# drscotthawley/signaltrain

Measured on AMD Instinct MI355X. Metric: audio-frames/sec (train step) comp_4c 8192-sample windows @ 1/2/4/8 GPUs, higher is better.
Workload: dtype f32; 1 GPU; comp_4c synthetic, 8192-sample windows, batch 256/GPU, fp32 (BASELINE configs[1]); window=8192, frames_per_window=25, global_batch=256, parallelism=dp1

## Files before the change

### signaltrain_amd/csrc/st_ae.h

```cpp
#pragma once
#include "st_common.h"

namespace sta {

constexpr int NL = 9;
#ifndef ST_AE_ABLATE
#define ST_AE_ABLATE 0
#endif

struct AEOffsets { int w[NL]; int b[NL]; };

struct GroupWalk { int first, end, stride; };
__device__ __forceinline__ GroupWalk fwd_group_walk(const int ngroups, const int NW, const int wave)
{
    const int G = (int)gridDim.x, b = (int)blockIdx.x;
    if ((G & 7) == 0) {
        const int S = G >> 3, x = b & 7, slot = b >> 3;
        const int per = (ngroups + 7) >> 3;
        const int lo = x * per, hi = lo + per < ngroups ? lo + per : ngroups;
        return GroupWalk{lo + wave * S + slot, hi, S * NW};
    }
    return GroupWalk{wave * G + b, ngroups, G * NW};
}

struct CL {
    static constexpr int O0 = 64, O1 = 32, O2 = 16, O3 = 16, O4 = 16, O5 = 16, O6 = 32, O7 = 64, O8 = 16;
    static constexpr int I0 = 32, I1 = 64, I2 = 32, I3 = 16, I4 = 32, I5 = 16, I6 = 16, I7 = 32, I8 = 64;
    static constexpr int A0 = 0, A1 = A0 + O0 * I0, A2 = A1 + O1 * I1, A3 = A2 + O2 * I2, A4 = A3 + O3 * I3, A5 = A4 + O4 * I4,
                         A6 = A5 + O5 * I5, A7 = A6 + O6 * I6, A8 = A7 + O7 * I7, AEND = A8 + O8 * I8;
    static constexpr int B0 = AEND, B1 = B0 + O0, B2 = B1 + O1, B3 = B2 + O2, B4 = B3 + O3, B5 = B4 + O4, B6 = B5 + O5,
                         B7 = B6 + O6, B8 = B7 + O7, FWD_TOTAL = B8 + O8;
    static constexpr int G0 = FWD_TOTAL, G1 = G0 + O0 * I0, G2 = G1 + O1 * I1, G3 = G2 + O2 * I2, G4 = G3 + O3 * I3, G5 = G4 + O4 * I4,
                         G6 = G5 + O5 * I5, G7 = G6 + O6 * I6, G8 = G7 + O7 * I7, BWD_TOTAL = G8 + O8 * I8;
    static_assert(FWD_TOTAL % 4 == 0 && BWD_TOTAL % 4 == 0, "16-byte aligned regions");
};

constexpr int ae_max_elems(int l) { return l == 0 ? 64 * 32 : l == 1 ? 32 * 64 : l == 2 ? 16 * 32 : l == 3 ? 16 * 16 : l == 4 ? 16 * 32 :
                                           l == 5 ? 16 * 16 : l == 6 ? 32 * 16 : l == 7 ? 64 * 32 : 16 * 64; }
template <int NT>
struct AEParamRegs { float v[NL][(64 * 32 + NT - 1) / NT]; float bv[NL]; };

template <int NT>
__device__ __forceinline__ void ae_params_issue(AEParamRegs<NT>& r, const float* __restrict__ ae, const AEOffsets& go,
                                                const int T, const int OT, const int K, const int tid, const int l0, const int l1)
{
    const int out[NL] = {64, 32, 16, 16, 16, 16, 32, 64, OT};
    const int in[NL] = {T, 64, 32, 16, 16 + K, 16, 16, 32, 64};
#pragma unroll
    for (int l = 0; l < NL; ++l) {
        const bool on = l >= l0 && l < l1;
        const int n = on ? out[l] * in[l] : 0;
        const float* src = ae + go.w[l];
#pragma unroll
        for (int u = 0; u < (ae_max_elems(l) + NT - 1) / NT; ++u) { const int e = tid + u * NT; r.v[l][u] = src[e < n ? e : 0]; }
        r.bv[l] = ae[go.b[l] + (tid < out[l] ? tid : 0)];
    }
}
template <int BF> __device__ __forceinline__ unsigned short st_half_bits(const float v)
{
    if constexpr (BF == 2) { union { _Float16 h; unsigned short u; } p; p.h = (_Float16)v; return p.u; }
    else { union { __bf16 h; unsigned short u; } p; p.h = (__bf16)v; return p.u; }
}
template <int BF> __device__ __forceinline__ float st_half_to_float(const unsigned short b)
{
    if constexpr (BF == 2) { union { unsigned short u; _Float16 h; } p; p.u = b; return (float)p.h; }
    else return __uint_as_float((unsigned)b << 16);
}
template <int NT, int BF = 0>
__device__ __forceinline__ void ae_params_scatter(float* lds, const AEParamRegs<NT>& r, const int T, const int OT, const int K,
                                                  const int tid, const int l0, const int l1, const bool dgrad_images)
{
    const int out[NL] = {64, 32, 16, 16, 16, 16, 32, 64, OT};
    const int in[NL] = {T, 64, 32, 16, 16 + K, 16, 16, 32, 64};
    const int outp[NL] = {CL::O0, CL::O1, CL::O2, CL::O3, CL::O4, CL::O5, CL::O6, CL::O7, CL::O8};
    const int inp[NL] = {CL::I0, CL::I1, CL::I2, CL::I3, CL::I4, CL::I5, CL::I6, CL::I7, CL::I8};
    const int ao[NL] = {CL::A0, CL::A1, CL::A2, CL::A3, CL::A4, CL::A5, CL::A6, CL::A7, CL::A8};
    const int bo[NL] = {CL::B0, CL::B1, CL::B2, CL::B3, CL::B4, CL::B5, CL::B6, CL::B7, CL::B8};
    const int gi[NL] = {CL::G0, CL::G1, CL::G2, CL::G3, CL::G4, CL::G5, CL::G6, CL::G7, CL::G8};
#pragma unroll
    for (int l = 0; l < NL; ++l) {
        const bool on = l >= l0 && l < l1;
        const int IN = in[l], n = on ? out[l] * IN : 0, OP = outp[l], IP = inp[l];
#pragma unroll
        for (int u = 0; u < (ae_max_elems(l) + NT - 1) / NT; ++u) {
            const int e = tid + u * NT;
            if (e < n) {
                const int o = e / IN, i = e - o * IN;
                if constexpr (BF) {
                    const unsigned short hb = st_half_bits<BF>(r.v[l][u]);
                    reinterpret_cast<unsigned short*>(lds + ao[l])[(((i >> 2) * OP + o) << 2) + (i & 3)] = hb;
                    if (dgrad_images) reinterpret_cast<unsigned short*>(lds + gi[l])[(((o >> 2) * IP + i) << 2) + (o & 3)] = hb;
                } else {
                lds[ao[l] + (((i >> 2) * OP + o) << 2) + (i & 3)] = r.v[l][u];
                if (dgrad_images) lds[gi[l] + (((o >> 2) * IP + i) << 2) + (o & 3)] = r.v[l][u];
                }
            }
        }
        if (on && tid < out[l]) lds[bo[l] + tid] = r.bv[l];
    }
}
template <int NT, int BF = 0>
__device__ inline void ae_load_lds(float* lds, const float* __restrict__ ae, const AEOffsets& go, const int T, const int OT, const int K,
                                   const int tid, const int l0, const int l1, const bool dgrad_images)
{
    AEParamRegs<NT> r;
    ae_params_issue<NT>(r, ae, go, T, OT, K, tid, l0, l1);
    const int total = dgrad_images ? CL::BWD_TOTAL : CL::FWD_TOTAL;
    for (int e = tid; e < total; e += NT) lds[e] = 0.f;
    __syncthreads();
    ae_params_scatter<NT, BF>(lds, r, T, OT, K, tid, l0, l1, dgrad_images);
}
template <int NT, int BF = 0>
__device__ inline void ae_load_lds2(float* lds, const float* __restrict__ ae_m, const float* __restrict__ ae_p, const AEOffsets& go,
                                    const int T, const int OT, const int K, const int tid, const int l0, const int l1)
{
    AEParamRegs<NT> rm, rp;
    ae_params_issue<NT>(rm, ae_m, go, T, OT, K, tid, l0, l1);
    ae_params_issue<NT>(rp, ae_p, go, T, OT, K, tid, l0, l1);
    for (int e = tid; e < 2 * CL::FWD_TOTAL; e += NT) lds[e] = 0.f;
    __syncthreads();
    ae_params_scatter<NT, BF>(lds, rm, T, OT, K, tid, l0, l1, false);
    ae_params_scatter<NT, BF>(lds + CL::FWD_TOTAL, rp, T, OT, K, tid, l0, l1, false);
}

#define ST_MFMA16(a, b, c) __builtin_amdgcn_mfma_f32_16x16x4f32((a), (b), (c), 0, 0, 0)

__device__ __forceinline__ float ldg32(const float* __restrict__ base, const unsigned elem)
{
    return *reinterpret_cast<const float*>(reinterpret_cast<const char*>(base) + (size_t)(elem << 2));
}
__device__ __forceinline__ void stg32(float* __restrict__ base, const unsigned elem, const float v)
{
    *reinterpret_cast<float*>(reinterpret_cast<char*>(base) + (size_t)(elem << 2)) = v;
}
#define ST_MUL24(a, b) __umul24((unsigned)(a), (unsigned)(b))

typedef short s16x4 __attribute__((ext_vector_type(4)));
typedef __bf16 bf16x4_t __attribute__((ext_vector_type(4)));
typedef _Float16 f16x4_t __attribute__((ext_vector_type(4)));
template <int BF>
__device__ __forceinline__ f32x4 mfma16h(const s16x4 a, const s16x4 b, const f32x4 c)
{
    if constexpr (BF == 2) {
        union { s16x4 s; f16x4_t h; } pa, pb; pa.s = a; pb.s = b;
        return __builtin_amdgcn_mfma_f32_16x16x16f16(pa.h, pb.h, c, 0, 0, 0);
    } else return __builtin_amdgcn_mfma_f32_16x16x16bf16_1k(a, b, c, 0, 0, 0);
}
#define ST_MFMA16B(a, b, c) mfma16h<BF>((a), (b), (c))
template <int BF>
__device__ __forceinline__ s16x4 pack_h4(f32x4 v)
{
    if constexpr (BF == 2) {
        union { f16x4_t h; s16x4 s; } p; p.h = __builtin_convertvector(v, f16x4_t); return p.s;
    } else {
        typedef __bf16 bf16x2_t __attribute__((ext_vector_type(2)));
        typedef float f32x2_t __attribute__((ext_vector_type(2)));
        union { bf16x2_t h; unsigned u; } lo, hi;
        lo.h = __builtin_convertvector((f32x2_t){v[0], v[1]}, bf16x2_t);
        hi.h = __builtin_convertvector((f32x2_t){v[2], v[3]}, bf16x2_t);
        union { unsigned u[2]; s16x4 s; } r; r.u[0] = lo.u; r.u[1] = hi.u; return r.s;
    }
}
#define pack_bf16x4(v) pack_h4<BF>(v)
template <int BF>
__device__ __forceinline__ float round_h(const float v)
{
    if constexpr (BF == 2) return (float)(_Float16)v;
    else {
        union { __bf16 h; unsigned short u; } p; p.h = (__bf16)v;
        union { unsigned u; float f; } q; q.u = (unsigned)p.u << 16; return q.f;
    }
}
#define bf16_rne(v) round_h<BF>(v)

template <int BF>
__device__ __forceinline__ f32x4 frag_read(const float* img, const int idx)
{
    if constexpr (BF) {
        typedef float f32x2_t __attribute__((ext_vector_type(2)));
        const f32x2_t lo = *reinterpret_cast<const f32x2_t*>(reinterpret_cast<const unsigned short*>(img) + idx);
        return __builtin_shufflevector(lo, lo, 0, 1, -1, -1);
    } else return *reinterpret_cast<const f32x4*>(img + idx);
}
__device__ __forceinline__ s16x4 frag_bits(const f32x4 v)
{
    typedef float f32x2_t __attribute__((ext_vector_type(2)));
    union { f32x2_t f; s16x4 s; } p; p.f = __builtin_shufflevector(v, v, 0, 1); return p.s;
}
template <int OUTP, int BF = 0>
__device__ __forceinline__ f32x4 frag_fwd(const float* img, const int ot, const int it, const int g, const int c)
{
    return frag_read<BF>(img, ((4 * it + g) * OUTP + 16 * ot + c) << 2);
}
template <int INP, int BF = 0>
__device__ __forceinline__ f32x4 frag_dgrad(const float* img, const int ot, const int it, const int g, const int c)
{
    return frag_read<BF>(img, ((4 * ot + g) * INP + 16 * it + c) << 2);
}

template <int NC, int OTL, int ITL, int OUTP, int BF = 0>
__device__ __forceinline__ void layer_fwd(const float* const (&W)[NC], const float* const (&bias)[NC],
                                          const f32x4 (&hin)[NC][ITL], f32x4 (&hout)[NC][OTL], const int g, const int c)
{
    s16x4 ph[NC][ITL];
    if constexpr (BF) {
// ... 72 lines not shown
        for (int r = 0; r < 4; ++r) {
            const int t = 16 * it + 4 * g + r;
            const unsigned o = base + ST_MUL24(t < T ? t : 0, F);
            in.v[0][it][r] = ldg32(mag, o); in.v[1][it][r] = ldg32(phs, o);
        }
}
__device__ __forceinline__ void fwd_load_kn(FwdIn& in, const float* __restrict__ knobs, const int K, const int b, const int g)
{
#pragma unroll
    for (int q = 0; q < 4; ++q) { const int kn = 4 * q + g; in.kn[q] = ldg32(knobs, ST_MUL24(b, K) + (unsigned)(kn < K ? kn : 0)); }
}
__device__ __forceinline__ void fwd_load_tl(FwdIn& in, const float* __restrict__ mag, const float* __restrict__ phs,
                                            const int b, const int f, const bool fv, const int T, const int OT, const int F, const int g)
{
    const unsigned base = ST_MUL24(ST_MUL24(b, T), F) + (unsigned)(fv ? f : 0);
#pragma unroll
    for (int r = 0; r < 4; ++r) {
        const int to = 4 * g + r;
        const unsigned o = base + ST_MUL24(to < OT ? T - OT + to : 0, F);
        in.tl[0][r] = ldg32(mag, o); in.tl[1][r] = ldg32(phs, o);
    }
}
__device__ __forceinline__ void fwd_mask_v(f32x4 (&v)[2][2], const FwdIn& in, const bool fv, const int T, const int g)
{
#pragma unroll
    for (int it = 0; it < 2; ++it)
#pragma unroll
        for (int r = 0; r < 4; ++r) {
            const bool ok = fv && 16 * it + 4 * g + r < T;
            v[0][it][r] = ok ? in.v[0][it][r] : 0.f; v[1][it][r] = ok ? in.v[1][it][r] : 0.f;
        }
}
__device__ __forceinline__ void fwd_mask_kn(float (&kn)[4], const FwdIn& in, const int K, const int g)
{
#pragma unroll
    for (int q = 0; q < 4; ++q) kn[q] = (4 * q + g) < K ? in.kn[q] : 0.f;
}
__device__ __forceinline__ void fwd_mask_tl(float (&tl)[2][4], const FwdIn& in, const bool fv, const int OT, const int g)
{
#pragma unroll
    for (int r = 0; r < 4; ++r) { const bool ok = fv && 4 * g + r < OT; tl[0][r] = ok ? in.tl[0][r] : 0.f; tl[1][r] = ok ? in.tl[1][r] : 0.f; }
}

constexpr int AE_SV_TILES = 17;
#ifndef ST_SV_NT
#define ST_SV_NT 1
#endif
template <int NTL>
__device__ __forceinline__ void sv_store(float* __restrict__ p, const unsigned lane16, const int tile0, const f32x4 (&h)[NTL])
{
#pragma unroll
    for (int t = 0; t < NTL; ++t) {
        f32x4* q = reinterpret_cast<f32x4*>(reinterpret_cast<char*>(p + (tile0 + t) * 256) + (size_t)lane16);
#if ST_SV_NT & 1
        __builtin_nontemporal_store(h[t], q);
#else
        *q = h[t];
#endif
    }
}
template <int NTL>
__device__ __forceinline__ void sv_load(const float* __restrict__ p, const unsigned lane16, const int tile0, f32x4 (&h)[NTL])
{
#pragma unroll
    for (int t = 0; t < NTL; ++t) {
        const f32x4* q = reinterpret_cast<const f32x4*>(reinterpret_cast<const char*>(p + (tile0 + t) * 256) + (size_t)lane16);
#if ST_SV_NT & 2
        h[t] = __builtin_nontemporal_load(q);
#else
        h[t] = *q;
#endif
    }
}

template <int NW, int BF = 0, bool SV = false>
__global__ void __launch_bounds__(NW * 64)
ae_fwd_kernel(const float* __restrict__ mag, const float* __restrict__ phs, const float* __restrict__ knobs,
              const float* __restrict__ ae_m, const float* __restrict__ ae_p, const AEOffsets go,
              float* __restrict__ mag_hat, float* __restrict__ phs_hat, float* __restrict__ AA,
              float* __restrict__ reg_partial,
              const int B, const int T, const int OT, const int F, const int K, const int KP, const float expfac,
              float* __restrict__ h4x = nullptr,
              unsigned short* __restrict__ AA16 = nullptr, const int aa_ht = 0,
              float* __restrict__ sv = nullptr)
{
    extern __shared__ __attribute__((aligned(16))) float lds[];
    const int tid = threadIdx.x, lane = tid & 63, wave = tid >> 6;
    const int g = lane >> 4, c = lane & 15;
    const float* const lw[2] = {lds, lds + CL::FWD_TOTAL};
    ae_load_lds2<NW * 64, BF>(lds, ae_m, ae_p, go, T, OT, K, tid, 0, NL);
    __syncthreads();

    const int FP = KP / 2, gpw = FP / 16;
    const int ngroups = B * gpw;
    const int KQ = (K + 3) / 4;
    float reg = 0.f;
    float* const wtab = lds + 2 * CL::FWD_TOTAL;
    for (int i = tid; i < FP; i += NW * 64) wtab[i] = i < F ? expf(expfac * (float)i) : 0.f;
    unsigned toF[4], toK[4];
#pragma unroll
    for (int r = 0; r < 4; ++r) { toF[r] = ST_MUL24(4 * g + r, F); toK[r] = ST_MUL24(4 * g + r, KP); }
    __syncthreads();

    f32x4 vin[2][2];
    const GroupWalk gw = fwd_group_walk(ngroups, NW, wave);
    int grp = gw.first;
    if (grp < gw.end) {
        const int b = grp / gpw, f = (grp - b * gpw) * 16 + c;
        FwdIn first; fwd_load_v(first, mag, phs, b, f, f < F, T, F, g); fwd_mask_v(vin, first, f < F, T, g);
    }
    for (; grp < gw.end; grp += gw.stride) {
        asm volatile("" ::: "memory");
        const int b = grp / gpw, f = (grp - b * gpw) * 16 + c;
        const bool fv = f < F;
        const int gn = grp + gw.stride < gw.end ? grp + gw.stride : grp;
        const int bn = gn / gpw, fn = (gn - bn * gpw) * 16 + c;
        FwdIn cur;
        fwd_load_v(cur, mag, phs, bn, fn, fn < F, T, F, g); fwd_load_kn(cur, knobs, K, b, g); fwd_load_tl(cur, mag, phs, b, f, fv, T, OT, F, g);

        f32x4 h1[2][4], h2[2][2], h3[2][1], h4[2][1], h5[2][1], h6[2][1], h7[2][2], h8[2][4], e9[2][1];
        const int grp_u = SV ? __builtin_amdgcn_readfirstlane(grp) : 0;
#ifdef ST_SV_DIAG
        float* const sv0 = SV ? sv + (size_t)(grp_u & ST_SV_DIAG) * (AE_SV_TILES * 256) : nullptr;
#else
        float* const sv0 = SV ? sv + (size_t)grp_u * (AE_SV_TILES * 256) : nullptr;
#endif
        float* const sv1 = SV ? sv0 + (size_t)ngroups * (AE_SV_TILES * 256) : nullptr;
        const unsigned lane16 = (unsigned)lane << 4;
#define ST_SV(t0_, h_) do { if constexpr (SV) { sv_store(sv0, lane16, t0_, h_[0]); sv_store(sv1, lane16, t0_, h_[1]); } } while (0)
        { const float* const W[2] = ST_W2(CL::A0); const float* const bb[2] = ST_W2(CL::B0); layer_fwd<2, 4, 2, CL::O0, BF>(W, bb, vin, h1, g, c); } ST_SV(0, h1);
        { const float* const W[2] = ST_W2(CL::A1); const float* const bb[2] = ST_W2(CL::B1); layer_fwd<2, 2, 4, CL::O1, BF>(W, bb, h1, h2, g, c); } ST_SV(4, h2);
        { const float* const W[2] = ST_W2(CL::A2); const float* const bb[2] = ST_W2(CL::B2); layer_fwd<2, 1, 2, CL::O2, BF>(W, bb, h2, h3, g, c); } ST_SV(6, h3);
        { const float* const W[2] = ST_W2(CL::A3); const float* const bb[2] = ST_W2(CL::B3); layer_fwd<2, 1, 1, CL::O3, BF>(W, bb, h3, h4, g, c); } ST_SV(7, h4);
        if (h4x) {
            float4* hv = reinterpret_cast<float4*>(h4x);
            hv[(size_t)grp * 64 + lane] = make_float4(h4[0][0][0], h4[0][0][1], h4[0][0][2], h4[0][0][3]);
            hv[((size_t)ngroups + grp) * 64 + lane] = make_float4(h4[1][0][0], h4[1][0][1], h4[1][0][2], h4[1][0][3]);
        }
        if (mag_hat) {
        float knv[4]; fwd_mask_kn(knv, cur, K, g);
        layer5_fwd<2, BF>(lw, h4, knv, KQ, h5, g, c); ST_SV(8, h5);
        { const float* const W[2] = ST_W2(CL::A5); const float* const bb[2] = ST_W2(CL::B5); layer_fwd<2, 1, 1, CL::O5, BF>(W, bb, h5, h6, g, c); } ST_SV(9, h6);
        { const float* const W[2] = ST_W2(CL::A6); const float* const bb[2] = ST_W2(CL::B6); layer_fwd<2, 2, 1, CL::O6, BF>(W, bb, h6, h7, g, c); } ST_SV(10, h7);
        { const float* const W[2] = ST_W2(CL::A7); const float* const bb[2] = ST_W2(CL::B7); layer_fwd<2, 4, 2, CL::O7, BF>(W, bb, h7, h8, g, c); } ST_SV(12, h8);
        { const float* const W[2] = ST_W2(CL::A8); const float* const bb[2] = ST_W2(CL::B8); layer_fwd<2, 1, 4, CL::O8, BF>(W, bb, h8, e9, g, c); } ST_SV(16, e9);
#undef ST_SV
        const float wf = fv ? wtab[f] : 0.f;
        float tlv[2][4]; fwd_mask_tl(tlv, cur, fv, OT, g);
        const unsigned boF = ST_MUL24(ST_MUL24(b, OT), F) + (unsigned)f, boK = ST_MUL24(ST_MUL24(b, OT), KP) + (unsigned)f;
#pragma unroll
        for (int r = 0; r < 4; ++r) {
            const int to = 4 * g + r;
            if (to < OT) {
                float mh = 0.f, ph = 0.f, sn = 0.f, cs = 1.f;
                if (fv) {
                    mh = e9[0][0][r] * tlv[0][r];
                    ph = e9[1][0][r] + tlv[1][r];
                    st_sincos(ph, sn, cs);
                    stg32(mag_hat, boF + toF[r], mh);
                    stg32(phs_hat, boF + toF[r], ph);
                    reg += fabsf(mh * wf);
                }
                if (AA16) {
                    const int ht = BF ? BF : aa_ht;
                    AA16[boK + toK[r]] = st_to_h16(mh * cs, ht);
                    AA16[boK + toK[r] + (unsigned)FP] = st_to_h16(mh * sn, ht);
                } else {
                    stg32(AA, boK + toK[r], mh * cs);
                    stg32(AA, boK + toK[r] + (unsigned)FP, mh * sn);
                }
            }
        }
        }
        fwd_mask_v(vin, cur, fn < F, T, g);
    }
    if (reg_partial) {
        reg = wave_sum(reg);
        if (lane == 0) reg_partial[blockIdx.x * NW + wave] = reg;
    }
}

// ... 171 lines not shown
#pragma unroll
        for (int r = 0; r < 4; ++r) d[t][r] = __builtin_fmaf(d[t][r], __builtin_amdgcn_fmed3f(h[t][r], 0.f, -3.0e38f), d[t][r]);
}

template <int OTL, int ITL, int BF = 0>
__device__ __forceinline__ void wgrad_reg(f32x4 (&dW)[OTL][ITL], float (&db)[OTL], const f32x4 (&daT)[OTL], const f32x4 (&hT)[ITL])
{
    s16x4 pht[ITL];
    if constexpr (BF) {
#pragma unroll
        for (int it = 0; it < ITL; ++it) pht[it] = pack_bf16x4(hT[it]);
    }
#pragma unroll
    for (int ot = 0; ot < OTL; ++ot) {
        s16x4 pdt;
        if constexpr (BF) pdt = pack_bf16x4(daT[ot]);
#pragma unroll
        for (int it = 0; it < ITL; ++it) {
#if ST_AE_ABLATE & 4
            dW[ot][it][0] += daT[ot][0] * hT[it][0];
#else
            if constexpr (BF) dW[ot][it] = ST_MFMA16B(pdt, pht[it], dW[ot][it]);
            else {
#pragma unroll
                for (int r = 0; r < 4; ++r) dW[ot][it] = ST_MFMA16(daT[ot][r], hT[it][r], dW[ot][it]);
            }
#endif
        }
        db[ot] += (daT[ot][0] + daT[ot][1]) + (daT[ot][2] + daT[ot][3]);
    }
}
template <int OTL, int ITL, int BF>
__device__ __forceinline__ void wgrad_regh(f32x4 (&dW)[OTL][ITL], float (&db)[OTL], const f32x4 (&daT)[OTL], const typename TTy<BF>::type (&hT)[ITL])
{
    if constexpr (BF == 0) wgrad_reg<OTL, ITL, 0>(dW, db, daT, hT);
    else {
#pragma unroll
        for (int ot = 0; ot < OTL; ++ot) {
            const s16x4 pdt = pack_bf16x4(daT[ot]);
#pragma unroll
            for (int it = 0; it < ITL; ++it) dW[ot][it] = ST_MFMA16B(pdt, hT[it], dW[ot][it]);
            db[ot] += (daT[ot][0] + daT[ot][1]) + (daT[ot][2] + daT[ot][3]);
        }
    }
}
template <int OTL, int ITL, int INP, bool FIRST>
__device__ __forceinline__ void dw_flush(float* dW, const f32x4 (&acc)[OTL][ITL], const int g, const int c)
{
#pragma unroll
    for (int ot = 0; ot < OTL; ++ot)
#pragma unroll
        for (int it = 0; it < ITL; ++it)
#pragma unroll
            for (int r = 0; r < 4; ++r) {
                float* p = dW + (16 * ot + 4 * g + r) * INP + 16 * it + c;
                if constexpr (FIRST) *p = acc[ot][it][r]; else *p += acc[ot][it][r];
            }
}
template <int OTL, bool FIRST>
__device__ __forceinline__ void db_flush(float* dst, float (&db)[OTL], const int g, const int c)
{
#pragma unroll
    for (int ot = 0; ot < OTL; ++ot) {
        float v = db[ot];
        v += __shfl_xor(v, 16); v += __shfl_xor(v, 32);
        if (g == 0) { if constexpr (FIRST) dst[16 * ot + c] = v; else dst[16 * ot + c] += v; }
    }
}

__device__ __forceinline__ void group_colsum_store(float* __restrict__ dst, const f32x4& t, const int g, const int c)
{
    const float v = (t[0] + t[1]) + (t[2] + t[3]);
    const unsigned u = __builtin_bit_cast(unsigned, v);
    const auto p = __builtin_amdgcn_permlane16_swap(u, u, false, false);
    const float w = __builtin_bit_cast(float, (unsigned)p[0]) + __builtin_bit_cast(float, (unsigned)p[1]);
    const unsigned x = __builtin_bit_cast(unsigned, w);
    const auto q = __builtin_amdgcn_permlane32_swap(x, x, false, false);
    const float s = __builtin_bit_cast(float, (unsigned)q[0]) + __builtin_bit_cast(float, (unsigned)q[1]);
    if (g == 0) dst[c] = s;
}

constexpr int AE_BWD_SCR = (32 + 16 + 16) * SP + 2 * 4 * 320;
constexpr int ae_bwd_lds_floats(int nw) { return (CL::BWD_TOTAL + nw * AE_BWD_SCR) > nw * CL::FWD_TOTAL ? (CL::BWD_TOTAL + nw * AE_BWD_SCR) : nw * CL::FWD_TOTAL; }
template <int NW, bool INNER = false, int BF = 0, int VAR = 1, bool SAVED = false, bool KG = false>
__global__ void __launch_bounds__(NW * 64, 1)
ae_bwd_kernel(const float* __restrict__ mag, const float* __restrict__ phs, const float* __restrict__ knobs,
              const float* __restrict__ ae_m, const float* __restrict__ ae_p, const AEOffsets go, const int PG,
              const float* __restrict__ mag_hat, const float* __restrict__ phs_hat, const float* __restrict__ dAA,
              const float* __restrict__ g_mag_hat, const float reg_coef, const float expfac,
              float* __restrict__ dmag, float* __restrict__ dphs, float* __restrict__ ws,
              const int B, const int T, const int OT, const int F, const int K, const int KP,
              const int to_lo, const int to_hi,
              const int nslab, const size_t slab,
              const float* __restrict__ sv = nullptr,
              float* __restrict__ kg = nullptr)
{
    static_assert(!SAVED || (!INNER && BF == 0), "the kept-activation backward exists for the fused fp32 geometries");
    extern __shared__ __attribute__((aligned(16))) float lds[];
    const int ae = blockIdx.y;
    const int tid = threadIdx.x, lane = tid & 63, wave = tid >> 6;
    const int g = lane >> 4, c = lane & 15;
    float* lw = lds;
    float* Vs = lds + CL::BWD_TOTAL + wave * AE_BWD_SCR;
    float* Ys = Vs + 32 * SP;
    float* Ts = Ys + 16 * SP;
    float* XH = Ts + 16 * SP;
    float* XD = XH + 4 * 320;
    ae_load_lds<NW * 64, BF>(lw, ae ? ae_p : ae_m, go, INNER ? 16 : T, INNER ? 16 : OT, K, tid, INNER ? 1 : 0, INNER ? 8 : NL, true);
    __syncthreads();

    const float* vin = ae ? phs : mag;
    const float* dh8in = ae ? phs_hat : mag_hat;
    float* dvout = ae ? dphs : dmag;
    const int FP = KP / 2, gpw = FP / 16;
    const int ngroups = B * gpw;
    const int gstride = gridDim.x * NW;

    f32x4 rW1[4][2], rW2[2][4], rW3[1][2], rW4[1][1], rW5[1][2], rW6[1][1], rW7[2][1], rW8[4][2], rW9[1][4];
    float rb1[4], rb2[2], rb3[1], rb4[1], rb5[1], rb6[1], rb7[2], rb8[4], rb9[1];
#define ST_ZT(x, A, Bq) { _Pragma("unroll") for (int a_ = 0; a_ < A; ++a_) _Pragma("unroll") for (int b_ = 0; b_ < Bq; ++b_) x[a_][b_] = (f32x4){0.f, 0.f, 0.f, 0.f}; }
#define ST_ZB(x, A) { _Pragma("unroll") for (int a_ = 0; a_ < A; ++a_) x[a_] = 0.f; }
    ST_ZT(rW1, 4, 2) ST_ZT(rW2, 2, 4) ST_ZT(rW3, 1, 2) ST_ZT(rW4, 1, 1) ST_ZT(rW5, 1, 2) ST_ZT(rW6, 1, 1) ST_ZT(rW7, 2, 1) ST_ZT(rW8, 4, 2) ST_ZT(rW9, 1, 4)
    ST_ZB(rb1, 4) ST_ZB(rb2, 2) ST_ZB(rb3, 1) ST_ZB(rb4, 1) ST_ZB(rb5, 1) ST_ZB(rb6, 1) ST_ZB(rb7, 2) ST_ZB(rb8, 4) ST_ZB(rb9, 1)
#undef ST_ZT
#undef ST_ZB

    f32x4 vr[2];
    int grp = blockIdx.x * NW + wave;
    auto load_v = [&](int gq, f32x4 (&dst)[2]) {
        const int bq = gq / gpw, fq = (gq - bq * gpw) * 16 + c;
        const unsigned base = ST_MUL24(ST_MUL24(bq, T), F) + (unsigned)(fq < F ? fq : 0);
#pragma unroll
        for (int it = 0; it < 2; ++it)
#pragma unroll
            for (int r = 0; r < 4; ++r) {
                const int t = 16 * it + 4 * g + r;
                dst[it][r] = ldg32(vin, base + ST_MUL24(t < T ? t : 0, F));
            }
    };
    auto mask_v = [&](int gq, f32x4 (&dst)[2]) {
        const int bq = gq / gpw, fq = (gq - bq * gpw) * 16 + c;
        const bool ok0 = fq < F;
#pragma unroll
        for (int it = 0; it < 2; ++it)
#pragma unroll
            for (int r = 0; r < 4; ++r) dst[it][r] = (ok0 && 16 * it + 4 * g + r < T) ? dst[it][r] : 0.f;
    };
    if constexpr (!INNER) { if (grp < ngroups) { load_v(grp, vr); mask_v(grp, vr); } }
    f32x4 kn = (f32x4){0.f, 0.f, 0.f, 0.f}; float knT = 0.f;
    auto load_kn = [&](int gq, f32x4& d4, float& dT) {
        const unsigned kb = ST_MUL24(gq / gpw, K);
#pragma unroll
        for (int r = 0; r < 4; ++r) { const int kidx = 4 * g + r; d4[r] = ldg32(knobs, kb + (unsigned)(kidx < K ? kidx : 0)); }
        dT = ldg32(knobs, kb + (unsigned)(c < K ? c : 0));
    };
    auto mask_kn = [&](f32x4& d4, float& dT) {
#pragma unroll
        for (int r = 0; r < 4; ++r) d4[r] = (4 * g + r) < K ? d4[r] : 0.f;
        dT = c < K ? dT : 0.f;
    };
    if (grp < ngroups) { load_kn(grp, kn, knT); mask_kn(kn, knT); }
    const unsigned Rw = (unsigned)B * FP;

    constexpr bool GM = (VAR & 1) != 0, TAIL16 = (VAR & 2) != 0;
    float q_x[4][3], q_y[4][3], q_ph[4], q_mh[4], q_mt[4], q_gm[4];
    auto load_q = [&](const int gq) {
        const int bq = gq / gpw, fq0 = (gq - bq * gpw) * 16 + c;
        const bool fvq = fq0 < F;
        const int fq = fvq ? fq0 : 0;
        const size_t o1 = nslab > 1 ? slab : 0, o2 = nslab > 2 ? 2 * slab : 0;
        const float* const dA0 = dAA, * const dA1 = dAA + o1, * const dA2 = dAA + o2;
        const float* const dB0 = dA0 + FP, * const dB1 = dA1 + FP, * const dB2 = dA2 + FP;
        const unsigned bOT = ST_MUL24(bq, OT), btF = ST_MUL24(ST_MUL24(bq, T), F) + (unsigned)fq;
#pragma unroll
        for (int r = 0; r < 4; ++r) {
            const int to = 4 * g + r;
            const bool ok = fvq && to < OT;
            const bool lv = ok && to >= to_lo && to <= to_hi;
            const unsigned ro = bOT + (unsigned)(ok ? to : 0);
            const unsigned p0 = ST_MUL24(lv ? ro : 0u, KP) + (unsigned)fq;
            const unsigned pF = ST_MUL24(ro, F) + (unsigned)fq;
#if ST_AE_ABLATE & 1
            q_x[r][0] = q_x[r][1] = q_x[r][2] = q_y[r][0] = q_y[r][1] = q_y[r][2] = 1e-3f * (float)(p0 & 7); q_ph[r] = 0.3f; q_mh[r] = 0.2f + 1e-3f * (float)(pF & 3);
#else
            q_x[r][0] = ldg32(dA0, p0); q_x[r][1] = ldg32(dA1, p0); q_x[r][2] = ldg32(dA2, p0);
            q_y[r][0] = ldg32(dB0, p0); q_y[r][1] = ldg32(dB1, p0); q_y[r][2] = ldg32(dB2, p0);
            q_ph[r] = ldg32(phs_hat, pF); q_mh[r] = ldg32(mag_hat, pF);
#endif
            if constexpr (GM) q_gm[r] = ldg32(g_mag_hat, pF); else q_gm[r] = 0.f;
            if constexpr (!TAIL16) q_mt[r] = ldg32(vin, btF + ST_MUL24(ok ? T - OT + to : 0, F));
// ... 7 lines not shown
#else
    auto svp = [&](const int gq) { return svn + (size_t)__builtin_amdgcn_readfirstlane(gq) * (AE_SV_TILES * 256); };
#endif
    if constexpr (SAVED) {
        if (grp < ngroups) {
            load_q(grp);
            const float* const p = svp(grp);
            sv_load(p, lane16, 16, s_e9); sv_load(p, lane16, 12, s_h8); sv_load(p, lane16, 10, s_h7); sv_load(p, lane16, 9, s_h6); sv_load(p, lane16, 8, s_h5);
            sv_load(p, lane16, 7, s_h4); sv_load(p, lane16, 6, s_h3); sv_load(p, lane16, 4, s_h2); sv_load(p, lane16, 0, s_h1);
        }
    }

    for (; grp < ngroups; grp += gstride) {
        asm volatile("" ::: "memory");
        const int b = grp / gpw, f = (grp - b * gpw) * 16 + c;
        const bool fv = f < F;
        if constexpr (!INNER && !SAVED) load_q(grp);
        f32x4 h1in[4], dh8[4];
        if constexpr (INNER) {
            const unsigned col0 = (unsigned)b * FP + (unsigned)(grp - b * gpw) * 16;
#pragma unroll
            for (int ot = 0; ot < 4; ++ot) {
#pragma unroll
                for (int r = 0; r < 4; ++r) {
                    h1in[ot][r] = ldg32(vin, (unsigned)(16 * ot + 4 * g + r) * Rw + col0 + c);
                    dh8[ot][r] = ldg32(dh8in, (unsigned)(16 * ot + 4 * g + r) * Rw + col0 + c);
                }
            }
        }
        f32x4 vn[2], knn; float knTn;
        const int gnext = grp + gstride < ngroups ? grp + gstride : grp;
#if ST_AE_ABLATE & 64
        vn[0] = vr[0]; vn[1] = vr[1]; knn = kn; knTn = knT;
#else
        if constexpr (!INNER) load_v(gnext, vn);
        load_kn(gnext, knn, knTn);
#endif

        f32x4 h1[4], h2[2], h3[1], h4[1], h5[1], h6[1], h7[2], h8[4], e9[1];
        f32x4 fr9[1 * 4];
        if constexpr (SAVED) {
#pragma unroll
            for (int it = 0; it < 2; ++it)
#pragma unroll
                for (int r = 0; r < 4; ++r) Vs[(16 * it + 4 * g + r) * SP + c] = vr[it][r];
#pragma unroll
            for (int k = 0; k < 4; ++k) { h1[k] = s_h1[k]; h8[k] = s_h8[k]; }
#pragma unroll
            for (int k = 0; k < 2; ++k) { h2[k] = s_h2[k]; h7[k] = s_h7[k]; }
            h3[0] = s_h3[0]; h4[0] = s_h4[0]; h5[0] = s_h5[0]; h6[0] = s_h6[0]; e9[0] = s_e9[0];
        } else {
        f32x4 fr2[2 * 4];
        if constexpr (INNER) {
#pragma unroll
            for (int ot = 0; ot < 4; ++ot) h1[ot] = h1in[ot];
            frags_fwd<2, 4, CL::O1, BF>(fr2, lw + CL::A1, g, c);
        } else {
            f32x4 fr1[4 * 2]; frags_fwd<4, 2, CL::O0, BF>(fr1, lw + CL::A0, g, c);
            frags_fwd<2, 4, CL::O1, BF>(fr2, lw + CL::A1, g, c);
#pragma unroll
            for (int it = 0; it < 2; ++it)
#pragma unroll
                for (int r = 0; r < 4; ++r) Vs[(16 * it + 4 * g + r) * SP + c] = vr[it][r];
            ST_FENCE();
            fwdD_fr<4, 2, BF>(fr1, lw + CL::B0, vr, h1, g);
        }
        f32x4 fr3[1 * 2]; frags_fwd<1, 2, CL::O2, BF>(fr3, lw + CL::A2, g, c); ST_FENCE(); fwdD_fr<2, 4, BF>(fr2, lw + CL::B1, h1, h2, g);
        f32x4 fr4[1 * 1]; frags_fwd<1, 1, CL::O3, BF>(fr4, lw + CL::A3, g, c); ST_FENCE(); fwdD_fr<1, 2, BF>(fr3, lw + CL::B2, h2, h3, g);
        f32x4 fr5[1 * 2]; frags_fwd<1, 2, CL::O4, BF>(fr5, lw + CL::A4, g, c); ST_FENCE(); fwdD_fr<1, 1, BF>(fr4, lw + CL::B3, h3, h4, g);
        f32x4 fr6[1 * 1]; frags_fwd<1, 1, CL::O5, BF>(fr6, lw + CL::A5, g, c); ST_FENCE();
        {
            const f32x4 hk[2] = {h4[0], kn};
            fwdD_fr<1, 2, BF>(fr5, lw + CL::B4, hk, h5, g);
        }
        f32x4 fr7[2 * 1]; frags_fwd<2, 1, CL::O6, BF>(fr7, lw + CL::A6, g, c); ST_FENCE(); fwdD_fr<1, 1, BF>(fr6, lw + CL::B5, h5, h6, g);
        f32x4 fr8[4 * 2]; frags_fwd<4, 2, CL::O7, BF>(fr8, lw + CL::A7, g, c); ST_FENCE(); fwdD_fr<2, 1, BF>(fr7, lw + CL::B6, h6, h7, g);
        if constexpr (!INNER) frags_fwd<1, 4, CL::O8, BF>(fr9, lw + CL::A8, g, c);
        ST_FENCE(); fwdD_fr<4, 2, BF>(fr8, lw + CL::B7, h7, h8, g);
        }
        f32x4 da9[1];
        float dxA[4], mtA[4];
        if constexpr (!INNER) {
            ST_FENCE();
            const float wf = fv ? expf(expfac * (float)f) : 0.f;
#pragma unroll
            for (int r = 0; r < 4; ++r) {
                const int to = 4 * g + r;
                const bool ok = fv && to < OT;
                const bool lv = ok && to >= to_lo && to <= to_hi;
                const float gre = lv ? q_x[r][0] + (nslab > 1 ? q_x[r][1] : 0.f) + (nslab > 2 ? q_x[r][2] : 0.f) : 0.f;
                const float gim = lv ? q_y[r][0] + (nslab > 1 ? q_y[r][1] : 0.f) + (nslab > 2 ? q_y[r][2] : 0.f) : 0.f;
                const float ph = q_ph[r], mh = q_mh[r];
                if constexpr (!TAIL16) asm volatile("" :: "v"(q_mt[r]));
                float sn, cs; st_sincos(ph, sn, cs);
                const float sg = mh > 0.f ? 1.f : (mh < 0.f ? -1.f : 0.f);
                const float dmh = gre * cs + gim * sn + reg_coef * sg * wf + (GM ? q_gm[r] : 0.f);
                const float dph = mh * (gim * cs - gre * sn);
                dxA[r] = ok ? (ae == 0 ? dmh : dph) : 0.f;
                mtA[r] = ae == 0 ? (TAIL16 ? vr[1][r] : q_mt[r]) : 1.f;
            }
            if constexpr (!SAVED) fwdD_fr<1, 4, BF>(fr9, lw + CL::B8, h8, e9, g);
            if constexpr (BF == 0 && !SAVED) {
#pragma unroll
                for (int p_ = 0; p_ < 16; ++p_) { __builtin_amdgcn_sched_group_barrier(0x008, 1, 0); __builtin_amdgcn_sched_group_barrier(0x002, 7, 0); }
            }
            ST_FENCE();
        }
        if constexpr (!INNER) {
#pragma unroll
            for (int r = 0; r < 4; ++r) {
                const int to = 4 * g + r;
                const float eg = elu_grad_from_out(e9[0][r]);
                const float e1 = ae == 0 ? e9[0][r] : 1.f;
                const float d9 = dxA[r] * mtA[r] * eg;
                const float tail = dxA[r] * e1;
                da9[0][r] = d9;
                Ts[to * SP + c] = tail;
                Ys[to * SP + c] = d9;
            }
        }
#define ST_REFILL(...) do { if constexpr (SAVED) { ST_FENCE(); __VA_ARGS__; ST_FENCE(); } } while (0)
        const float* const svq = SAVED ? svp(gnext) : nullptr;
        ST_REFILL(load_q(gnext); sv_load(svq, lane16, 16, s_e9));
#define ST_PIPE(N_) do { \
        __builtin_amdgcn_sched_group_barrier(0x008, (N_) + 2, 0); \
        _Pragma("unroll") for (int p_ = 0; p_ < (N_) - 2; ++p_) { \
            __builtin_amdgcn_sched_group_barrier(0x002, 2, 0); __builtin_amdgcn_sched_group_barrier(0x300, 1, 0); \
            __builtin_amdgcn_sched_group_barrier(0x008, 1, 0); } \
        ST_FENCE(); } while (0)
#define ST_BWD_STAGE(O_, I_, FD_, DA_, DAT_, HP_, HTP_, DAP_, DATP_, RW_, RB_, NEXT_) \
        to_Th<I_, BF>(XH, HP_, HTP_, g, c); ST_FENCE(); \
        dgradD_fr<O_, I_, BF>(FD_, DA_, DAP_); mul_elu_grad<I_>(DAP_, HP_); \
        to_T<I_>(XD, DAP_, DATP_, g, c); NEXT_; \
        wgrad_regh<O_, I_, BF>(RW_, RB_, DAT_, HTP_); \
        ST_PIPE(BF ? O_ * I_ : O_ * I_ * 4);
        typedef typename TTy<BF>::type tt_t;
        tt_t hT8[4]; f32x4 da8[4], daT8[4], fd8[2 * 4];
        if constexpr (INNER) {
            frags_dgrad<4, 2, CL::I7, BF>(fd8, lw + CL::G7, g, c);
            to_Th<4, BF>(XH, h8, hT8, g, c);
#pragma unroll
            for (int ot = 0; ot < 4; ++ot) da8[ot] = dh8[ot];
            mul_elu_grad<4>(da8, h8); to_T<4>(XD, da8, daT8, g, c);
        } else {
            f32x4 daT9[1], fd9[4 * 1];
            frags_dgrad<1, 4, CL::I8, BF>(fd9, lw + CL::G8, g, c);
            daT9[0] = *reinterpret_cast<const f32x4*>(Ys + c * SP + 4 * g);
            ST_BWD_STAGE(1, 4, fd9, da9, daT9, h8, hT8, da8, daT8, rW9, rb9, (frags_dgrad<4, 2, CL::I7, BF>(fd8, lw + CL::G7, g, c)))
            ST_REFILL(sv_load(svq, lane16, 12, s_h8));
        }
        tt_t hT7[2]; f32x4 da7[2], daT7[2], fd7[1 * 2];
        ST_BWD_STAGE(4, 2, fd8, da8, daT8, h7, hT7, da7, daT7, rW8, rb8, (frags_dgrad<2, 1, CL::I6, BF>(fd7, lw + CL::G6, g, c)))
        ST_REFILL(sv_load(svq, lane16, 10, s_h7));
        tt_t hT6[1]; f32x4 da6[1], daT6[1], fd6[1];
        ST_BWD_STAGE(2, 1, fd7, da7, daT7, h6, hT6, da6, daT6, rW7, rb7, (frags_dgrad<1, 1, CL::I5, BF>(fd6, lw + CL::G5, g, c)))
        ST_REFILL(sv_load(svq, lane16, 9, s_h6));
        tt_t hT5[1]; f32x4 da5[1], daT5[1], fd5[1];
        ST_BWD_STAGE(1, 1, fd6, da6, daT6, h5, hT5, da5, daT5, rW6, rb6, (frags_dgrad<1, 1, CL::I4, BF>(fd5, lw + CL::G4, g, c)))
        ST_REFILL(sv_load(svq, lane16, 8, s_h5));
        tt_t hT4[1], hT4k[2]; f32x4 da4[1], daT4[1], fd4[1];
        {
            to_Th<1, BF>(XH, h4, hT4, g, c); ST_FENCE();
            dgradD_fr<1, 1, BF>(fd5, da5, da4); mul_elu_grad<1>(da4, h4);
            to_T<1>(XD, da4, daT4, g, c); frags_dgrad<1, 1, CL::I3, BF>(fd4, lw + CL::G3, g, c); ST_FENCE();
            hT4k[0] = hT4[0];
            hT4k[1] = tt_splat<BF>(knT);
            wgrad_regh<1, 2, BF>(rW5, rb5, daT5, hT4k);
            if constexpr (KG) group_colsum_store(kg + ((size_t)ae * ngroups + grp) * 16, daT5[0], g, c);
        }
        ST_REFILL(sv_load(svq, lane16, 7, s_h4));
        tt_t hT3[1]; f32x4 da3[1], daT3[1], fd3[2 * 1];
        ST_BWD_STAGE(1, 1, fd4, da4, daT4, h3, hT3, da3, daT3, rW4, rb4, (frags_dgrad<1, 2, CL::I2, BF>(fd3, lw + CL::G2, g, c)))
        ST_REFILL(sv_load(svq, lane16, 6, s_h3));
        tt_t hT2[2]; f32x4 da2[2], daT2[2], fd2[4 * 2];
        ST_BWD_STAGE(1, 2, fd3, da3, daT3, h2, hT2, da2, daT2, rW3, rb3, (frags_dgrad<2, 4, CL::I1, BF>(fd2, lw + CL::G1, g, c)))
        ST_REFILL(sv_load(svq, lane16, 4, s_h2));
        tt_t hT1[4]; f32x4 da1[4], daT1[4], fd1[2 * 4];
        if constexpr (INNER) {
            to_Th<4, BF>(XH, h1, hT1, g, c); ST_FENCE();
            dgradD_fr<2, 4, BF>(fd2, da2, da1); mul_elu_grad<4>(da1, h1);
            const unsigned col0 = (unsigned)b * FP + (unsigned)(grp - b * gpw) * 16;
#pragma unroll
            for (int ot = 0; ot < 4; ++ot)
#pragma unroll
                for (int r = 0; r < 4; ++r) stg32(dvout, (unsigned)(16 * ot + 4 * g + r) * Rw + col0 + c, da1[ot][r]);
            ST_FENCE();
            wgrad_regh<2, 4, BF>(rW2, rb2, daT2, hT1);
        } else {
            ST_BWD_STAGE(2, 4, fd2, da2, daT2, h1, hT1, da1, daT1, rW2, rb2, (frags_dgrad<4, 2, CL::I0, BF>(fd1, lw + CL::G0, g, c)))
            ST_REFILL(sv_load(svq, lane16, 0, s_h1));
        }
        f32x4 vT[2], dv[2];
        if constexpr (!INNER) {
#pragma unroll
            for (int it = 0; it < 2; ++it) vT[it] = *reinterpret_cast<const f32x4*>(Vs + (16 * it + c) * SP + 4 * g);
            ST_FENCE();
            dgradD_fr<4, 2, BF>(fd1, da1, dv);
            wgrad_reg<4, 2, BF>(rW1, rb1, daT1, vT);
        }
#undef ST_BWD_STAGE
#undef ST_PIPE
#undef ST_REFILL
        if constexpr (!INNER) {
            mask_v(gnext, vn);
            vr[0] = vn[0]; vr[1] = vn[1];
        }
        mask_kn(knn, knTn); kn = knn; knT = knTn;
        if constexpr (!INNER) {
        float dvs[2][4], tls[2][4];
#pragma unroll
        for (int it = 0; it < 2; ++it)
#pragma unroll
            for (int r = 0; r < 4; ++r) {
                dvs[it][r] = dv[it][r]; asm volatile("" : "+v"(dvs[it][r]));
                const int ti = 16 * it + 4 * g + r - (T - OT);
                tls[it][r] = Ts[(ti >= 0 && ti < OT ? ti : 0) * SP + c];
            }
        const unsigned dv0 = ST_MUL24(ST_MUL24(b, T), F) + (unsigned)f;
#pragma unroll
        for (int it = 0; it < 2; ++it)
#pragma unroll
            for (int r = 0; r < 4; ++r) {
                const int t = 16 * it + 4 * g + r;
                const float v = dvs[it][r] + (t >= T - OT ? tls[it][r] : 0.f);
#if ST_AE_ABLATE & 2
                asm volatile("" :: "v"(v));
#else
                if (fv && t < T) stg32(dvout, dv0 + ST_MUL24(t, F), v);
#endif
            }
        }
    }
    __syncthreads();
    static_assert(NW == 4, "the store pass sums exactly four per-wave images");
    float* dwl = lds + wave * CL::FWD_TOTAL;
    if constexpr (!INNER) { dw_flush<4, 2, CL::I0, true>(dwl + CL::A0, rW1, g, c); dw_flush<1, 4, CL::I8, true>(dwl + CL::A8, rW9, g, c);
                            db_flush<4, true>(dwl + CL::B0, rb1, g, c); db_flush<1, true>(dwl + CL::B8, rb9, g, c); }
    dw_flush<2, 4, CL::I1, true>(dwl + CL::A1, rW2, g, c); dw_flush<1, 2, CL::I2, true>(dwl + CL::A2, rW3, g, c);
    dw_flush<1, 1, CL::I3, true>(dwl + CL::A3, rW4, g, c); dw_flush<1, 2, CL::I4, true>(dwl + CL::A4, rW5, g, c);
    dw_flush<1, 1, CL::I5, true>(dwl + CL::A5, rW6, g, c); dw_flush<2, 1, CL::I6, true>(dwl + CL::A6, rW7, g, c);
    dw_flush<4, 2, CL::I7, true>(dwl + CL::A7, rW8, g, c);
    db_flush<2, true>(dwl + CL::B1, rb2, g, c); db_flush<1, true>(dwl + CL::B2, rb3, g, c); db_flush<1, true>(dwl + CL::B3, rb4, g, c);
    db_flush<1, true>(dwl + CL::B4, rb5, g, c); db_flush<1, true>(dwl + CL::B5, rb6, g, c); db_flush<2, true>(dwl + CL::B6, rb7, g, c);
    db_flush<4, true>(dwl + CL::B7, rb8, g, c);
    __syncthreads();
    auto sum4 = [&](int idx) { return (lds[idx] + lds[CL::FWD_TOTAL + idx]) + (lds[2 * CL::FWD_TOTAL + idx] + lds[3 * CL::FWD_TOTAL + idx]); };
    float* base = ws + ((size_t)blockIdx.x * 2 + ae) * PG;
    const int out[NL] = {64, 32, 16, 16, 16, 16, 32, 64, OT};
    const int in[NL] = {T, 64, 32, 16, 16 + K, 16, 16, 32, 64};
    const int inp[NL] = {CL::I0, CL::I1, CL::I2, CL::I3, CL::I4, CL::I5, CL::I6, CL::I7, CL::I8};
    const int ao[NL] = {CL::A0, CL::A1, CL::A2, CL::A3, CL::A4, CL::A5, CL::A6, CL::A7, CL::A8};
    const int bo[NL] = {CL::B0, CL::B1, CL::B2, CL::B3, CL::B4, CL::B5, CL::B6, CL::B7, CL::B8};
    constexpr int NT = NW * 64;
#pragma unroll
    for (int l = 0; l < NL; ++l) {
        const bool have = !INNER || (l >= 1 && l < 8);
        const int IN = in[l], n = out[l] * IN;
#pragma unroll
        for (int u = 0; u < (ae_max_elems(l) + NT - 1) / NT; ++u) {
            const int e = tid + u * NT;
            if (e < n) { const int o = e / IN, i = e - o * IN; base[go.w[l] + e] = have ? sum4(ao[l] + o * inp[l] + i) : 0.f; }
        }
        if (tid < out[l]) base[go.b[l] + tid] = have ? sum4(bo[l] + tid) : 0.f;
        { const int p0 = go.w[l] + n, np = go.b[l] - p0; if (tid < np) base[p0 + tid] = 0.f; }
        { const int p0 = go.b[l] + out[l], np = (l + 1 < NL ? go.w[l + 1] : PG) - p0; if (tid < np) base[p0 + tid] = 0.f; }
    }
}

}
```

### signaltrain_amd/csrc/st_api.hip

```cpp
#include <hip/hip_runtime.h>
#include <stdarg.h>
#include <stdio.h>
#include <string.h>
#include <math.h>
#include <mutex>
#include <set>
#include <utility>
#include "st_common.h"
#include "st_gemm.h"
#include "st_gemm_planes.h"
#include "st_gemm_tn.h"
#include "st_gemm16.h"
#include "st_misc.h"
#include "st_ae.h"
#include "st_ae_wide.h"
#include "st_ae_split.h"
#include "st_ae32.h"
#include "st_dp.h"
#include "st_feed.h"

static thread_local char g_err[512] = "";
int st_fail(int code, const char* fmt, ...)
{
    va_list ap; va_start(ap, fmt); vsnprintf(g_err, sizeof(g_err), fmt, ap); va_end(ap);
// ... 81 lines not shown
           d->T, d->L, d->N, d->H);
    ST_REQ(d->K <= 16, "at most 16 knobs");
    ST_REQ(d->prec >= ST_PREC_F32 && d->prec <= ST_PREC_F32X3, "st_dims.prec = %d is not an ST_PREC_* level", d->prec);
    ST_REQ(d->loss_scale >= 0.f && d->loss_scale <= 3.0e38f, "st_dims.loss_scale must be 0 (none) or a positive finite scale");
    ST_REQ((size_t)d->B * d->T < ((size_t)1 << 24) && (size_t)d->B * d->T * st_kp_of(d->F) < ((size_t)1 << 30) &&
           (size_t)d->B * ((size_t)d->L + 2 * (size_t)d->N) < ((size_t)1 << 30), "batch too large for 32-bit element offsets (B=%d)", d->B);
    ST_REQ(((unsigned long long)d->B * d->T - 1) * (unsigned long long)d->T < (1ull << 32), "row split inexact: (B*T - 1)*T must stay below 2^32 (B=%d T=%d)", d->B, d->T);
    return ST_OK;
}

static void ae_shapes(const st_dims* d, int* out, int* in)
{
    const int o[9] = {64, 32, 16, 16, 16, 16, 32, 64, d->OT};
    const int i[9] = {d->T, 64, 32, 16, 16 + d->K, 16, 16, 32, 64};
    memcpy(out, o, sizeof(o)); memcpy(in, i, sizeof(i));
}

extern "C" int64_t st_param_offsets(const st_dims* d, int64_t* offs)
{
    if (check_dims(d) != ST_OK) return -1;
    int64_t off = 0; int n = 0;
    auto put = [&](int64_t sz) { if (offs) offs[n] = off; ++n; off += (sz + 3) / 4 * 4; };
    for (int s = 0; s < 4; ++s) put((int64_t)d->N * d->N);
    int out[9], in[9]; ae_shapes(d, out, in);
    for (int a = 0; a < 2; ++a)
        for (int l = 0; l < 9; ++l) { put((int64_t)out[l] * in[l]); put(out[l]); }
    return off;
}

struct Layout {
    int64_t offs[40]; int64_t total; int64_t n_stft; int PG; sta::AEOffsets go; int KP;
};
static int make_layout(const st_dims* d, Layout* L)
{
    ST_TRY(check_dims(d));
    L->total = st_param_offsets(d, L->offs);
    L->n_stft = L->offs[4];
    L->PG = (int)(L->offs[22] - L->offs[4]);
    for (int l = 0; l < 9; ++l) {
        L->go.w[l] = (int)(L->offs[4 + 2 * l] - L->offs[4]);
        L->go.b[l] = (int)(L->offs[5 + 2 * l] - L->offs[4]);
    }
    L->KP = st_kp_of(d->F);
    return ST_OK;
}

static int num_cus()
{
    static int n = 0;
    if (!n) { int dev = 0; (void)hipGetDevice(&dev); hipDeviceProp_t p; if (hipGetDeviceProperties(&p, dev) == hipSuccess) n = p.multiProcessorCount; if (n <= 0) n = 256; }
    return n;
}
extern "C" int st_set_debug(int v) { return v == 0 ? ST_OK : st_fail(ST_ERR_ARG, "st_set_debug(%d): the product library has no run-time ablations (build with -DST_*_ABLATE=bits)", v); }
static int g_dp_inline = 1;
static int g_ae_save = 1;
static int g_ae_split = -1;
static int g_ae32 = 1;
static int g_pl_bf16 = 0;
static int g_wg_split = 0;
static int g_pl_dgrad = 0;
static int g_pl_shape = 3;
static int g_g16 = 1;
static int g_g16_dma = 0;
static int g_nt128 = 1;
static int g_tn128 = 1;
static int g_tn_fm = 3;
static int g_g16_crop = 15;
static int g_frs_nt = 1;
static int g_xt = 0;
static const int NORM_E_PARTIALS = 32;
static const int NORM_E_MAX = 4096;
static int g_wide_direct = 1;
static int g_an_bk = 32;
static int g_bk = 16;
static int g_wg_mode = 0;
#define ST_TUNING_LIST(X) X(g_ae_split, -1) X(g_ae_save, 1) X(g_dp_inline, 1) X(g_pl_bf16, 0) X(g_wg_split, 0) X(g_pl_dgrad, 0) X(g_pl_shape, 3) X(g_g16, 1) X(g_g16_dma, 0) \
    X(g_nt128, 1) X(g_tn128, 1) X(g_frs_nt, 1) X(g_xt, 0) X(g_an_bk, 32) X(g_bk, 16) X(g_wg_mode, 0) X(g_ae32, 1) X(g_wide_direct, 1) X(g_tn_fm, 3) X(g_g16_crop, 15)
static const struct { int first, count; int* var; int value; int* also; } k_tuning_codes[] = {
    {16, 1, &g_an_bk, 16, &g_bk}, {32, 1, &g_an_bk, 32, &g_bk},
    {100, 1, &g_wg_mode, 0, nullptr}, {102, 1, &g_wg_mode, 2, nullptr},
    {7000, 2, &g_xt, 0, nullptr},
    {8000, 2, &g_ae_split, 0, nullptr}, {8002, 1, &g_ae_split, -1, nullptr},
    {8100, 2, &g_ae32, 0, nullptr},
    {8200, 2, &g_ae_save, 0, nullptr},
    {8300, 2, &g_dp_inline, 0, nullptr},
    {9000, 2, &g_frs_nt, 0, nullptr},
    {9100, 1, &g_pl_shape, 0, nullptr}, {9103, 1, &g_pl_shape, 3, nullptr},
    {9200, 2, &g_pl_dgrad, 0, nullptr},
    {9300, 2, &g_wg_split, 0, nullptr},
    {9400, 2, &g_pl_bf16, 0, nullptr},
    {9500, 2, &g_tn128, 0, nullptr}, {9580, 1, &g_tn128, 2, nullptr}, {9581, 1, &g_tn128, 1, nullptr},
    {9540, 4, &g_tn_fm, 0, nullptr},
    {9560, 16, &g_g16_crop, 0, nullptr},
    {9600, 2, &g_g16, 0, nullptr},
    {9690, 4, &g_g16_dma, 0, nullptr},
    {9950, 2, &g_nt128, 0, nullptr},
    {9970, 2, &g_wide_direct, 0, nullptr},
};
extern "C" int st_set_tuning(int code)
{
    for (const auto& t : k_tuning_codes)
        if (code >= t.first && code < t.first + t.count) { *t.var = t.value + (code - t.first); if (t.also) *t.also = *t.var; return ST_OK; }
    return st_fail(ST_ERR_ARG, "st_set_tuning(%d): no such code", code);
}
extern "C" int st_get_tuning(int* out, int n)
{
    int i = 0;
#define X(v_, d_) if (out && i < n) out[i] = v_; ++i;
    ST_TUNING_LIST(X)
#undef X
    return i;
}
extern "C" int st_tuning_defaults(int* out, int n)
{
    int i = 0;
#define X(v_, d_) if (out && i < n) out[i] = d_; ++i;
    ST_TUNING_LIST(X)
#undef X
    return i;
}
extern "C" int st_reset_tuning(void)
{
#define X(v_, d_) v_ = d_;
    ST_TUNING_LIST(X)
#undef X
    return ST_OK;
}
static inline int gemm_ht(int prec) { return (prec == ST_PREC_BF16 || prec == ST_PREC_BF16_ALL) ? 1 : ((prec == ST_PREC_F16 || prec == ST_PREC_F16_ALL) ? 2 : (prec == ST_PREC_F32X3 ? 3 : 0)); }
static inline int ae_ht(int prec) { return prec == ST_PREC_BF16_ALL ? 1 : (prec == ST_PREC_F16_ALL ? 2 : 0); }
static inline float loss_scale_of(const st_dims* d) { return d->loss_scale > 0.f ? d->loss_scale : 1.0f; }
#define ST_GEMM_BK(BK_, W_, ...) do { const int ht_ = gemm_ht(d->prec); \
                              if (ht_ == 1) stg::launch_half<W_, 1>(__VA_ARGS__); else if (ht_ == 2) stg::launch_half<W_, 2>(__VA_ARGS__); \
                              else if (ht_ == 3) { ST_TRY((stg::launch_half<W_, 1, 3>(__VA_ARGS__))); } \
                              else if (g_xt) { if ((BK_) == 16) stg::launch<W_, 16, true>(__VA_ARGS__); else stg::launch<W_, 32, true>(__VA_ARGS__); } \
                              else if ((BK_) == 16) stg::launch<W_, 16>(__VA_ARGS__); else stg::launch<W_, 32>(__VA_ARGS__); } while (0)
#define ST_GEMM(W_, ...) ST_GEMM_BK(g_bk, W_, __VA_ARGS__)
#define ST_GEMM_AN(W_, ...) ST_GEMM_BK(g_an_bk, W_, __VA_ARGS__)
#define ST_GEMM_WG(...) do { if (g_wg_mode == 2 && gemm_ht(d->prec) == 0) stg::launch<3, 16, true>(__VA_ARGS__); \
                             else if (gemm_ht(d->prec) == 3 && !g_wg_split) stg::launch<3, 16>(__VA_ARGS__); else ST_GEMM(3, __VA_ARGS__); } while (0)
static int ensure_dyn_lds(const void* fn, const char* name)
{
    static std::mutex mu; static std::set<std::pair<int, const void*>> done;
    int dev = 0; (void)hipGetDevice(&dev);
    std::lock_guard<std::mutex> lk(mu);
    if (done.count({dev, fn})) return ST_OK;
    const hipError_t e = hipFuncSetAttribute(fn, hipFuncAttributeMaxDynamicSharedMemorySize, 160 * 1024);
    if (e != hipSuccess) return st_fail(ST_ERR_LAUNCH, "hipFuncSetAttribute(%s, 160 KB dynamic LDS): %s", name, hipGetErrorString(e));
    done.insert({dev, fn});
    return ST_OK;
}
#define ST_DYN_LDS(kernel_) ST_TRY(ensure_dyn_lds(reinterpret_cast<const void*>(&kernel_), #kernel_))
static const int AE_FWD_NW = 8, AE_BWD_NW = 4;
static int synth_live_rows(const st_dims* d);
static bool ae_is_wide(const st_dims* d);
static int ae_fwd_groups(const st_dims* d) { return d->B * (st_kp_of(d->F) / 32); }
static int ae_fwd_nw(const st_dims* d)
{
    if (ae_is_wide(d) || ae_ht(d->prec) != 0) return AE_FWD_NW;
    const int groups = ae_fwd_groups(d), c = num_cus();
    auto cost = [&](int nw) { int grid = (groups + nw - 1) / nw; if (grid > c) grid = c; const int rounds = (groups + grid * nw - 1) / (grid * nw); return rounds * nw; };
    return cost(11) < cost(AE_FWD_NW) ? 11 : AE_FWD_NW;
}
static int ae_inner_nw(const st_dims* d)
{
    const int groups = ae_fwd_groups(d), c = num_cus();
    int best = AE_FWD_NW, best_cost = 1 << 30;
    for (int nw : {8, 9, 12}) {
// ... 2 lines not shown
        if (cost < best_cost) { best_cost = cost; best = nw; }
    }
    return best;
}
static int ae_inner_grid(const st_dims* d) { const int nw = ae_inner_nw(d); int g = (ae_fwd_groups(d) + nw - 1) / nw; int c = num_cus(); return g < c ? g : c; }
static int ae_fwd_grid(const st_dims* d) { const int nw = ae_fwd_nw(d); int g = (ae_fwd_groups(d) + nw - 1) / nw; int c = num_cus(); return g < c ? g : c; }
static int ae_bwd_grid(const st_dims* d) { int groups = d->B * (st_kp_of(d->F) / 32); int g = (groups + AE_BWD_NW - 1) / AE_BWD_NW; int c = num_cus() / 2; if (c < 1) c = 1; return g < c ? g : c; }
static const int WSPLIT_ROWS = 200, WSPLIT_MAX = 16;
static int wgrad_split(int R) { int s = R / WSPLIT_ROWS; if (s < 1) s = 1; if (s > WSPLIT_MAX) s = WSPLIT_MAX; return s; }
static int wgrad_split_tiles(int R, int M, int Nc)
{
    int s = wgrad_split(R);
    const int tiles = ((M + 95) / 96) * ((Nc + 95) / 96), slots = 6 * num_cus();
    int fit = slots / (tiles > 0 ? tiles : 1); if (fit < 1) fit = 1;
    if (fit >= 2) fit &= ~1;
    return s < fit ? s : fit;
}
static int synth_split(int R) { return R >= 4096 ? 1 : 3; }

extern "C" int st_ae_fwd_partials(const st_dims* d) { return check_dims(d) != ST_OK ? 0 : ae_fwd_grid(d) * ae_fwd_nw(d); }
extern "C" int st_ola_loss_partials(const st_dims* d) { return check_dims(d) != ST_OK ? 0 : d->B * ((d->y + 255) / 256); }
extern "C" int st_norm_partials(const st_dims* d) { return check_dims(d) != ST_OK ? 0 : stm::norm_partial_count(d->F, d->N); }
static int tn_split(int R, int N)
{
    const int tiles = (N / 128) * (N / 128);
    int s = num_cus() / (tiles > 0 ? tiles : 1); if (s > 16) s = 16;
    const int cap = R / 64; if (s > cap) s = cap;
    return s < 1 ? 1 : s;
}
extern "C" size_t st_wgrad_ws_floats(const st_dims* d)
{
    if (check_dims(d) != ST_OK) return 0;
    int s = wgrad_split_tiles(d->B * d->T, st_kp_of(d->F), d->N);
    const int s2 = tn_split(d->B * d->T, d->N); if (s2 > s) s = s2;
    return (size_t)s * st_kp_of(d->F) * d->N + (size_t)64 * 2 * d->N;
}
static size_t synth_wgrad_ws_floats(const st_dims* d) { return st_wgrad_ws_floats(d); }
extern "C" int st_synth_slabs(const st_dims* d) { return check_dims(d) != ST_OK ? 0 : synth_split(synth_live_rows(d)); }
static int frames_split(int R) { return R >= 4096 ? 1 : 3; }
extern "C" int st_synth_frame_slabs(const st_dims* d) { return check_dims(d) != ST_OK ? 0 : frames_split(synth_live_rows(d)); }
static bool ae_is_wide(const st_dims* d) { return d->T > 32 || d->OT > 16; }
struct WideWS {
    float *W1p[2], *W5p[2], *V[2], *H[2][8], *E9[2];
    float *DA[2][9], *TL[2], *slabs, *inner_ws;
    size_t fwd_floats, floats; int Tp, nsplit; size_t R, SL; int so[10];
};
static void wide_carve(const st_dims* d, float* base, WideWS* w)
{
    const int FP = st_kp_of(d->F) / 2;
    const size_t R = (size_t)d->B * FP;
    const int hrows[8] = {64, 32, 16, 16 + d->K, 16, 16, 32, 64};
    const int drows[9] = {64, 32, 16, 16, 16, 16, 32, 64, d->OT};
    int out[9], in[9]; ae_shapes(d, out, in);
    w->R = R; w->Tp = st_round_up(d->T, 32);
    { long ns = (long)(R / 128); w->nsplit = (int)(ns < 1 ? 1 : (ns > 256 ? 256 : ns)); }
    w->so[0] = 0;
    for (int l = 0; l < 9; ++l) w->so[l + 1] = w->so[l] + st_round_up(out[l] * (in[l] + 1), 64);
    w->SL = (size_t)w->so[9];
    size_t off = 0;
    auto take = [&](size_t n) { float* p = base ? base + off : nullptr; off += (n + 63) / 64 * 64; return p; };
    for (int a = 0; a < 2; ++a) {
        w->W1p[a] = take((size_t)64 * w->Tp); w->W5p[a] = take(16 * 32);
        w->V[a] = take((size_t)(d->T + 1) * R);
        for (int j = 0; j < 8; ++j) w->H[a][j] = take((size_t)(hrows[j] + 1) * R);
        w->E9[a] = take((size_t)d->OT * R);
    }
    w->fwd_floats = off;
    for (int a = 0; a < 2; ++a) {
        for (int l = 0; l < 9; ++l) w->DA[a][l] = take((size_t)drows[l] * R);
        w->TL[a] = take((size_t)d->OT * R);
    }
    w->slabs = take((size_t)2 * w->nsplit * w->SL);
    { Layout L; if (make_layout(d, &L) == ST_OK) w->inner_ws = take((size_t)ae_bwd_grid(d) * 2 * L.PG); else w->inner_ws = nullptr; }
    w->floats = off;
}
static const int AE_SPLIT_NW = 8;
static size_t ae_h4_floats(const st_dims* d) { return (size_t)2 * ae_fwd_groups(d) * 256; }
static int ae_split_grid(const st_dims* d) { int g = (ae_fwd_groups(d) + AE_SPLIT_NW - 1) / AE_SPLIT_NW; int c = num_cus() / 2; if (c < 1) c = 1; return g < c ? g : c; }
static bool ae_use_split(const st_dims* d) { return (g_ae_split < 0 ? ae_ht(d->prec) != 0 : g_ae_split != 0) && !ae_is_wide(d); }
static size_t ae_sv_floats(const st_dims* d) { return (!ae_is_wide(d) && ae_ht(d->prec) == 0) ? (size_t)2 * ae_fwd_groups(d) * sta::AE_SV_TILES * 256 : 0; }
static int ae_parts_max(const st_dims* d) { return ae_split_grid(d) > ae_bwd_grid(d) ? ae_split_grid(d) : ae_bwd_grid(d); }
static bool ae_use_saved(const st_dims* d) { return g_ae_save && !ae_is_wide(d) && ae_ht(d->prec) == 0 && !ae_use_split(d); }
static float* ae_sv_ptr(const st_dims* d, const Layout& L, float* aews) { return aews + 2 * ae_h4_floats(d) + (size_t)ae_parts_max(d) * 2 * L.PG; }
static const char* ae_kg_why(const st_dims* d)
{
    if (ae_is_wide(d)) return nullptr;
    if (ae_use_split(d)) return ae_ht(d->prec) != 0 ? nullptr : "g_ae_split routes fp32 layers to the split kernels";
    if (ae_ht(d->prec) != 0) return "g_ae_split routes 16-bit layers to the single kernel";
    return ae_use_saved(d) ? nullptr : "g_ae_save is off: the recomputing fp32 kernel";
}
static bool ae_kg_route(const st_dims* d) { return ae_kg_why(d) == nullptr; }
extern "C" size_t st_ae_fwd_ws_floats(const st_dims* d)
{
    if (check_dims(d) != ST_OK) return 0;
    if (!ae_is_wide(d)) return ae_h4_floats(d);
    WideWS w; wide_carve(d, nullptr, &w); return w.fwd_floats;
}
extern "C" size_t st_ae_kept_activation_bytes(const st_dims* d)
{
    if (check_dims(d) != ST_OK || !ae_use_saved(d)) return 0;
    return ae_sv_floats(d) * sizeof(float);
}
extern "C" size_t st_ae_bwd_ws_floats(const st_dims* d)
{
    Layout L; if (make_layout(d, &L) != ST_OK) return 0;
    if (ae_is_wide(d)) { WideWS w; wide_carve(d, nullptr, &w); return w.floats; }
    return 2 * ae_h4_floats(d) + (size_t)ae_parts_max(d) * 2 * L.PG + ae_sv_floats(d);
}
static int ae_wide_fwd(const st_dims* d, const Layout& L, const float* mag, const float* phs, const float* knobs,
                       const float* ae_m, const float* ae_p, float* mag_hat, float* phs_hat, float* AA, float* reg_partial,
                       WideWS& w, void* stream, unsigned short* AA16 = nullptr, bool in_done = false);

struct PolarWide { float* Vm; float* Vp; int FP; unsigned RV; };
static inline void polar_wide_set(stg::PolarStore& ep, const PolarWide* pw) { if (pw && pw->Vm) { ep.Vm = pw->Vm; ep.Vp = pw->Vp; ep.FP = pw->FP; ep.RV = pw->RV; } }
static int analysis_fwd_impl(const st_dims* d, const float* sig, bool padded, const float* Wr, const float* Wi, float in_scale,
                             float* re, float* im, float* mag, float* phs, void* stream, bool dead_frames_done = false, const PolarWide* pw = nullptr)
{
    const stg::RowMap map = stg::live_frames(d->T, d->H, d->N, d->N, d->L);
    const int R = map.rows(d->B);
    stg::AnalysisW bl{Wr, Wi, d->F, d->N};
    stg::PolarStore ep{re, im, mag, phs, R, d->F, map};
    polar_wide_set(ep, pw);
    if (padded) {
        stg::FramedNT<true> al{sig, d->L, d->H, d->N, R, d->N, 1.0f, map};
        ST_GEMM_AN(4, al, bl, ep, R, 2 * d->F, d->N, 1, st_stream(stream));
    }
    else { stg::FramedNT<false> al{sig, d->L, d->H, d->N, R, d->N, in_scale, map}; ST_GEMM(4, al, bl, ep, R, 2 * d->F, d->N, 1, st_stream(stream)); }
    ST_LAUNCHED("analysis_fwd");
    if (map.Tv < d->T && !dead_frames_done) {
        hipLaunchKernelGGL(stm::zero_dead_frames_kernel, dim3(d->B * (d->T - map.Tv)), dim3(256), 0, st_stream(stream),
                           re, im, mag, phs, d->T, d->F, map.t_lo, map.Tv);
        ST_LAUNCHED("zero_dead_frames");
    }
    return ST_OK;
}
extern "C" int st_analysis_fwd(const st_dims* d, const float* x, const float* Wr, const float* Wi, float in_scale,
                               float* re, float* im, float* mag, float* phs, void* stream)
{
    ST_TRY(check_dims(d)); ST_REQ(x && Wr && Wi, "st_analysis_fwd: null input");
    return analysis_fwd_impl(d, x, false, Wr, Wi, in_scale, re, im, mag, phs, stream);
}
static int pad_scale(const float* in, float* out, int B, int Ls, int pad, float s, void* stream)
{
    hipLaunchKernelGGL(stm::pad_scale_kernel, dim3(((Ls + 2 * pad) / 4 + 255) / 256, B), dim3(256), 0, st_stream(stream), in, out, Ls, pad, s);
    ST_LAUNCHED("pad_scale");
    return ST_OK;
}

static int ae_fwd_impl(const st_dims* d, const float* mag, const float* phs, const float* knobs,
                       const float* ae_m, const float* ae_p, float* mag_hat, float* phs_hat, float* AA,
                       float* reg_partial, float* ws, void* stream, unsigned short* AA16 = nullptr, bool wide_in_done = false, float* sv = nullptr);
extern "C" int st_ae_fwd(const st_dims* d, const float* mag, const float* phs, const float* knobs,
                         const float* ae_m, const float* ae_p, float* mag_hat, float* phs_hat, float* AA,
                         float* reg_partial, float* ws, void* stream)
{
    return ae_fwd_impl(d, mag, phs, knobs, ae_m, ae_p, mag_hat, phs_hat, AA, reg_partial, ws, stream);
}
static int ae_fwd_impl(const st_dims* d, const float* mag, const float* phs, const float* knobs,
                       const float* ae_m, const float* ae_p, float* mag_hat, float* phs_hat, float* AA,
                       float* reg_partial, float* ws, void* stream, unsigned short* AA16, bool wide_in_done, float* sv)
{
    Layout L; ST_TRY(make_layout(d, &L));
    const int aa_ht = AA16 ? gemm_ht(d->prec) : 0;
    ST_REQ(mag && phs && (knobs || d->K == 0) && ae_m && ae_p && ((mag_hat && phs_hat && AA) || (!mag_hat && !phs_hat && !AA && ws)), "st_ae_fwd: null pointer");
    if (!knobs) knobs = ae_m;
    if (ae_is_wide(d)) {
        ST_REQ(mag_hat, "st_ae_fwd: the code-only pass exists for the fused geometries only");
        ST_REQ(ws, "st_ae_fwd: this geometry (T=%d, OT=%d) needs st_ae_fwd_ws_floats() floats of workspace", d->T, d->OT);
        WideWS w; wide_carve(d, ws, &w);
        return ae_wide_fwd(d, L, mag, phs, knobs, ae_m, ae_p, mag_hat, phs_hat, AA, reg_partial, w, stream, AA16, wide_in_done);
    }
    ST_REQ((size_t)d->B * d->T * d->F < ((size_t)1 << 30) && (size_t)d->B * d->OT * L.KP < ((size_t)1 << 30),
           "st_ae_fwd: batch too large for the kernel's 32-bit element offsets (B=%d)", d->B);
    const size_t lds = ((size_t)2 * sta::CL::FWD_TOTAL + (size_t)(L.KP / 2)) * sizeof(float);
    const float expfac = (float)(7.0 / d->F);
#define ST_AE_FWD_LAUNCH(HT_) do { ST_DYN_LDS((sta::ae_fwd_kernel<AE_FWD_NW, HT_>)); \
        hipLaunchKernelGGL((sta::ae_fwd_kernel<AE_FWD_NW, HT_>), dim3(ae_fwd_grid(d)), dim3(AE_FWD_NW * 64), lds, st_stream(stream), \
                           mag, phs, knobs, ae_m, ae_p, L.go, mag_hat, phs_hat, AA, reg_partial, \
                           d->B, d->T, d->OT, d->F, d->K, L.KP, expfac, ws, AA16, aa_ht); } while (0)
    const bool use32 = g_ae32 && ae_ht(d->prec) != 0 && L.KP / 2 <= 17 * 32 && AE_FWD_NW == 8;
#define ST_AE_FWD32_LAUNCH(HT_) do { ST_DYN_LDS((sta::ae_fwd32_kernel<AE_FWD_NW, HT_>)); \
        hipLaunchKernelGGL((sta::ae_fwd32_kernel<AE_FWD_NW, HT_>), dim3(ae_fwd_grid(d)), dim3(AE_FWD_NW * 64), (size_t)sta::ae32_lds_floats(L.KP / 2) * sizeof(float), st_stream(stream), \
                           mag, phs, knobs, ae_m, ae_p, L.go, mag_hat, phs_hat, AA, reg_partial, \
                           d->B, d->T, d->OT, d->F, d->K, L.KP, expfac, ws, AA16, aa_ht); } while (0)
    switch (ae_ht(d->prec)) {
    case 1: if (use32) ST_AE_FWD32_LAUNCH(1); else ST_AE_FWD_LAUNCH(1); break;
    case 2: if (use32) ST_AE_FWD32_LAUNCH(2); else ST_AE_FWD_LAUNCH(2); break;
    default:
        if (sv) {
            ST_REQ(mag_hat, "st_ae_fwd: internal: kept activations on a code-only pass");
#define ST_AE_FWD_SV(NW_) do { ST_DYN_LDS((sta::ae_fwd_kernel<NW_, 0, true>)); \
            hipLaunchKernelGGL((sta::ae_fwd_kernel<NW_, 0, true>), dim3(ae_fwd_grid(d)), dim3(NW_ * 64), lds, st_stream(stream), \
                               mag, phs, knobs, ae_m, ae_p, L.go, mag_hat, phs_hat, AA, reg_partial, d->B, d->T, d->OT, d->F, d->K, L.KP, expfac, ws, AA16, aa_ht, sv); } while (0)
            if (ae_fwd_nw(d) == 11) ST_AE_FWD_SV(11); else ST_AE_FWD_SV(AE_FWD_NW);
#undef ST_AE_FWD_SV
        } else if (ae_fwd_nw(d) == 11) {
            ST_DYN_LDS((sta::ae_fwd_kernel<11, 0>));
            hipLaunchKernelGGL((sta::ae_fwd_kernel<11, 0>), dim3(ae_fwd_grid(d)), dim3(11 * 64), lds, st_stream(stream),
                               mag, phs, knobs, ae_m, ae_p, L.go, mag_hat, phs_hat, AA, reg_partial, d->B, d->T, d->OT, d->F, d->K, L.KP, expfac, ws, AA16, aa_ht);
        } else ST_AE_FWD_LAUNCH(0);
    }
#undef ST_AE_FWD_LAUNCH
#undef ST_AE_FWD32_LAUNCH
    ST_LAUNCHED("ae_fwd"); return ST_OK;
}

extern "C" int st_synth_fold(const st_dims* d, const float* Sr, const float* Si, float* Sfold, void* stream)
{
    ST_TRY(check_dims(d)); ST_REQ(Sr && Si && Sfold, "st_synth_fold: null pointer");
    const int KP = st_kp_of(d->F);
    hipLaunchKernelGGL(stm::fold_kernel, dim3(KP), dim3(256), 0, st_stream(stream), Sr, Si, Sfold, d->N, d->F, KP);
    ST_LAUNCHED("synth_fold"); return ST_OK;
}

static stg::RowMap synth_live(const st_dims* d) { return stg::live_frames(d->OT, d->H, d->N, d->N, d->y); }
static int synth_live_rows(const st_dims* d) { return synth_live(d).rows(d->B); }

static int synthesis_frames_impl(const st_dims* d, const float* AA, const float* Sfold, const float* SfoldT, float* frs, void* stream);
extern "C" int st_synthesis_frames(const st_dims* d, const float* AA, const float* Sfold, float* frs, void* stream)
{
    ST_TRY(check_dims(d)); ST_REQ(AA && Sfold && frs, "st_synthesis_frames: null pointer");
    return synthesis_frames_impl(d, AA, Sfold, nullptr, frs, stream);
}
static double synth_crop_fraction(const st_dims* d)
{
    const stg::RowMap ms = synth_live(d);
    long live = 0;
    for (int t = ms.t_lo; t < ms.t_lo + ms.Tv; ++t) { int lo, hi; stg::ntw_live_taps(t, t, d->H, d->N, d->N, d->y, lo, hi); live += hi - lo; }
    return 1.0 - (double)live / ((double)ms.Tv * (double)d->N);
}
static inline bool fm_div_exact(int R, int B) { return R >= 0 && B >= 1 && (unsigned long long)(unsigned)R * (unsigned long long)(unsigned)B < (1ull << 32); }
extern "C" int st_fm_div_exact(int R, int B) { return fm_div_exact(R, B) ? 1 : 0; }
static bool use_nt128(const st_dims* d, int M, int Nc, int ncus = 0)
{
    if (!(g_nt128 && gemm_ht(d->prec) == 0 && d->N % 32 == 0 && (M + 127) / 128 <= 255 && fm_div_exact(M, d->B))) return false;
    if (ncus <= 0) ncus = num_cus();
    return ((M + 127) / 128) * ((Nc + 127) / 128) * 2 <= ncus || synth_crop_fraction(d) >= 0.10;
}
static int synthesis_frames_impl(const st_dims* d, const float* AA, const float* Sfold, const float* SfoldT, float* frs, void* stream)
{
    const int KP = st_kp_of(d->F);
    const stg::RowMap ms = synth_live(d);
    const int R = ms.rows(d->B);
    stg::PlainNT al{AA, R, KP, KP, ms};
    stg::PlainTN bl{Sfold, KP, d->N, d->N, stg::all_frames(1)};
    stg::StoreC ep{frs, R, d->N, d->N, (size_t)d->B * d->OT * d->N, ms};
    if (SfoldT && g_frs_nt) {
        stg::PlainNT bt{SfoldT, d->N, KP, KP, stg::all_frames(1)};
        stg::NTWork wk;
        if (use_nt128(d, R, d->N) && stg::ntw_frames(wk, ms, d->B, d->H, d->N, d->N, d->y, KP, frames_split(R), num_cus())) {
            const stg::NTRows ra = stg::ntrows_frame_major(AA, (unsigned)(d->OT * KP), (unsigned)KP, ms, d->B, R), rb{SfoldT, (unsigned)KP, 0u, 0u, 1, 0, d->N};
            const stg::StoreSlab es{frs, R, d->N, d->N, (size_t)d->B * d->OT * d->N, stg::frame_major(ms, d->B)};
            ST_TRY(stg::launch_nt128(ra, rb, es, wk, st_stream(stream)));
        }
        else if (R >= 4096) ST_GEMM(4, al, bt, ep, R, d->N, KP, 1, st_stream(stream));
        else ST_GEMM(2, al, bt, ep, R, d->N, KP, frames_split(R), st_stream(stream));
    }
    else if (R >= 4096) ST_GEMM(4, al, bl, ep, R, d->N, KP, 1, st_stream(stream));
    else ST_GEMM(2, al, bl, ep, R, d->N, KP, frames_split(R), st_stream(stream));
    ST_LAUNCHED("synthesis_frames"); return ST_OK;
}

extern "C" int st_nt128_worklist(const st_dims* d, int which, int ncus, unsigned* out, int cap, int* head6)
{
    if (check_dims(d) != ST_OK || !out || !head6 || cap < 0 || (which != 0 && which != 1)) return -1;
    const int KP = st_kp_of(d->F);
    const stg::RowMap ms = synth_live(d);
    const int R = ms.rows(d->B);
    if (ncus <= 0) ncus = num_cus();
    stg::NTWork wk; wk.n = 0;
    if (!use_nt128(d, R, which ? KP : d->N, ncus)) return 0;
    const bool ok = which ? stg::ntw_dgrad(wk, ms, d->B, d->H, d->N, d->N, d->y, d->F, KP, R >= 4096 ? 1 : synth_split(R), ncus)
                          : stg::ntw_frames(wk, ms, d->B, d->H, d->N, d->N, d->y, KP, frames_split(R), ncus);
    if (!ok) return 0;
    head6[0] = wk.nslabs; head6[1] = wk.col_h; head6[2] = wk.col_stride; head6[3] = d->B; head6[4] = wk.kunit; head6[5] = wk.kt_total;
    for (int i = 0; i < wk.n && i < cap; ++i) out[i] = wk.e[i];
    return wk.n;
}

static int ola_loss_impl(const st_dims* d, const float* frs, const float* x, const float* y_true,
                         float* y_hat, float* dsyn, int dsyn_pad, float* loss_partial, void* stream, unsigned short* dsyn16 = nullptr,
                         bool with_mae = false)
// ... 219 lines not shown
                       const float* g_mag_hat, float reg_coef, float* dmag, float* dphs, WideWS& w, float* g_m, float* g_p,
                       bool have_fwd, void* stream, const PolarSink* sink = nullptr,
                       const stw::SynReduce* syn = nullptr, float* norm_e = nullptr, int* n_norm_e = nullptr, float* kg = nullptr)
{
    hipStream_t s = st_stream(stream);
    const int FP = L.KP / 2, F = d->F, T = d->T, OT = d->OT, R = (int)w.R;
    const int wide_ht = ae_ht(d->prec);
    const stg::RowMap id = stg::all_frames(1);
    int out[9], in[9]; ae_shapes(d, out, in);
    if (!have_fwd) ST_TRY(ae_wide_fwd(d, L, mag, phs, knobs, ae_m, ae_p, nullptr, nullptr, nullptr, nullptr, w, stream));
    stw::OnesRows rows;
    for (int a = 0; a < 2; ++a) {
        rows.p[9 * a] = w.V[a] + (size_t)in[0] * R;
        for (int j = 0; j < 8; ++j) rows.p[9 * a + 1 + j] = w.H[a][j] + (size_t)in[j + 1] * R;
    }
    const float expfac = (float)(7.0 / d->F);
    const stg::RowMap ms = synth_live(d);
    {
        const size_t n = (size_t)d->B * OT * FP;
        ST_REQ(n < ((size_t)1 << 30), "wide autoencoder path: batch too large (B=%d)", d->B);
        int grid = (int)((n + 255) / 256); if (grid > 8192) grid = 8192;
        hipLaunchKernelGGL(stw::wide_dout_kernel, dim3(grid + 18 * d->B), dim3(256), 0, s, dAA, st_synth_slabs(d), (size_t)d->B * OT * L.KP,
                           mag_hat, phs_hat, w.E9[0], w.E9[1], w.V[0] + (size_t)(T - OT) * R, g_mag_hat, reg_coef, expfac,
                           w.DA[0][8], w.DA[1][8], w.TL[0], w.TL[1], d->B, OT, F, FP, L.KP, ms.t_lo, ms.t_lo + ms.Tv - 1, grid, rows);
        ST_LAUNCHED("ae_wide_dout");
    }
    stw::GradTab tab;
    for (int l = 0; l < 9; ++l) { tab.so[l] = w.so[l]; tab.out[l] = out[l]; tab.in[l] = in[l]; tab.gw[l] = L.go.w[l]; tab.gb[l] = L.go.b[l]; }
    tab.so[9] = w.so[9];
    int inner_parts = 0;
    wide_wgrad_pair(d, w, 8, out, in, s, wide_ht);
    {
        stg::PlainTN al0{ae_m + L.go.w[8], out[8], in[8], in[8], id}, al1{ae_p + L.go.w[8], out[8], in[8], in[8], id};
        stg::PlainTN bl0{w.DA[0][8], out[8], R, R, id}, bl1{w.DA[1][8], out[8], R, R, id};
        stg::StoreC ep0{w.DA[0][7], in[8], R, R, 0, id}, ep1{w.DA[1][7], in[8], R, R, 0, id};
        ST_WGEMM_PAIR(al0, bl0, ep0, al1, bl1, ep1, in[8], R, out[8], 1, s);
    }
    {
        const size_t lds = (size_t)sta::ae_bwd_lds_floats(AE_BWD_NW) * sizeof(float);
        const int grid = ae_bwd_grid(d);
#define ST_AE_INNER_BWD_K(HT_, KG_) do { ST_DYN_LDS((sta::ae_bwd_kernel<AE_BWD_NW, true, HT_, 0, false, KG_>)); \
            hipLaunchKernelGGL((sta::ae_bwd_kernel<AE_BWD_NW, true, HT_, 0, false, KG_>), dim3(grid, 2), dim3(AE_BWD_NW * 64), lds, s, \
                               (const float*)w.H[0][0], (const float*)w.H[1][0], knobs, ae_m, ae_p, L.go, L.PG, \
                               (const float*)w.DA[0][7], (const float*)w.DA[1][7], (const float*)nullptr, (const float*)nullptr, 0.f, 0.f, \
                               w.DA[0][0], w.DA[1][0], w.inner_ws, d->B, T, OT, F, d->K, L.KP, 0, 0, 1, (size_t)0, (const float*)nullptr, kg); } while (0)
#define ST_AE_INNER_BWD(HT_) do { if (kg) ST_AE_INNER_BWD_K(HT_, true); else ST_AE_INNER_BWD_K(HT_, false); } while (0)
        switch (wide_ht) { case 1: ST_AE_INNER_BWD(1); break; case 2: ST_AE_INNER_BWD(2); break; default: ST_AE_INNER_BWD(0); }
#undef ST_AE_INNER_BWD
#undef ST_AE_INNER_BWD_K
        inner_parts = grid;
    }
    for (int l = 1; l < 8; ++l) tab.out[l] = 0;
    wide_wgrad_pair(d, w, 0, out, in, s, wide_ht);
    if (norm_e && 2 * ((w.so[9] + 63) / 64 + (L.PG + 63) / 64) > NORM_E_MAX) norm_e = nullptr;
    hipLaunchKernelGGL(stw::wide_grad_finish_kernel, dim3((w.so[9] + 63) / 64 + (L.PG + 63) / 64 + (syn ? st_norm_partials(d) : 0), 2), dim3(256), 0, s, w.slabs, w.nsplit, w.SL, tab, g_m, g_p,
                       (w.so[9] + 63) / 64, (const float*)w.inner_ws, inner_parts, L.PG, syn ? *syn : stw::SynReduce{}, norm_e);
    if (norm_e && n_norm_e) *n_norm_e = 2 * ((w.so[9] + 63) / 64 + (L.PG + 63) / 64);
    {
        stw::DvPolarArgs q;
        q.DA1m = w.DA[0][0]; q.DA1p = w.DA[1][0]; q.TLm = w.TL[0]; q.TLp = w.TL[1]; q.W1m = ae_m + L.go.w[0]; q.W1p = ae_p + L.go.w[0];
        q.re = sink ? sink->re : nullptr; q.im = sink ? sink->im : nullptr; q.g_mag = sink ? sink->g_mag : nullptr;
        q.dG = sink ? sink->dG : nullptr; q.dG16 = sink ? sink->dG16 : nullptr;
        q.dmag = sink ? nullptr : dmag; q.dphs = sink ? nullptr : dphs;
        q.ht = gemm_ht(d->prec) <= 2 ? gemm_ht(d->prec) : 0; q.sat = gemm_ht(d->prec) == 2 ? 65504.0f : 0.0f;
        q.B = d->B; q.T = T; q.OT = OT; q.F = F; q.FP = FP; q.KP = L.KP;
        const int TP16 = (T + 15) / 16 * 16, groups = d->B * (FP / 16);
        ST_REQ(TP16 <= 192, "wide autoencoder path: T = %d frames exceeds the layer-1 data-gradient kernel's 192", T);
        const size_t lds = (size_t)2 * (wide_ht ? 32 : 64) * TP16 * sizeof(float);
        int grid = ((groups + 7) / 8) * (TP16 / 16); if (grid > num_cus()) grid = num_cus();
#define ST_DVP(HT_) do { ST_DYN_LDS((stw::wide_dv_polar_kernel<HT_>)); hipLaunchKernelGGL((stw::wide_dv_polar_kernel<HT_>), dim3(grid), dim3(512), lds, s, q); } while (0)
        switch (wide_ht) { case 1: ST_DVP(1); break; case 2: ST_DVP(2); break; default: ST_DVP(0); }
#undef ST_DVP
    }
    ST_LAUNCHED("ae_wide_bwd");
    return ST_OK;
}
#undef ST_WGEMM_PAIR

static int ae_bwd_impl(const st_dims* d, const float* mag, const float* phs, const float* knobs,
                       const float* ae_m, const float* ae_p, const float* mag_hat, const float* phs_hat,
                       const float* dAA, const float* g_mag_hat, float reg_coef, float* dmag, float* dphs, float* ws,
                       float* g_m, float* g_p, bool have_fwd, void* stream, bool* defer_reduce = nullptr,
                       const PolarSink* sink = nullptr, const stw::SynReduce* syn = nullptr, float* norm_e = nullptr, int* n_norm_e = nullptr,
                       float* kg = nullptr)
{
    Layout L; ST_TRY(make_layout(d, &L));
    ST_REQ(mag && phs && (knobs || d->K == 0) && ae_m && ae_p && mag_hat && phs_hat && dAA && dmag && dphs && ws && g_m && g_p, "st_ae_bwd: null pointer");
    if (!knobs) knobs = ae_m;
    if (ae_is_wide(d)) {
        if (defer_reduce) *defer_reduce = false;
        WideWS w; wide_carve(d, ws, &w);
        return ae_wide_bwd(d, L, mag, phs, knobs, ae_m, ae_p, mag_hat, phs_hat, dAA, g_mag_hat, reg_coef, dmag, dphs, w, g_m, g_p, have_fwd, stream, sink, syn, norm_e, n_norm_e, kg);
    }
    if (kg && !(ae_kg_route(d) && have_fwd)) return st_fail(ST_ERR_UNSUPPORTED, "st_ae_bwd: no per-group d a5 output on this autoencoder backward route (%s)", ae_kg_why(d));
    const size_t lds = (size_t)sta::ae_bwd_lds_floats(AE_BWD_NW) * sizeof(float);
    static_assert((size_t)sta::ae_bwd_lds_floats(AE_BWD_NW) * sizeof(float) <= 160 * 1024, "ae_bwd LDS budget");
    ST_REQ((size_t)st_synth_slabs(d) * d->B * d->OT * L.KP < ((size_t)1 << 30) && (size_t)d->B * d->T * L.KP < ((size_t)1 << 30),
           "st_ae_bwd: batch too large for the kernel's 32-bit element offsets (B=%d)", d->B);
    const float expfac = (float)(7.0 / d->F);
    const stg::RowMap live = synth_live(d);
    float* h4x = ws;
    float* da4x = ws + ae_h4_floats(d);
    float* parts = ws + 2 * ae_h4_floats(d);
    int grid = ae_bwd_grid(d);
    if (ae_use_split(d)) {
        if (!have_fwd) {
            st_dims dd = *d; dd.prec = d->prec;
            ST_TRY(st_ae_fwd(&dd, mag, phs, knobs, ae_m, ae_p, nullptr, nullptr, nullptr, nullptr, h4x, stream));
        }
        grid = ae_split_grid(d);
        static_assert((size_t)sta::ae_split_lds_floats<1>(AE_SPLIT_NW) * sizeof(float) <= 160 * 1024 && (size_t)sta::ae_split_lds_floats<2>(AE_SPLIT_NW) * sizeof(float) <= 160 * 1024, "split ae_bwd LDS budget");
#define ST_AE_PART_K(PART_, HT_, GM_, KG_) do { ST_DYN_LDS((sta::ae_bwd_part_kernel<AE_SPLIT_NW, PART_, HT_, GM_, KG_>)); \
        hipLaunchKernelGGL((sta::ae_bwd_part_kernel<AE_SPLIT_NW, PART_, HT_, GM_, KG_>), dim3(grid, 2), dim3(AE_SPLIT_NW * 64), \
                           (size_t)sta::ae_split_lds_floats<PART_>(AE_SPLIT_NW) * sizeof(float), st_stream(stream), \
                           mag, phs, knobs, ae_m, ae_p, L.go, L.PG, mag_hat, phs_hat, dAA, g_mag_hat, reg_coef, expfac, dmag, dphs, parts, \
                           (const float*)h4x, da4x, d->B, d->T, d->OT, d->F, d->K, L.KP, live.t_lo, live.t_lo + live.Tv - 1, st_synth_slabs(d), \
                           (size_t)d->B * d->OT * L.KP, kg); } while (0)
#define ST_AE_PART(PART_, HT_, GM_) ST_AE_PART_K(PART_, HT_, GM_, false)
#define ST_AE_PARTS(HT_) do { if (g_mag_hat) ST_AE_PART(1, HT_, true); else ST_AE_PART(1, HT_, false); ST_LAUNCHED("ae_bwd_dec"); ST_AE_PART(2, HT_, false); ST_LAUNCHED("ae_bwd_enc"); } while (0)
#define ST_AE_PARTS_KG(HT_) do { if (g_mag_hat) ST_AE_PART_K(1, HT_, true, true); else ST_AE_PART_K(1, HT_, false, true); ST_LAUNCHED("ae_bwd_dec"); ST_AE_PART(2, HT_, false); ST_LAUNCHED("ae_bwd_enc"); } while (0)
        if (kg) { if (ae_ht(d->prec) == 1) ST_AE_PARTS_KG(1); else ST_AE_PARTS_KG(2); }
        else
        switch (ae_ht(d->prec)) { case 1: ST_AE_PARTS(1); break; case 2: ST_AE_PARTS(2); break; default: ST_AE_PARTS(0); }
#undef ST_AE_PARTS_KG
#undef ST_AE_PARTS
#undef ST_AE_PART
#undef ST_AE_PART_K
        if (defer_reduce && *defer_reduce) return ST_OK;
        hipLaunchKernelGGL(stm::ae_grad_reduce_kernel, dim3((L.PG + 63) / 64, 2), dim3(256), 0, st_stream(stream), parts, grid, L.PG, g_m, g_p);
        ST_LAUNCHED("ae_grad_reduce"); return ST_OK;
    }
#define ST_AE_BWD_LAUNCH(HT_, VAR_) do { ST_DYN_LDS((sta::ae_bwd_kernel<AE_BWD_NW, false, HT_, VAR_>)); \
    hipLaunchKernelGGL((sta::ae_bwd_kernel<AE_BWD_NW, false, HT_, VAR_>), dim3(grid, 2), dim3(AE_BWD_NW * 64), lds, st_stream(stream), \
                       mag, phs, knobs, ae_m, ae_p, L.go, L.PG, mag_hat, phs_hat, dAA, g_mag_hat, reg_coef, expfac, \
                       dmag, dphs, parts, d->B, d->T, d->OT, d->F, d->K, L.KP, live.t_lo, live.t_lo + live.Tv - 1, st_synth_slabs(d), (size_t)d->B * d->OT * L.KP); } while (0)
    const int var = g_mag_hat ? 1 : (d->T - d->OT == 16 ? 2 : 0);
    if (have_fwd && ae_use_saved(d)) {
        const float* sv = ae_sv_ptr(d, L, ws);
#define ST_AE_BWD_SV_K(VAR_, KG_) do { ST_DYN_LDS((sta::ae_bwd_kernel<AE_BWD_NW, false, 0, VAR_, true, KG_>)); \
        hipLaunchKernelGGL((sta::ae_bwd_kernel<AE_BWD_NW, false, 0, VAR_, true, KG_>), dim3(grid, 2), dim3(AE_BWD_NW * 64), lds, st_stream(stream), \
                       mag, phs, knobs, ae_m, ae_p, L.go, L.PG, mag_hat, phs_hat, dAA, g_mag_hat, reg_coef, expfac, \
                       dmag, dphs, parts, d->B, d->T, d->OT, d->F, d->K, L.KP, live.t_lo, live.t_lo + live.Tv - 1, st_synth_slabs(d), (size_t)d->B * d->OT * L.KP, sv, kg); } while (0)
#define ST_AE_BWD_SV(VAR_) do { if (kg) ST_AE_BWD_SV_K(VAR_, true); else ST_AE_BWD_SV_K(VAR_, false); } while (0)
        if (var == 1) ST_AE_BWD_SV(1); else if (var == 2) ST_AE_BWD_SV(2); else ST_AE_BWD_SV(0);
#undef ST_AE_BWD_SV
#undef ST_AE_BWD_SV_K
        ST_LAUNCHED("ae_bwd");
        if (defer_reduce && *defer_reduce) return ST_OK;
        hipLaunchKernelGGL(stm::ae_grad_reduce_kernel, dim3((L.PG + 63) / 64, 2), dim3(256), 0, st_stream(stream), parts, grid, L.PG, g_m, g_p);
        ST_LAUNCHED("ae_grad_reduce"); return ST_OK;
    }
#define ST_AE_BWD_VARS(HT_) do { if (var == 1) ST_AE_BWD_LAUNCH(HT_, 1); else if (var == 2) ST_AE_BWD_LAUNCH(HT_, 2); else ST_AE_BWD_LAUNCH(HT_, 0); } while (0)
    switch (ae_ht(d->prec)) { case 1: ST_AE_BWD_VARS(1); break; case 2: ST_AE_BWD_VARS(2); break; default: ST_AE_BWD_VARS(0); }
#undef ST_AE_BWD_VARS
#undef ST_AE_BWD_LAUNCH
    ST_LAUNCHED("ae_bwd");
    if (defer_reduce && *defer_reduce) return ST_OK;
    hipLaunchKernelGGL(stm::ae_grad_reduce_kernel, dim3((L.PG + 63) / 64, 2), dim3(256), 0, st_stream(stream),
                       parts, grid, L.PG, g_m, g_p);
    ST_LAUNCHED("ae_grad_reduce"); return ST_OK;
}
extern "C" int st_ae_bwd(const st_dims* d, const float* mag, const float* phs, const float* knobs,
                         const float* ae_m, const float* ae_p, const float* mag_hat, const float* phs_hat,
                         const float* dAA, const float* g_mag_hat, float reg_coef, float* dmag, float* dphs, float* ws,
                         float* g_m, float* g_p, void* stream)
{
    return ae_bwd_impl(d, mag, phs, knobs, ae_m, ae_p, mag_hat, phs_hat, dAA, g_mag_hat, reg_coef, dmag, dphs, ws, g_m, g_p, false, stream);
}

extern "C" int st_polar_bwd(const st_dims* d, const float* re, const float* im, const float* dmag, const float* dphs,
                            const float* g_mag, float* dG, void* stream)
{
    ST_TRY(check_dims(d)); ST_REQ(re && im && dmag && dphs && dG, "st_polar_bwd: null pointer");
    const int R = d->B * d->T, KP = st_kp_of(d->F);
    hipLaunchKernelGGL(stm::polar_bwd_kernel, dim3((KP / 2 + 255) / 256, R), dim3(256), 0, st_stream(stream),
                       re, im, dmag, dphs, g_mag, dG, R, d->F, KP, gemm_ht(d->prec) == 2 ? 65504.0f : 0.0f);
    ST_LAUNCHED("polar_bwd"); return ST_OK;
}

static int analysis_wgrad_impl(const st_dims* d, const float* dG, const float* sig, bool padded, float in_scale, float* ws,
                               float* gWr, float* gWi, float* norm_partial, void* stream, int half = -1, float* stage = nullptr, int stage_bf16 = 0)
{
    const int KP = st_kp_of(d->F);
    const stg::RowMap ma = stg::live_frames(d->T, d->H, d->N, d->N, d->L);
    const int R = ma.rows(d->B);
    int ns = wgrad_split_tiles(R, KP, d->N);
    if (half >= 0) {
        const int tiles = ((KP / 2 + 95) / 96) * ((d->N + 95) / 96), cus = num_cus();
        int best = ns; double bf = -1.0;
        for (int c = ns; c >= (ns + 1) / 2 && c >= 1; --c) {
            const int w = tiles * c, rounds = (w + cus - 1) / cus;
            const double f = (double)w / ((double)rounds * cus);
            if (f > bf + 1e-9) { bf = f; best = c; }
        }
        ns = best;
    }
    const int M = half < 0 ? KP : KP / 2, m0 = half > 0 ? KP / 2 : 0;
    stm::NyqJob nyq{}; nyq.on = 0;
    const stg::TNOperand ta{dG, (unsigned)(d->T * KP), (unsigned)KP}, tb{sig, (unsigned)(d->L + 2 * d->N), (unsigned)d->H};
    if (half < 0 && use_tn128(d, padded) && stg::tn128_fits(ta, tb, sig, ma, d->N, d->N, (size_t)d->B * d->T * KP, (size_t)d->B * (d->L + 2 * d->N))) {
        ns = tn_split(R, d->N);
        const TNFrameMajor fm = tn_frame_major(ta, tb, ma, d->B, d->H, d->N, d->N, d->L, (g_tn_fm & 2) != 0);
        ST_TRY(wgrad_tn128(d, fm.a, fm.b, sig, fm.map, R, ws, ns, &nyq, stream, &fm.trim));
    } else {
        stg::PlainTN al{dG + m0, R, KP, M, ma};
        stg::StoreC ep{ws + (size_t)m0 * d->N, M, d->N, d->N, (size_t)KP * d->N, stg::all_frames(1)};
        if (padded) { stg::FramedTN<true> bl{sig, d->L, d->H, d->N, R, d->N, 1.0f, ma}; ST_GEMM_WG(al, bl, ep, M, d->N, R, ns, st_stream(stream)); }
        else { stg::FramedTN<false> bl{sig, d->L, d->H, d->N, R, d->N, in_scale, ma}; ST_GEMM_WG(al, bl, ep, M, d->N, R, ns, st_stream(stream)); }
    }
    ST_LAUNCHED("analysis_wgrad");
    const int nrows = half < 0 ? 2 * d->F : d->F, extra = half == 0 ? 0 : stm::nyq_blocks(d->N);
    hipLaunchKernelGGL(stm::wgrad_reduce_kernel, dim3(nrows + extra), dim3(256), 0, st_stream(stream),
                       ws, ns, gWr, gWi, norm_partial, d->N, d->F, KP, 0, half > 0 ? d->F : 0, nrows, stage, nyq, 0, stage_bf16);
    ST_LAUNCHED("analysis_wgrad_reduce");
    return ST_OK;
}
extern "C" int st_analysis_wgrad(const st_dims* d, const float* dG, const float* x, float in_scale, float* ws,
                                 float* gWr, float* gWi, float* norm_partial, void* stream)
{
    ST_TRY(check_dims(d)); ST_REQ(dG && x && ws && gWr && gWi && norm_partial, "st_analysis_wgrad: null pointer");
    return analysis_wgrad_impl(d, dG, x, false, in_scale, ws, gWr, gWi, norm_partial, stream);
}

extern "C" int st_finalize_scalars(const st_dims* d, const float* loss_partial, const float* reg_partial,
                                   const float* norm_a, const float* norm_s, float inv_world, float* scalars, void* stream)
{
// ... 241 lines not shown
    if ((g_g16_dma & 2) && d->N % 64 == 0 && d->N / 64 >= ns) {
        if (gemm_ht(d->prec) == 2) ST_TRY((stg::launch16_nt256<2>(ra, rb, ep, R, KP, d->N, ns, st_stream(stream))));
        else ST_TRY((stg::launch16_nt256<1>(ra, rb, ep, R, KP, d->N, ns, st_stream(stream))));
    }
    else if (gemm_ht(d->prec) == 2) ST_TRY((stg::launch16_nt<2>(ra, rb, ep, R, KP, d->N, ns, st_stream(stream), &cr)));
    else ST_TRY((stg::launch16_nt<1>(ra, rb, ep, R, KP, d->N, ns, st_stream(stream), &cr)));
    ST_LAUNCHED("synthesis_dgrad"); return ST_OK;
}
static int g16_wsplit(const st_dims* d, int R)
{
    const int KP = st_kp_of(d->F), tiles = ((KP + 127) / 128) * (d->N / 128);
    int s = (2 * num_cus()) / (tiles > 0 ? tiles : 1);
    const int cap = R / 128; if (s > cap) s = cap;
    const int room = (int)(st_wgrad_ws_floats(d) / ((size_t)KP * d->N)); if (s > room) s = room;
    return s < 1 ? 1 : s;
}
static int wgrad16(const st_dims* d, const unsigned short* A, unsigned SA1, const unsigned short* Bsig, unsigned SB1, const stg::RowMap& map, int R,
                   float* slabs, int ns, void* stream, int m0 = 0, int M = -1,
                   int trim_Ls = 0)
{
    const int KP = st_kp_of(d->F);
    if (M < 0) M = KP;
    const unsigned short* lo = A < Bsig ? A : Bsig;
    ST_REQ((size_t)(A - lo) + (size_t)R / map.Tv * SA1 + 256 < ((size_t)1 << 30) && (size_t)(Bsig - lo) + (size_t)R / map.Tv * SB1 + 256 < ((size_t)1 << 30) && map.Tv >= 2 &&
           SA1 < (1u << 23) && SB1 < (1u << 23), "16-bit weight-gradient GEMM: operands out of the 32-bit / 24-bit addressing range (B=%d)", d->B);
    stg::TN16Job j;
    j.base = lo; j.a0 = (unsigned)(A - lo) + (unsigned)m0; j.b0 = (unsigned)(Bsig - lo); j.zero = j.b0;
    j.SA1 = SA1; j.SA2 = (unsigned)KP; j.SB1 = SB1; j.SB2 = (unsigned)d->H;
    j.magic = map.magic; j.Tv = map.Tv; j.t_lo = map.t_lo; j.K = R;
    j.trim = 0; j.fB = 0; j.nsplit = 1;
    for (int i = 0; i < 64; ++i) { j.fa[i] = 0; j.fb[i] = 0; }
    if (trim_Ls > 0 && d->B >= 2 && fm_div_exact(R, d->B)) {
        const stg::FrameTrim ft = stg::frame_trim(map, d->B, d->H, d->N, d->N, trim_Ls);
        j.a0 += (unsigned)map.t_lo * (unsigned)KP; j.b0 += (unsigned)map.t_lo * (unsigned)d->H;
        j.SA1 = (unsigned)KP; j.SA2 = SA1; j.SB1 = (unsigned)d->H; j.SB2 = SB1;
        j.magic = stg::rowmap_magic(d->B); j.Tv = d->B; j.t_lo = 0;
        j.trim = ft.on; j.fB = d->B;
        for (int i = 0; i < 64; ++i) { j.fa[i] = ft.fa[i]; j.fb[i] = ft.fb[i]; }
    }
    stg::StoreC ep{slabs + (size_t)m0 * d->N, M, d->N, d->N, (size_t)KP * d->N, stg::all_frames(1)};
    const int ht = gemm_ht(d->prec);
    if (ht == 2) ST_TRY((stg::launch16_tn<2, 64>(j, ep, M, d->N, ns, st_stream(stream)))); else ST_TRY((stg::launch16_tn<1, 64>(j, ep, M, d->N, ns, st_stream(stream))));
    return ST_OK;
}

static int forward_impl(const st_dims* d, const Layout& L, const float* params, const float* x, const float* knobs,
                        const float* y_true, float* y_hat, float* mag, float* mag_hat, WS& w, bool save, void* stream, float* eval_p = nullptr)
{
    const float* Wr = params + L.offs[0]; const float* Wi = params + L.offs[1];
    const float* Sr = params + L.offs[2]; const float* Si = params + L.offs[3];
    const float* ae_m = params + L.offs[4]; const float* ae_p = params + L.offs[22];
    const bool wide_direct = ae_is_wide(d) && g_wide_direct && (size_t)d->B * (L.KP / 2) * (size_t)(d->T > 64 ? d->T : 64) < ((size_t)1 << 30);
    WideWS ww; if (wide_direct) wide_carve(d, w.aews, &ww);
    PolarWide pwide{nullptr, nullptr, 0, 0u};
    if (wide_direct) pwide = PolarWide{ww.V[0], ww.V[1], L.KP / 2, (unsigned)ww.R};
    {
        const stg::RowMap map = stg::live_frames(d->T, d->H, d->N, d->N, d->L);
        stm::PrepArgs a;
        a.x = x; a.xp = w.xp; a.Ls = d->L; a.pad = d->N; a.scale = 0.5f;
        a.nbx = ((d->L + 2 * d->N) / 4 + 255) / 256; a.n_pad = a.nbx * d->B;
        a.Sr = Sr; a.Si = Si; a.Sfold = w.Sfold; a.SfoldT = w.SfoldT; a.N = d->N; a.F = d->F; a.KP = L.KP; a.n_fold = (L.KP / 32) * (d->N / 32);
        a.re = save ? w.re : nullptr; a.im = save ? w.im : nullptr; a.mag = w.mag; a.phs = w.phs; a.T = d->T; a.t_lo = map.t_lo; a.Tv = map.Tv;
        const int n_dead = d->B * (d->T - map.Tv);
        a.n_dead = n_dead; a.ht = w.g16 ? gemm_ht(d->prec) : 0; a.n_w16 = 0;
        a.xp16 = w.xp16; a.Sfold16 = w.Sfold16; a.SfoldT16 = w.SfoldT16; a.W16 = w.W16; a.Wr = Wr; a.Wi = Wi;
        if (a.ht) a.n_w16 = (int)(((size_t)2 * d->F * (d->N / 4) + 255) / 256);
        a.wd = stm::PrepWide{}; a.wd.n_vpad = a.wd.n_kn = a.wd.n_pj = 0;
        if (wide_direct) {
            const int FP = L.KP / 2, Tp = ww.Tp;
            a.wd.Vm = ww.V[0]; a.wd.Vp = ww.V[1]; a.wd.FP = FP; a.wd.B = d->B; a.wd.R = (unsigned)ww.R;
            a.wd.H4Km = ww.H[0][3]; a.wd.H4Kp = ww.H[1][3]; a.wd.knobs = knobs; a.wd.K = d->K;
            int blk = 0;
            for (int n = 0; n < 2; ++n) {
                const float* ae = n ? ae_p : ae_m;
                a.wd.pj.src[2 * n] = ae + L.go.w[0]; a.wd.pj.dst[2 * n] = ww.W1p[n]; a.wd.pj.rows[2 * n] = 64; a.wd.pj.cols[2 * n] = d->T; a.wd.pj.pitch[2 * n] = Tp;
                a.wd.pj.blk0[2 * n] = blk; blk += (64 * Tp + 255) / 256;
                a.wd.pj.src[2 * n + 1] = ae + L.go.w[4]; a.wd.pj.dst[2 * n + 1] = ww.W5p[n]; a.wd.pj.rows[2 * n + 1] = 16; a.wd.pj.cols[2 * n + 1] = 16 + d->K; a.wd.pj.pitch[2 * n + 1] = 32;
                a.wd.pj.blk0[2 * n + 1] = blk; blk += 2;
            }
            a.wd.pj.blk0[4] = blk; a.wd.n_pj = blk;
            a.wd.n_vpad = (int)(((size_t)d->B * d->T * (FP - d->F) + 255) / 256); if (a.wd.n_vpad < 1) a.wd.n_vpad = 1;
            a.wd.n_kn = (int)(((size_t)d->K * d->B * (FP / 4) + 255) / 256);
        }
        hipLaunchKernelGGL(stm::prep_kernel, dim3(a.n_pad + a.n_fold + n_dead + a.wd.n_vpad + a.wd.n_kn + a.wd.n_pj + a.n_w16), dim3(256), 0, st_stream(stream), a);
        ST_LAUNCHED("prep");
    }
    const bool planes = use_planes(d) && !w.g16;
    const bool polar_rows = !(wide_direct && y_true && !mag);
    float* const pmag = polar_rows ? w.mag : nullptr; float* const pphs = polar_rows ? w.phs : nullptr;
    if (w.g16) ST_TRY(analysis_fwd16(d, w, save ? w.re : nullptr, save ? w.im : nullptr, pmag, pphs, stream, &pwide));
    else if (planes) {
        ST_TRY(planes_prepare(d, Wr, Wi, w, stream));
        ST_TRY(analysis_fwd_planes(d, w, save ? w.re : nullptr, save ? w.im : nullptr, pmag, pphs, stream, &pwide));
    } else
    ST_TRY(analysis_fwd_impl(d, w.xp, true, Wr, Wi, 1.0f, save ? w.re : nullptr, save ? w.im : nullptr, pmag, pphs, stream, true, &pwide));
    float* sv = nullptr;
    if (save && ae_use_saved(d)) { Layout Ls; ST_TRY(make_layout(d, &Ls)); sv = ae_sv_ptr(d, Ls, w.aews); }
    ST_TRY(ae_fwd_impl(d, w.mag, w.phs, knobs, ae_m, ae_p, w.mag_hat, w.phs_hat, w.AA, w.reg_p,
                       (ae_is_wide(d) || (save && ae_use_split(d))) ? w.aews : nullptr, stream, w.g16 ? w.AA16 : nullptr, wide_direct, sv));
    if (w.g16) ST_TRY(synthesis_frames16(d, w, stream)); else
    if (planes) ST_TRY(synthesis_frames_planes(d, w, stream)); else
    ST_TRY(synthesis_frames_impl(d, w.AA, w.Sfold, w.SfoldT, w.frs, stream));
    ST_TRY(ola_loss_impl(d, w.frs, x, y_true, y_hat ? y_hat : w.y_hat, (save && y_true) ? w.dsyn : nullptr, d->N,
                         eval_p ? eval_p : y_true ? w.loss_p : nullptr, stream, w.g16 ? w.dsyn16 : nullptr, eval_p != nullptr));
    const size_t nm = (size_t)d->B * d->T * d->F * sizeof(float), nh = (size_t)d->B * d->OT * d->F * sizeof(float);
    if (mag && hipMemcpyAsync(mag, w.mag, nm, hipMemcpyDeviceToDevice, st_stream(stream)) != hipSuccess) return st_fail(ST_ERR_LAUNCH, "copy mag");
    if (mag_hat && hipMemcpyAsync(mag_hat, w.mag_hat, nh, hipMemcpyDeviceToDevice, st_stream(stream)) != hipSuccess) return st_fail(ST_ERR_LAUNCH, "copy mag_hat");
    return ST_OK;
}

static int backward_syn(const st_dims* d, const Layout& L, float* grads, WS& w, void* stream, int* defer_slabs = nullptr, stm::NyqJob* defer_nyq = nullptr)
{
    if (w.g16) {
        ST_TRY(synthesis_dgrad16(d, w, stream));
        const stg::RowMap ms = synth_live(d);
        const int R = ms.rows(d->B), KP = st_kp_of(d->F), ns = g16_wsplit(d, R);
        ST_TRY(wgrad16(d, w.AA16, (unsigned)(d->OT * KP), w.dsyn16, (unsigned)(d->y + 2 * d->N), ms, R, w.wg, ns, stream, 0, -1, (g_g16_crop & 4) ? d->y : 0));
        ST_LAUNCHED("synthesis_wgrad");
        if (defer_slabs) { *defer_slabs = ns; if (defer_nyq) { *defer_nyq = stm::NyqJob{}; defer_nyq->on = 0; } return ST_OK; }
        stm::NyqJob nq{}; nq.on = 0;
        hipLaunchKernelGGL(stm::wgrad_reduce_kernel, dim3(st_norm_partials(d)), dim3(256), 0, st_stream(stream),
                           w.wg, ns, grads + L.offs[2], grads + L.offs[3], w.norm_s, d->N, d->F, KP, 1, 0, 2 * d->F, (float*)nullptr, nq);
        ST_LAUNCHED("synthesis_wgrad_reduce");
        return ST_OK;
    }
    if (use_planes(d) && g_pl_dgrad) ST_TRY(synthesis_dgrad_planes(d, w, stream)); else
    ST_TRY(synthesis_dgrad_impl(d, w.dsyn, true, w.Sfold, w.dAA, stream));
    return synthesis_wgrad_impl(d, w.AA, w.dsyn, true, w.wg, grads + L.offs[2], grads + L.offs[3], w.norm_s, stream, defer_slabs, defer_nyq);
}
static int backward_ae(const st_dims* d, const Layout& L, const float* params, float* grads,
                       const float* knobs, const float* g_mag_hat, const float* g_mag, float reg_coef, WS& w, void* stream, int syn_slabs = 0,
                       const stm::NyqJob* syn_nyq = nullptr, float* kg = nullptr)
{
    const float* ae_m = params + L.offs[4]; const float* ae_p = params + L.offs[22];
    bool deferred = true;
    const PolarSink sink{w.re, w.im, g_mag, w.g16 ? nullptr : w.dG, w.g16 ? w.dG16 : nullptr};
    stw::SynReduce syn{};
    if (syn_slabs > 0 && ae_is_wide(d)) {
        syn.wg = w.wg; syn.nz = syn_slabs; syn.gSr = grads + L.offs[2]; syn.gSi = grads + L.offs[3]; syn.norm_s = w.norm_s; syn.N = d->N; syn.F = d->F; syn.KP = L.KP;
        syn.nyq = stm::NyqJob{}; syn.nyq.on = 0; if (syn_nyq) syn.nyq = *syn_nyq;
    }
    ST_TRY(ae_bwd_impl(d, w.mag, w.phs, knobs, ae_m, ae_p, w.mag_hat, w.phs_hat, w.dAA, g_mag_hat, reg_coef, w.dmag, w.dphs,
                       w.aews, grads + L.offs[4], grads + L.offs[22], true, stream, &deferred, &sink, syn.wg ? &syn : nullptr,
                       (d->clip_all && ae_is_wide(d)) ? w.norm_e : nullptr, &w.n_norm_e, kg));
    if (!deferred) return ST_OK;
    stm::PostAeArgs a;
    a.ws = w.aews + 2 * ae_h4_floats(d); a.nparts = ae_use_split(d) ? ae_split_grid(d) : ae_bwd_grid(d); a.PG = L.PG; a.g_m = grads + L.offs[4]; a.g_p = grads + L.offs[22];
    a.n_red_x = (L.PG + 63) / 64; a.n_red = 2 * a.n_red_x;
    a.re = w.re; a.im = w.im; a.dmag = w.dmag; a.dphs = w.dphs; a.g_mag = g_mag; a.dG = w.dG; a.F = d->F; a.KP = L.KP;
    a.gx = (L.KP / 2 + 255) / 256; a.sat = gemm_ht(d->prec) == 2 ? 65504.0f : 0.0f;
    a.n_polar = a.gx * d->B * d->T;
    a.polar_total = 0; a.polar_magic = 0;
    if (stm::polar_flat_ok((long long)d->B * d->T, L.KP / 2)) {
        a.polar_total = (unsigned)((long long)d->B * d->T * (L.KP / 2)); a.polar_magic = stm::polar_magic(L.KP / 2);
        a.n_polar = (int)((a.polar_total + 256 * stm::POLAR_EPT - 1) / (256 * stm::POLAR_EPT));
    }
    a.wg = w.wg; a.wg_nz = syn_slabs; a.gSr = grads + L.offs[2]; a.gSi = grads + L.offs[3]; a.norm_s = w.norm_s; a.N = d->N;
    a.nyq = stm::NyqJob{}; a.nyq.on = 0; if (syn_nyq) a.nyq = *syn_nyq;
    a.dG16 = nullptr; a.ht = 0;
    if (w.g16) { a.dG16 = w.dG16; a.ht = gemm_ht(d->prec); a.dG = nullptr; }
    a.norm_e = nullptr;
    if (d->clip_all && a.n_red <= NORM_E_MAX) { a.norm_e = w.norm_e; w.n_norm_e = a.n_red; }
    hipLaunchKernelGGL(stm::post_ae_kernel, dim3(a.n_red + a.n_polar + (syn_slabs > 0 ? st_norm_partials(d) : 0)), dim3(256), 0, st_stream(stream), a);
    ST_LAUNCHED("post_ae");
    return ST_OK;
}
static int backward_p1(const st_dims* d, const Layout& L, const float* params, float* grads,
                       const float* knobs, const float* g_mag_hat, const float* g_mag, float reg_coef, WS& w, void* stream, float* kg = nullptr)
{
    int syn_slabs = 0; stm::NyqJob syn_nyq{}; syn_nyq.on = 0;
    ST_TRY(backward_syn(d, L, grads, w, stream, &syn_slabs, &syn_nyq));
    return backward_ae(d, L, params, grads, knobs, g_mag_hat, g_mag, reg_coef, w, stream, syn_slabs, &syn_nyq, kg);
}
static int backward_p2(const st_dims* d, const Layout& L, float* grads, const float* x, WS& w, void* stream, float* stage = nullptr, int stage_bf16 = 0)
{
    (void)x;
    if (w.g16) {
        const stg::RowMap ma = stg::live_frames(d->T, d->H, d->N, d->N, d->L);
        const int R = ma.rows(d->B), KP = st_kp_of(d->F), ns = g16_wsplit(d, R);
        ST_TRY(wgrad16(d, w.dG16, (unsigned)(d->T * KP), w.xp16, (unsigned)(d->L + 2 * d->N), ma, R, w.wg, ns, stream, 0, -1, (g_g16_crop & 8) ? d->L : 0));
        ST_LAUNCHED("analysis_wgrad");
        stm::NyqJob nq{}; nq.on = 0;
        hipLaunchKernelGGL(stm::wgrad_reduce_kernel, dim3(st_norm_partials(d)), dim3(256), 0, st_stream(stream),
                           w.wg, ns, grads + L.offs[0], grads + L.offs[1], w.norm_a, d->N, d->F, KP, 0, 0, 2 * d->F, stage, nq, 0, stage_bf16);
        ST_LAUNCHED("analysis_wgrad_reduce");
        return ST_OK;
    }
    return analysis_wgrad_impl(d, w.dG, w.xp, true, 1.0f, w.wg, grads + L.offs[0], grads + L.offs[1], w.norm_a, stream, -1, stage, stage_bf16);
}
static int analysis_wgrad_half(const st_dims* d, const Layout& L, float* grads, WS& w, int half, float* stage, int stage_bf16, stm::NyqJob* nyq_io, void* stream)
{
    const int KP = st_kp_of(d->F), F = d->F, N = d->N, m0 = half ? KP / 2 : 0;
    const stg::RowMap ma = stg::live_frames(d->T, d->H, d->N, d->N, d->L);
    const int R = ma.rows(d->B);
    const int room = (int)((st_wgrad_ws_floats(d) - (size_t)64 * 2 * N) / ((size_t)KP * N));
    const int per = stm::nyq_blocks(N) / 2;
    int ns;
    const stg::TNOperand ta{w.dG + m0, (unsigned)(d->T * KP), (unsigned)KP}, tb{w.xp, (unsigned)(d->L + 2 * d->N), (unsigned)d->H};
    if (w.g16) {
        const int tiles = ((KP / 2 + 127) / 128) * (N / 128);
        ns = (2 * num_cus()) / (tiles > 0 ? tiles : 1);
        if (ns > R / 128) ns = R / 128; if (ns > room) ns = room; if (ns < 1) ns = 1;
        ST_TRY(wgrad16(d, w.dG16, (unsigned)(d->T * KP), w.xp16, (unsigned)(d->L + 2 * d->N), ma, R, w.wg, ns, stream, m0, KP / 2, (g_g16_crop & 8) ? d->L : 0));
        if (!half) { *nyq_io = stm::NyqJob{}; nyq_io->on = 0; }
    } else if (use_tn128(d, true) && stg::tn128_fits(ta, tb, w.xp, ma, N / 2, N, (size_t)d->B * d->T * KP, (size_t)d->B * (d->L + 2 * d->N))) {
        const int mh = (N / 2) / 128, tiles = mh * (N / 128);
        ns = num_cus() / (tiles > 0 ? tiles : 1); if (ns > 16) ns = 16; if (ns > R / 64) ns = R / 64; if (ns > room) ns = room; if (ns < 1) ns = 1;
        float* part = w.wg + (size_t)room * KP * N;
        int P = 0;
        const TNFrameMajor fm = tn_frame_major(ta, tb, ma, d->B, d->H, N, N, d->L, (g_tn_fm & 2) != 0);
        ST_TN128(fm.a, fm.b, w.xp, fm.map, R, N / 2, mh, (unsigned)(KP / 2), N, w.wg + (size_t)m0 * N, N, (size_t)KP * N, ns, st_stream(stream),
                 half ? nullptr : part, (unsigned)(F - 1), (unsigned)(KP / 2 + F - 1), &P, &fm.trim);
        if (!half) { nyq_io->part = part; nyq_io->P = P; nyq_io->on = 1; }
    } else {
        ST_LAUNCHED("analysis_wgrad");
        if (!half) { *nyq_io = stm::NyqJob{}; nyq_io->on = 0; }
        return analysis_wgrad_impl(d, w.dG, w.xp, true, 1.0f, w.wg, grads + L.offs[0], grads + L.offs[1], w.norm_a, stream, half, stage, stage_bf16);
    }
    ST_LAUNCHED("analysis_wgrad");
    hipLaunchKernelGGL(stm::wgrad_reduce_kernel, dim3(F + per), dim3(256), 0, st_stream(stream),
                       w.wg, ns, grads + L.offs[0], grads + L.offs[1], w.norm_a, N, F, KP, 0, half * F, F, stage, *nyq_io, half * per, stage_bf16);
    ST_LAUNCHED("analysis_wgrad_reduce");
    return ST_OK;
}
static int backward_impl(const st_dims* d, const Layout& L, const float* params, float* grads, const float* x,
                         const float* knobs, const float* g_mag_hat, const float* g_mag, float reg_coef, WS& w, void* stream, float* kg = nullptr)
{
// ... 592 lines not shown
    ST_REQ(params && grads && x && (knobs || d->K == 0) && y_true && ws, "st_dp_train_step: null pointer");
    if (!knobs) knobs = params;
    const float gs = (1.0f / (float)p->world) / loss_scale_of(d);
    const bool split_last = (force_exchange & 2) != 0;
    const int pack16 = ((force_exchange & 4) != 0 && ae_ht(d->prec) != 0) ? 1 : 0;
    WS w; carve(d, ws, &w);
    w.g16 = use_g16(d);
    {
        prof_mark("begin", stream);
        ST_TRY(forward_impl(d, L, params, x, knobs, y_true, nullptr, nullptr, nullptr, w, true, stream));
        const float reg_coef = loss_scale_of(d) * (float)(2e-5 / 10.0) / ((float)d->B * (float)d->OT * (float)d->F);
        int syn_slabs = 0; stm::NyqJob syn_nyq{}; syn_nyq.on = 0;
        float* const wg_main = w.wg;
        if (g_dp_inline) w.wg = w.wg2;
        ST_TRY(backward_syn(d, L, grads, w, stream, &syn_slabs, &syn_nyq));
        ST_TRY(dp_fork(p, stream));
        hipLaunchKernelGGL(stm::wgrad_reduce_kernel, dim3(st_norm_partials(d)), dim3(256), 0, p->cs,
                           w.wg, syn_slabs, grads + L.offs[2], grads + L.offs[3], w.norm_s, d->N, d->F, L.KP, 1, 0, 2 * d->F, (float*)nullptr, syn_nyq);
        w.wg = wg_main;
        if (!g_dp_inline) ST_HIP(hipEventRecord(p->wgfree, p->cs), "event record");
        ST_TRY(dp_allreduce_on_cs(p, grads + L.offs[2], L.offs[4] - L.offs[2], ncclFloat32));
        hipLaunchKernelGGL(stm::l1_partial_kernel, dim3(st_norm_partials(d)), dim3(256), 0, p->cs, grads + L.offs[2], L.offs[4] - L.offs[2], gs, w.norm_s);
        ST_TRY(backward_ae(d, L, params, grads, knobs, nullptr, nullptr, reg_coef, w, stream, 0, nullptr));
        ST_TRY(st_dp_allreduce(p, grads + L.offs[4], L.total - L.offs[4], stream));
        if (d->clip_all) hipLaunchKernelGGL(stm::l1_partial_kernel, dim3(NORM_E_PARTIALS), dim3(256), 0, p->cs, grads + L.n_stft, L.total - L.n_stft, gs, w.norm_e);
        if (!g_dp_inline) ST_HIP(hipStreamWaitEvent(st_stream(stream), p->wgfree, 0), "stream wait");
    }
    const int64_t half_n = (int64_t)d->F * d->N;
    bool last_in_line = false;
    if (!split_last && g_dp_inline) {
        ST_HIP(hipEventRecord(p->done, p->cs), "event record");
        ST_TRY(backward_p2(d, L, grads, x, w, stream, stage, pack16));
        ST_HIP(hipStreamWaitEvent(st_stream(stream), p->done, 0), "stream wait");
        ST_NCCL(p, p->AllReduce(stage, stage, (size_t)(2 * half_n), pack16 ? ncclBfloat16 : ncclFloat32, ncclSum, p->comm, st_stream(stream)), "ncclAllReduce");
        last_in_line = true;
    } else if (!split_last) {
        ST_TRY(backward_p2(d, L, grads, x, w, stream, stage, pack16));
        ST_TRY(dp_fork(p, stream));
        ST_TRY(dp_allreduce_on_cs(p, stage, 2 * half_n, pack16 ? ncclBfloat16 : ncclFloat32));
    } else {
        stm::NyqJob nyq{}; nyq.on = 0;
        for (int h = 0; h < 2; ++h) {
            ST_TRY(analysis_wgrad_half(d, L, grads, w, h, stage, pack16, &nyq, stream));
            void* part = pack16 ? (void*)(reinterpret_cast<unsigned short*>(stage) + (size_t)h * half_n) : (void*)(stage + (size_t)h * half_n);
            if (h == 1 && g_dp_inline) {
                ST_HIP(hipStreamWaitEvent(st_stream(stream), p->done, 0), "stream wait");
                ST_NCCL(p, p->AllReduce(part, part, (size_t)half_n, pack16 ? ncclBfloat16 : ncclFloat32, ncclSum, p->comm, st_stream(stream)), "ncclAllReduce");
                last_in_line = true;
                break;
            }
            ST_TRY(dp_fork(p, stream));
            ST_TRY(dp_allreduce_on_cs(p, part, half_n, pack16 ? ncclBfloat16 : ncclFloat32));
            if (g_dp_inline) ST_HIP(hipEventRecord(p->done, p->cs), "event record");
        }
    }
    if (!last_in_line) ST_TRY(st_dp_sync(p, stream));
    {
        const int np = st_norm_partials(d);
        hipLaunchKernelGGL(stm::unstage_l1_kernel, dim3(2 * d->F), dim3(256), 0, st_stream(stream), stage, grads + L.offs[0], grads + L.offs[1], d->F, d->N, gs, w.norm_a, np, pack16);
        ST_LAUNCHED("unstage_l1");
        stm::FinArgs f = fin_args(d, w.loss_p, w.reg_p, w.norm_a, w.norm_s, 1.0f);
        if (d->clip_all) { f.norm_e = w.norm_e; f.n_ne = NORM_E_PARTIALS; }
        return clip_adam_impl(params, grads, m, v, L.total, d->clip_all ? L.total : L.n_stft, scalars, gs, lr, beta1, beta2, eps, step, &f, stream);
    }
}


struct st_graph { hipGraph_t graph; hipGraphExec_t exec; };

static int attr_prepare(const st_dims* d)
{
    const int ht = ae_ht(d->prec);
#define ST_PREP3(K0_, K1_, K2_) do { if (ht == 1) ST_DYN_LDS(K1_); else if (ht == 2) ST_DYN_LDS(K2_); else ST_DYN_LDS(K0_); } while (0)
    if (ae_is_wide(d)) {
        ST_PREP3((sta::ae_inner_fwd_kernel<AE_FWD_NW, 0>), (sta::ae_inner_fwd_kernel<AE_FWD_NW, 1>), (sta::ae_inner_fwd_kernel<AE_FWD_NW, 2>));
        ST_PREP3((sta::ae_inner_fwd_kernel<9, 0>), (sta::ae_inner_fwd_kernel<9, 1>), (sta::ae_inner_fwd_kernel<9, 2>));
        ST_PREP3((sta::ae_inner_fwd_kernel<12, 0>), (sta::ae_inner_fwd_kernel<12, 1>), (sta::ae_inner_fwd_kernel<12, 2>));
        ST_PREP3((sta::ae_bwd_kernel<AE_BWD_NW, true, 0, 0>), (sta::ae_bwd_kernel<AE_BWD_NW, true, 1, 0>), (sta::ae_bwd_kernel<AE_BWD_NW, true, 2, 0>));
        ST_PREP3((stw::wide_dv_polar_kernel<0>), (stw::wide_dv_polar_kernel<1>), (stw::wide_dv_polar_kernel<2>));
    } else {
        ST_PREP3((sta::ae_fwd_kernel<AE_FWD_NW, 0>), (sta::ae_fwd_kernel<AE_FWD_NW, 1>), (sta::ae_fwd_kernel<AE_FWD_NW, 2>));
        if (ht == 1) ST_DYN_LDS((sta::ae_fwd32_kernel<AE_FWD_NW, 1>)); else if (ht == 2) ST_DYN_LDS((sta::ae_fwd32_kernel<AE_FWD_NW, 2>));
        if (ht == 0) { ST_DYN_LDS((sta::ae_fwd_kernel<11, 0>)); ST_DYN_LDS((sta::ae_fwd_kernel<11, 0, true>)); ST_DYN_LDS((sta::ae_fwd_kernel<AE_FWD_NW, 0, true>));
                       ST_DYN_LDS((sta::ae_bwd_kernel<AE_BWD_NW, false, 0, 0, true>)); ST_DYN_LDS((sta::ae_bwd_kernel<AE_BWD_NW, false, 0, 1, true>)); ST_DYN_LDS((sta::ae_bwd_kernel<AE_BWD_NW, false, 0, 2, true>)); }
        ST_PREP3((sta::ae_bwd_part_kernel<AE_SPLIT_NW, 1, 0, false>), (sta::ae_bwd_part_kernel<AE_SPLIT_NW, 1, 1, false>), (sta::ae_bwd_part_kernel<AE_SPLIT_NW, 1, 2, false>));
        ST_PREP3((sta::ae_bwd_part_kernel<AE_SPLIT_NW, 2, 0, false>), (sta::ae_bwd_part_kernel<AE_SPLIT_NW, 2, 1, false>), (sta::ae_bwd_part_kernel<AE_SPLIT_NW, 2, 2, false>));
        if (d->T - d->OT == 16) ST_PREP3((sta::ae_bwd_kernel<AE_BWD_NW, false, 0, 2>), (sta::ae_bwd_kernel<AE_BWD_NW, false, 1, 2>), (sta::ae_bwd_kernel<AE_BWD_NW, false, 2, 2>));
        else ST_PREP3((sta::ae_bwd_kernel<AE_BWD_NW, false, 0, 0>), (sta::ae_bwd_kernel<AE_BWD_NW, false, 1, 0>), (sta::ae_bwd_kernel<AE_BWD_NW, false, 2, 0>));
    }
#undef ST_PREP3
    if (g_nt128 && gemm_ht(d->prec) == 0) ST_DYN_LDS((stg::gemm_nt128_kernel));
    if (use_g16(d)) {
        if (gemm_ht(d->prec) == 2) {
            ST_DYN_LDS((stg::gemm16_nt256_kernel<2, stg::PolarStore>)); ST_DYN_LDS((stg::gemm16_nt256_kernel<2, stg::StoreC>));
            ST_DYN_LDS((stg::gemm16_nt_kernel<2, 64, stg::PolarStore>)); ST_DYN_LDS((stg::gemm16_nt_kernel<2, 64, stg::StoreC>)); ST_DYN_LDS((stg::gemm16_tn_kernel<2, 64>));
        } else {
            ST_DYN_LDS((stg::gemm16_nt256_kernel<1, stg::PolarStore>)); ST_DYN_LDS((stg::gemm16_nt256_kernel<1, stg::StoreC>));
            ST_DYN_LDS((stg::gemm16_nt_kernel<1, 64, stg::PolarStore>)); ST_DYN_LDS((stg::gemm16_nt_kernel<1, 64, stg::StoreC>)); ST_DYN_LDS((stg::gemm16_tn_kernel<1, 64>));
        }
    }
    if (use_planes(d)) {
        ST_DYN_LDS((stg::gemm_planes_kernel<4, 3, stg::FramedNT<true>, stg::ChunkP, stg::PolarStore>));
        ST_DYN_LDS((stg::gemm_planes_kernel<8, 3, stg::FramedNT<true>, stg::ChunkP, stg::PolarStore>));
        ST_DYN_LDS((stg::gemm_planes_kernel<4, 3, stg::PlainNT, stg::ChunkP, stg::StoreC>));
        ST_DYN_LDS((stg::gemm_planes_kernel<4, 3, stg::FramedNT<true>, stg::ChunkP, stg::StoreC>));
    }
    (void)num_cus();
    return ST_OK;
}

extern "C" int st_graph_create(const st_dims* d, float* params, float* grads, float* m, float* v, const float* x,
                               const float* knobs, const float* y_true, void* ws, float* scalars,
                               const float* lr_table, int n_lr, float beta1, float beta2, float eps, void* stream, st_graph** out)
{
    Layout L; ST_TRY(make_layout(d, &L));
    ST_REQ(params && grads && m && v && x && (knobs || d->K == 0) && y_true && ws && scalars && lr_table && n_lr > 0 && out, "st_graph_create: bad arguments");
    if (!knobs) knobs = params;
    ST_REQ(!g_prof, "st_graph_create: switch the event profiling off first (event records would be captured)");
    ST_TRY(attr_prepare(d));
    hipStream_t s = st_stream(stream);
    if (hipStreamBeginCapture(s, hipStreamCaptureModeThreadLocal) != hipSuccess) return st_fail(ST_ERR_LAUNCH, "st_graph_create: hipStreamBeginCapture failed (is `stream` the legacy default stream?)");
    hipLaunchKernelGGL(stm::step_tick_kernel, dim3(1), dim3(64), 0, s, scalars, lr_table, n_lr);
    int rc = train_step_impl(d, params, grads, m, v, x, knobs, y_true, ws, scalars, 0.f, beta1, beta2, eps, 1, stream, true);
    hipGraph_t g = nullptr;
    const hipError_t e = hipStreamEndCapture(s, &g);
    if (rc != ST_OK) { if (g) (void)hipGraphDestroy(g); return rc; }
    if (e != hipSuccess || !g) return st_fail(ST_ERR_LAUNCH, "st_graph_create: capture failed: %s", hipGetErrorString(e));
    hipGraphExec_t ex = nullptr;
    if (hipGraphInstantiate(&ex, g, nullptr, nullptr, 0) != hipSuccess) { (void)hipGraphDestroy(g); return st_fail(ST_ERR_LAUNCH, "st_graph_create: hipGraphInstantiate failed"); }
    st_graph* p = new st_graph{g, ex};
    *out = p;
    return ST_OK;
}
extern "C" int st_graph_launch(st_graph* g, void* stream)
{
    ST_REQ(g && g->exec, "st_graph_launch: null graph");
    const hipError_t e = hipGraphLaunch(g->exec, st_stream(stream));
    if (e != hipSuccess) return st_fail(ST_ERR_LAUNCH, "hipGraphLaunch: %s", hipGetErrorString(e));
    return ST_OK;
}
extern "C" int st_graph_destroy(st_graph* g)
{
    if (!g) return ST_OK;
    if (g->exec) (void)hipGraphExecDestroy(g->exec);
    if (g->graph) (void)hipGraphDestroy(g->graph);
    delete g;
    return ST_OK;
}
```

### signaltrain_amd/csrc/st_misc.h

```cpp
#pragma once
#include "st_common.h"

namespace stm {

__device__ __forceinline__ void fold_row(const float* __restrict__ Sr, const float* __restrict__ Si, float* __restrict__ Sfold,
                                         const int N, const int F, const int KP, const int row)
{
    const int half = KP / 2;
    const bool is_im = row >= half;
    const int k = is_im ? row - half : row;
    const float* S = is_im ? Si : Sr;
    const bool valid = k < F;
    const bool paired = valid && k >= 1 && k <= F - 2;
    const float sgn = is_im ? -1.f : 1.f;
    for (int n4 = threadIdx.x; n4 < N / 4; n4 += blockDim.x) {
        float4 v = make_float4(0.f, 0.f, 0.f, 0.f);
        if (valid) {
            v = reinterpret_cast<const float4*>(S + (size_t)k * N)[n4];
            if (paired) {
                const float4 u = reinterpret_cast<const float4*>(S + (size_t)(N - k) * N)[n4];
                v.x += sgn * u.x; v.y += sgn * u.y; v.z += sgn * u.z; v.w += sgn * u.w;
            }
        }
        reinterpret_cast<float4*>(Sfold + (size_t)row * N)[n4] = v;
    }
}
__global__ void __launch_bounds__(256)
fold_kernel(const float* __restrict__ Sr, const float* __restrict__ Si, float* __restrict__ Sfold, int N, int F, int KP)
{
    fold_row(Sr, Si, Sfold, N, F, KP, blockIdx.x);
}

__device__ __forceinline__ void zero_dead_frame(float* __restrict__ a0, float* __restrict__ a1, float* __restrict__ a2, float* __restrict__ a3,
                                                const int T, const int F, const int t_lo, const int Tv, const int blk)
{
    const int nd = T - Tv;
    const int b = blk / nd, j = blk - b * nd;
    const int t = j < t_lo ? j : j + Tv;
    const size_t base = ((size_t)b * T + t) * F;
    for (int f = threadIdx.x; f < F; f += 256) {
        if (a0) a0[base + f] = 0.f;
        if (a1) a1[base + f] = 0.f;
        if (a2) a2[base + f] = 0.f;
        if (a3) a3[base + f] = 0.f;
    }
}
__global__ void __launch_bounds__(256)
zero_dead_frames_kernel(float* __restrict__ a0, float* __restrict__ a1, float* __restrict__ a2, float* __restrict__ a3,
                        int T, int F, int t_lo, int Tv)
{
    zero_dead_frame(a0, a1, a2, a3, T, F, t_lo, Tv, blockIdx.x);
}

__host__ __device__ __forceinline__ int mae_partial_offset(const int n_loss) { return (n_loss + 3) & ~3; }
template <bool MAE = false>
__global__ void __launch_bounds__(256)
ola_loss_kernel(const float* __restrict__ frs, const float* __restrict__ x, const float* __restrict__ y_true,
                float* __restrict__ y_hat, float* __restrict__ dsyn, float* __restrict__ loss_partial,
                int L, int N, int H, int OT, int ysz, float inv_count, int nslab, size_t slab, int dsyn_pad,
                unsigned short* __restrict__ dsyn16 = nullptr, int ht = 0)
{
    __shared__ float red[4];
    const int b = blockIdx.y;
    const int j = blockIdx.x * 256 + threadIdx.x;
    float lc = 0.f;
    [[maybe_unused]] float ma = 0.f;
    if (j < ysz) {
        int t0 = j / H + 1;
        int t1 = (N + j) / H;
        if (t1 > OT - 1) t1 = OT - 1;
        const float* fb = frs + (size_t)b * OT * N;
        float s = 0.f;
        for (int t = t0; t <= t1; ++t) {
            const size_t o = (size_t)t * N + (N + j - H * t);
            float v[6];
#pragma unroll
            for (int z = 0; z < 6; ++z) v[z] = fb[(z < nslab ? z * slab : 0) + o];
#pragma unroll
            for (int z = 0; z < 6; ++z) s += z < nslab ? v[z] : 0.f;
        }
        const float out = x ? 2.0f * (s + 0.5f * x[(size_t)b * L + (L - ysz) + j]) : s;
        if (y_hat) y_hat[(size_t)b * ysz + j] = out;
        if (y_true) {
            const float dlt = y_true[(size_t)b * ysz + j] - out;
// ... 82 lines not shown
            const float dlt = ys[q] - out[q];
            const float a = fabsf(dlt);
            float l1;
            if (a < 8.0f) { const float u = expm1f(0.5f * a); const float sh = 0.5f * (u + u / (u + 1.0f)); l1 = log1pf(2.0f * sh * sh); }
            else l1 = a + log1pf(__expf(-2.0f * a)) - 0.69314718056f;
            lc += y_true ? l1 : 0.f;
            if (MAE) ma += y_true ? a : 0.f;
            if (!MAE) ds[q] = -2.0f * tanhf(dlt) * inv_count;
        }
        if (y_hat) *reinterpret_cast<float4*>(y_hat + (size_t)b * ysz + j) = make_float4(out[0], out[1], out[2], out[3]);
        if (!MAE && y_true) {
            const size_t o = (size_t)b * (ysz + 2 * dsyn_pad) + dsyn_pad + j;
            if (dsyn16) *reinterpret_cast<uint2*>(dsyn16 + o) = st_to_h16x4(make_float4(ds[0], ds[1], ds[2], ds[3]), ht);
            else if (dsyn) *reinterpret_cast<float4*>(dsyn + o) = make_float4(ds[0], ds[1], ds[2], ds[3]);
        }
    }
    if (!MAE && (dsyn || dsyn16) && dsyn_pad > 0) {
        const size_t ro = (size_t)b * (ysz + 2 * dsyn_pad);
        for (int m = blockIdx.x * 256 + threadIdx.x; m < 2 * dsyn_pad; m += gridDim.x * 256) {
            if (dsyn16) dsyn16[ro + (m < dsyn_pad ? m : ysz + m)] = 0;
            else dsyn[ro + (m < dsyn_pad ? m : ysz + m)] = 0.f;
        }
    }
    if (loss_partial) {
        float q = lc;
#pragma unroll
        for (int o = 1; o < 64; o <<= 1) q += __shfl_xor(q, o);
        const int slot = 4 * blockIdx.x + (threadIdx.x >> 6);
        if ((threadIdx.x & 63) == 0 && slot < nslot) loss_partial[blockIdx.y * nslot + slot] = q;
    }
    if (MAE) {
        float q = ma;
#pragma unroll
        for (int o = 1; o < 64; o <<= 1) q += __shfl_xor(q, o);
        const int slot = 4 * blockIdx.x + (threadIdx.x >> 6);
        if ((threadIdx.x & 63) == 0 && slot < nslot) loss_partial[mae_partial_offset(gridDim.y * nslot) + blockIdx.y * nslot + slot] = q;
    }
}

__device__ __forceinline__ void pad_scale_block(const float* __restrict__ in, float* __restrict__ out, const int Ls, const int pad, const float s,
                                                const int bx, const int nbx, const int b, unsigned short* __restrict__ out16 = nullptr, const int ht = 0)
{
    const int Lp4 = (Ls + 2 * pad) / 4;
    const float4* src = reinterpret_cast<const float4*>(in + (size_t)b * Ls);
    float4* dst = reinterpret_cast<float4*>(out + (size_t)b * (Ls + 2 * pad));
    uint2* dst16 = reinterpret_cast<uint2*>(out16 + (size_t)b * (Ls + 2 * pad));
    for (int i = bx * 256 + threadIdx.x; i < Lp4; i += nbx * 256) {
        const int j = i - pad / 4;
        float4 v = make_float4(0.f, 0.f, 0.f, 0.f);
        if (j >= 0 && j < Ls / 4) { v = src[j]; v.x *= s; v.y *= s; v.z *= s; v.w *= s; }
        if (out16) dst16[i] = st_to_h16x4(v, ht);
        else dst[i] = v;
    }
}
__global__ void __launch_bounds__(256)
pad_scale_kernel(const float* __restrict__ in, float* __restrict__ out, int Ls, int pad, float s)
{
    pad_scale_block(in, out, Ls, pad, s, blockIdx.x, gridDim.x, blockIdx.y);
}

struct PadJobs { const float* src[4]; float* dst[4]; int rows[4], cols[4], pitch[4], blk0[5]; };
__device__ __forceinline__ void pad_rows4_block(const PadJobs& j, const int blk)
{
    int q = 0;
#pragma unroll
    for (int k = 1; k < 4; ++k) q += blk >= j.blk0[k];
    const int i = (blk - j.blk0[q]) * 256 + threadIdx.x;
    if (i >= j.rows[q] * j.pitch[q]) return;
    const int r = i / j.pitch[q], c = i - r * j.pitch[q];
    j.dst[q][i] = c < j.cols[q] ? j.src[q][r * j.cols[q] + c] : 0.f;
}
struct PrepWide {
    float *Vm, *Vp; int FP, B; unsigned R;
    float *H4Km, *H4Kp; const float* knobs; int K;
    PadJobs pj;
    int n_vpad, n_kn, n_pj;
};
struct PrepArgs {
    const float* x; float* xp; int Ls, pad; float scale; int nbx, n_pad;
    const float* Sr; const float* Si; float* Sfold; float* SfoldT; int N, F, KP, n_fold;
    float *re, *im, *mag, *phs; int T, t_lo, Tv;
    int ht; unsigned short *xp16, *Sfold16, *SfoldT16, *W16; const float* Wr; const float* Wi; int n_w16, n_dead;
    PrepWide wd;
};
__device__ __forceinline__ void fold_tile(const float* __restrict__ Sr, const float* __restrict__ Si, float* __restrict__ Sfold,
                                          float* __restrict__ SfoldT, const int N, const int F, const int KP, const int tile,
                                          unsigned short* __restrict__ Sfold16 = nullptr, unsigned short* __restrict__ SfoldT16 = nullptr, const int ht = 0)
{
    __shared__ float tl[32][33];
    const int ntn = N / 32, tk = tile / ntn, tn = tile - tk * ntn;
    const int half = KP / 2;
    const int cx = threadIdx.x & 31, ry = threadIdx.x >> 5;
    float a0[4], a1[4];
#pragma unroll
    for (int j = 0; j < 4; ++j) {
        const int row = tk * 32 + ry + 8 * j, n = tn * 32 + cx;
        const bool is_im = row >= half;
        const int k = is_im ? row - half : row;
        const float* S = is_im ? Si : Sr;
        const int kc = k < F ? k : F - 1, km = (k >= 1 && k <= F - 2) ? N - k : N - 1;
        a0[j] = S[(size_t)kc * N + n]; a1[j] = S[(size_t)km * N + n];
    }
#pragma unroll
    for (int j = 0; j < 4; ++j) {
        const int row = tk * 32 + ry + 8 * j, n = tn * 32 + cx;
        const bool is_im = row >= half;
        const int k = is_im ? row - half : row;
        float v = 0.f;
        if (k < F) {
            v = a0[j];
            if (k >= 1 && k <= F - 2) v += is_im ? -a1[j] : a1[j];
        }
        if (Sfold16) Sfold16[(size_t)row * N + n] = st_to_h16(v, ht); else Sfold[(size_t)row * N + n] = v;
        tl[ry + 8 * j][cx] = v;
    }
    __syncthreads();
#pragma unroll
    for (int j = 0; j < 4; ++j) {
        const int n = tn * 32 + ry + 8 * j, row = tk * 32 + cx;
        if (SfoldT16) SfoldT16[(size_t)n * KP + row] = st_to_h16(tl[cx][ry + 8 * j], ht); else SfoldT[(size_t)n * KP + row] = tl[cx][ry + 8 * j];
    }
}
__global__ void __launch_bounds__(256)
prep_kernel(const PrepArgs a)
{
    const int blk = blockIdx.x;
    if (blk < a.n_pad) { const int b = blk / a.nbx; pad_scale_block(a.x, a.xp, a.Ls, a.pad, a.scale, blk - b * a.nbx, a.nbx, b, a.ht ? a.xp16 : nullptr, a.ht); }
    else if (blk < a.n_pad + a.n_fold) fold_tile(a.Sr, a.Si, a.Sfold, a.SfoldT, a.N, a.F, a.KP, blk - a.n_pad, a.ht ? a.Sfold16 : nullptr, a.ht ? a.SfoldT16 : nullptr, a.ht);
    else if (blk < a.n_pad + a.n_fold + a.n_dead) {
        zero_dead_frame(a.re, a.im, a.mag, a.phs, a.T, a.F, a.t_lo, a.Tv, blk - a.n_pad - a.n_fold);
        if (a.wd.n_vpad) {
            const int nd = a.T - a.Tv, j0 = blk - a.n_pad - a.n_fold, b = j0 / nd, j = j0 - b * nd, t = j < a.t_lo ? j : j + a.Tv;
            const size_t o = (size_t)t * a.wd.R + (size_t)b * a.wd.FP;
            for (int f = threadIdx.x; f < a.wd.FP; f += 256) { a.wd.Vm[o + f] = 0.f; a.wd.Vp[o + f] = 0.f; }
        }
    }
    else if (blk < a.n_pad + a.n_fold + a.n_dead + a.wd.n_vpad) {
        const int np = a.wd.FP - a.F;
        const unsigned idx = (unsigned)(blk - a.n_pad - a.n_fold - a.n_dead) * 256u + threadIdx.x;
        if (np > 0 && idx < (unsigned)a.wd.B * (unsigned)a.T * (unsigned)np) {
            const unsigned bt = idx / (unsigned)np, pcol = idx - bt * (unsigned)np, b = bt / (unsigned)a.T, t = bt - b * (unsigned)a.T;
            const size_t o = (size_t)t * a.wd.R + (size_t)b * a.wd.FP + a.F + pcol;
            a.wd.Vm[o] = 0.f; a.wd.Vp[o] = 0.f;
        }
    }
    else if (blk < a.n_pad + a.n_fold + a.n_dead + a.wd.n_vpad + a.wd.n_kn) {
        const unsigned Q = (unsigned)a.wd.FP / 4, idx = (unsigned)(blk - a.n_pad - a.n_fold - a.n_dead - a.wd.n_vpad) * 256u + threadIdx.x;
        if (idx < (unsigned)a.wd.K * (unsigned)a.wd.B * Q) {
            const unsigned kb = idx / Q, j = idx - kb * Q, k = kb / (unsigned)a.wd.B, b = kb - k * (unsigned)a.wd.B;
            const int f0 = 4 * (int)j;
            const float v = a.wd.knobs[b * a.wd.K + k];
            const float4 q = make_float4(f0 < a.F ? v : 0.f, f0 + 1 < a.F ? v : 0.f, f0 + 2 < a.F ? v : 0.f, f0 + 3 < a.F ? v : 0.f);
            const size_t o = (size_t)(16 + k) * a.wd.R + (size_t)b * a.wd.FP;
            reinterpret_cast<float4*>(a.wd.H4Km + o)[j] = q; reinterpret_cast<float4*>(a.wd.H4Kp + o)[j] = q;
        }
    }
    else if (blk < a.n_pad + a.n_fold + a.n_dead + a.wd.n_vpad + a.wd.n_kn + a.wd.n_pj)
        pad_rows4_block(a.wd.pj, blk - a.n_pad - a.n_fold - a.n_dead - a.wd.n_vpad - a.wd.n_kn);
    else {
        const size_t i4 = (size_t)(blk - a.n_pad - a.n_fold - a.n_dead - a.wd.n_vpad - a.wd.n_kn - a.wd.n_pj) * 256 + threadIdx.x, n4 = a.N / 4;
        if (i4 < (size_t)2 * a.F * n4) {
            const int jrow = (int)(i4 / n4), c = (int)(i4 - (size_t)jrow * n4);
            const float4 v = reinterpret_cast<const float4*>(((jrow & 1) ? a.Wi : a.Wr) + (size_t)(jrow >> 1) * a.N)[c];
            reinterpret_cast<uint2*>(a.W16 + (size_t)jrow * a.N)[c] = st_to_h16x4(v, a.ht);
        }
    }
}

__global__ void __launch_bounds__(256)
scale_kernel(const float* __restrict__ in, float* __restrict__ out, int64_t n, float s)
{
    for (int64_t i = (int64_t)blockIdx.x * 256 + threadIdx.x; i < n; i += (int64_t)gridDim.x * 256) out[i] = s * in[i];
}

__device__ __forceinline__ void polar_bwd_block(const float* __restrict__ re, const float* __restrict__ im, const float* __restrict__ dmag,
                 const float* __restrict__ dphs, const float* __restrict__ g_mag, float* __restrict__ dG, const int F, const int KP,
                 const float sat,
                 const int bx, const int r, unsigned short* __restrict__ dG16 = nullptr, const int ht = 0)
{
    const int half = KP / 2;
    const int c = bx * 256 + threadIdx.x;
    if (c >= half) return;
    float gre = 0.f, gim = 0.f;
    if (c < F) {
        const size_t i = (size_t)r * F + c;
        const float a = re[i], bb = im[i], dm = dmag[i] + (g_mag ? g_mag[i] : 0.f), dp = dphs[i];
        const float mg = sqrtf(a * a + bb * bb);
        const float inv = mg > 0.f ? 1.0f / mg : 0.f;
        const float rp = a + 1e-7f;
        const float den = rp * rp + bb * bb;
        gre = dm * a * inv - dp * bb / den;
        gim = dm * bb * inv + dp * rp / den;
        if (sat > 0.f) { gre = __builtin_amdgcn_fmed3f(gre, -sat, sat); gim = __builtin_amdgcn_fmed3f(gim, -sat, sat); }
    }
    if (dG16) { dG16[(size_t)r * KP + c] = st_to_h16(gre, ht); dG16[(size_t)r * KP + half + c] = st_to_h16(gim, ht); }
    if (dG) { dG[(size_t)r * KP + c] = gre; dG[(size_t)r * KP + half + c] = gim; }
}
constexpr int POLAR_EPT = 4;
__host__ __device__ static inline unsigned polar_magic(int half) { return (unsigned)((0x100000000ull + (unsigned)half - 1) / (unsigned)half); }
__host__ static inline bool polar_flat_ok(long long R, int half)
{
    const unsigned long long M = polar_magic(half), slack = M * (unsigned)half - 0x100000000ull;
    const unsigned long long total = (unsigned long long)R * (unsigned)half;
    return total < 0x7fffffffull && (slack == 0 || total < 0x100000000ull / slack);
}
__device__ __forceinline__ void polar_bwd_flat(const float* __restrict__ re, const float* __restrict__ im, const float* __restrict__ dmag,
                 const float* __restrict__ dphs, const float* __restrict__ g_mag, float* __restrict__ dG, const int F, const int KP, const float sat,
                 const unsigned bx, const unsigned total, const unsigned magic, unsigned short* __restrict__ dG16, const int ht)
{
    const unsigned half = (unsigned)KP / 2;
    unsigned r[POLAR_EPT], c[POLAR_EPT]; bool on[POLAR_EPT], live[POLAR_EPT];
    float a[POLAR_EPT], bb[POLAR_EPT], dm[POLAR_EPT], dp[POLAR_EPT];
#pragma unroll
    for (int u = 0; u < POLAR_EPT; ++u) {
        const unsigned e = (bx * POLAR_EPT + u) * 256 + threadIdx.x;
        on[u] = e < total;
        r[u] = __umulhi(on[u] ? e : 0u, magic); c[u] = (on[u] ? e : 0u) - r[u] * half;
        live[u] = on[u] && c[u] < (unsigned)F;
        const size_t i = live[u] ? (size_t)r[u] * F + c[u] : 0;
        a[u] = re[i]; bb[u] = im[i]; dm[u] = dmag[i] + (g_mag ? g_mag[i] : 0.f); dp[u] = dphs[i];
    }
#pragma unroll
    for (int u = 0; u < POLAR_EPT; ++u) {
        float gre = 0.f, gim = 0.f;
        if (live[u]) {
            const float mg = sqrtf(a[u] * a[u] + bb[u] * bb[u]);
            const float inv = mg > 0.f ? 1.0f / mg : 0.f;
            const float rp = a[u] + 1e-7f;
            const float den = rp * rp + bb[u] * bb[u];
            gre = dm[u] * a[u] * inv - dp[u] * bb[u] / den;
            gim = dm[u] * bb[u] * inv + dp[u] * rp / den;
            if (sat > 0.f) { gre = __builtin_amdgcn_fmed3f(gre, -sat, sat); gim = __builtin_amdgcn_fmed3f(gim, -sat, sat); }
        }
        if (on[u]) {
            const size_t o = (size_t)r[u] * KP + c[u];
            if (dG16) { dG16[o] = st_to_h16(gre, ht); dG16[o + half] = st_to_h16(gim, ht); }
            if (dG) { dG[o] = gre; dG[o + half] = gim; }
        }
    }
}
__global__ void __launch_bounds__(256)
polar_bwd_kernel(const float* __restrict__ re, const float* __restrict__ im, const float* __restrict__ dmag,
                 const float* __restrict__ dphs, const float* __restrict__ g_mag, float* __restrict__ dG, int R, int F, int KP, const float sat,
// ... 589 lines not shown
```

Before: 10.92 million frames/s.

## Prebuild autoencoder LDS weight images once in prep kernel for fwd/bwd

Adds a prep-kernel pass that builds the swizzled, zero-padded LDS images of both autoencoder weight sets, the frequency weight table, and the transposed dgrad images in workspace memory. The fused forward kernel and the kept-activation backward kernel then copy these images straight into LDS with vector loads, instead of each block doing scattered gathers, zero-fill, a barrier and an expf table. This removes per-block setup cost in exchange for an extra workspace write/read and more prep blocks. The g_ae_save knob range grows so the old path can still be selected, and ablation flags are added.

```diff
diff --git a/signaltrain_amd/csrc/st_ae.h b/signaltrain_amd/csrc/st_ae.h
--- a/signaltrain_amd/csrc/st_ae.h
+++ b/signaltrain_amd/csrc/st_ae.h
@@ -41,7 +41,7 @@
 struct AEParamRegs { float v[NL][(64 * 32 + NT - 1) / NT]; float bv[NL]; };
 
 template <int NT>
-__device__ __forceinline__ void ae_params_issue(AEParamRegs<NT>& r, const float* __restrict__ ae, const AEOffsets& go,
+__host__ __device__ __forceinline__ void ae_params_issue(AEParamRegs<NT>& r, const float* __restrict__ ae, const AEOffsets& go,
                                                 const int T, const int OT, const int K, const int tid, const int l0, const int l1)
 {
     const int out[NL] = {64, 32, 16, 16, 16, 16, 32, 64, OT};
@@ -67,7 +67,7 @@
     else return __uint_as_float((unsigned)b << 16);
 }
 template <int NT, int BF = 0>
-__device__ __forceinline__ void ae_params_scatter(float* lds, const AEParamRegs<NT>& r, const int T, const int OT, const int K,
+__host__ __device__ __forceinline__ void ae_params_scatter(float* lds, const AEParamRegs<NT>& r, const int T, const int OT, const int K,
                                                   const int tid, const int l0, const int l1, const bool dgrad_images)
 {
     const int out[NL] = {64, 32, 16, 16, 16, 16, 32, 64, OT};
@@ -103,17 +103,24 @@
 __device__ inline void ae_load_lds(float* lds, const float* __restrict__ ae, const AEOffsets& go, const int T, const int OT, const int K,
                                    const int tid, const int l0, const int l1, const bool dgrad_images)
 {
+    const int total = dgrad_images ? CL::BWD_TOTAL : CL::FWD_TOTAL;
+#if ST_AE_ABLATE & 128
+    for (int e = tid; e < total; e += NT) lds[e] = 0.f;
+#else
     AEParamRegs<NT> r;
     ae_params_issue<NT>(r, ae, go, T, OT, K, tid, l0, l1);
-    const int total = dgrad_images ? CL::BWD_TOTAL : CL::FWD_TOTAL;
     for (int e = tid; e < total; e += NT) lds[e] = 0.f;
     __syncthreads();
     ae_params_scatter<NT, BF>(lds, r, T, OT, K, tid, l0, l1, dgrad_images);
+#endif
 }
 template <int NT, int BF = 0>
 __device__ inline void ae_load_lds2(float* lds, const float* __restrict__ ae_m, const float* __restrict__ ae_p, const AEOffsets& go,
                                     const int T, const int OT, const int K, const int tid, const int l0, const int l1)
 {
+#if ST_AE_ABLATE & 128
+    for (int e = tid; e < 2 * CL::FWD_TOTAL; e += NT) lds[e] = 0.f;
+#else
     AEParamRegs<NT> rm, rp;
     ae_params_issue<NT>(rm, ae_m, go, T, OT, K, tid, l0, l1);
     ae_params_issue<NT>(rp, ae_p, go, T, OT, K, tid, l0, l1);
@@ -121,6 +128,47 @@
     __syncthreads();
     ae_params_scatter<NT, BF>(lds, rm, T, OT, K, tid, l0, l1, false);
     ae_params_scatter<NT, BF>(lds + CL::FWD_TOTAL, rp, T, OT, K, tid, l0, l1, false);
+#endif
+}
+
+constexpr int AE_IMG_DG = CL::BWD_TOTAL - CL::FWD_TOTAL;
+__host__ __device__ constexpr int ae_img_fwd_floats(const int FP) { return 2 * CL::FWD_TOTAL + FP; }
+__host__ __device__ constexpr int ae_img_floats(const int FP) { return ae_img_fwd_floats(FP) + 2 * AE_IMG_DG; }
+struct AEImgJob { const float* ae[2]; float* img; AEOffsets go; int T, OT, K, F, FP; float expfac; int n, n_blk; };
+__host__ __device__ __forceinline__ float ae_freq_weight(const float expfac, const int f) { return expf(expfac * (float)f); }
+__host__ __device__ __forceinline__ void ae_img_build(const AEImgJob& j, const int p)
+{
+    if (p >= j.n) return;
+    const int out[NL] = {64, 32, 16, 16, 16, 16, 32, 64, j.OT};
+    const int in[NL] = {j.T, 64, 32, 16, 16 + j.K, 16, 16, 32, 64};
+    const int outp[NL] = {CL::O0, CL::O1, CL::O2, CL::O3, CL::O4, CL::O5, CL::O6, CL::O7, CL::O8};
+    const int inp[NL] = {CL::I0, CL::I1, CL::I2, CL::I3, CL::I4, CL::I5, CL::I6, CL::I7, CL::I8};
+    const int ao[NL + 1] = {CL::A0, CL::A1, CL::A2, CL::A3, CL::A4, CL::A5, CL::A6, CL::A7, CL::A8, CL::AEND};
+    const int bo[NL + 1] = {CL::B0, CL::B1, CL::B2, CL::B3, CL::B4, CL::B5, CL::B6, CL::B7, CL::B8, CL::FWD_TOTAL};
+    float v = 0.f;
+    const int q0 = p - 2 * CL::FWD_TOTAL;
+    if (q0 >= 0 && q0 < j.FP) v = q0 < j.F ? ae_freq_weight(j.expfac, q0) : 0.f;
+    else {
+        const bool dg = q0 >= 0;
+        const int net = dg ? (q0 - j.FP >= AE_IMG_DG) : (p >= CL::FWD_TOTAL);
+        const int q = dg ? q0 - j.FP - net * AE_IMG_DG : p - net * CL::FWD_TOTAL;
+        const float* __restrict__ ae = j.ae[net];
+        if (!dg && q >= CL::AEND) {
+#pragma unroll
+            for (int l = 0; l < NL; ++l)
+                if (q >= bo[l] && q < bo[l + 1]) { const int o = q - bo[l]; if (o < out[l]) v = ae[j.go.b[l] + o]; }
+        } else {
+#pragma unroll
+            for (int l = 0; l < NL; ++l)
+                if (q >= ao[l] && q < ao[l + 1]) {
+                    const int s = (q - ao[l]) >> 2, lo = (q - ao[l]) & 3;
+                    const int o = dg ? ((s / inp[l]) << 2) + lo : s % outp[l];
+                    const int i = dg ? s % inp[l] : ((s / outp[l]) << 2) + lo;
+                    if (o < out[l] && i < in[l]) v = ae[j.go.w[l] + o * in[l] + i];
+                }
+        }
+    }
+    j.img[p] = v;
 }
 
 #define ST_MFMA16(a, b, c) __builtin_amdgcn_mfma_f32_16x16x4f32((a), (b), (c), 0, 0, 0)
@@ -359,21 +407,37 @@
               const int B, const int T, const int OT, const int F, const int K, const int KP, const float expfac,
               float* __restrict__ h4x = nullptr,
               unsigned short* __restrict__ AA16 = nullptr, const int aa_ht = 0,
-              float* __restrict__ sv = nullptr)
+              float* __restrict__ sv = nullptr,
+              const float* __restrict__ img = nullptr)
 {
     extern __shared__ __attribute__((aligned(16))) float lds[];
     const int tid = threadIdx.x, lane = tid & 63, wave = tid >> 6;
     const int g = lane >> 4, c = lane & 15;
     const float* const lw[2] = {lds, lds + CL::FWD_TOTAL};
-    ae_load_lds2<NW * 64, BF>(lds, ae_m, ae_p, go, T, OT, K, tid, 0, NL);
-    __syncthreads();
-
     const int FP = KP / 2, gpw = FP / 16;
+    float* const wtab = lds + 2 * CL::FWD_TOTAL;
+    const bool ready = BF == 0 && !(ST_AE_ABLATE & 128) && img != nullptr;
+    if (ready) {
+        constexpr int N4 = 2 * CL::FWD_TOTAL / 4, U = (N4 + NW * 64 - 1) / (NW * 64);
+        f32x4 v[U];
+#pragma unroll
+        for (int u = 0; u < U; ++u) { const int e = tid + u * NW * 64; v[u] = reinterpret_cast<const f32x4*>(img)[e < N4 ? e : 0]; }
+        for (int i = tid; i < FP / 4; i += NW * 64) reinterpret_cast<f32x4*>(wtab)[i] = reinterpret_cast<const f32x4*>(img + 2 * CL::FWD_TOTAL)[i];
+#pragma unroll
+        for (int u = 0; u < U; ++u) { const int e = tid + u * NW * 64; if (e < N4) reinterpret_cast<f32x4*>(lds)[e] = v[u]; }
+    } else {
+        ae_load_lds2<NW * 64, BF>(lds, ae_m, ae_p, go, T, OT, K, tid, 0, NL);
+        __syncthreads();
+#if ST_AE_ABLATE & 128
+        for (int i = tid; i < FP; i += NW * 64) wtab[i] = 0.f;
+#else
+        for (int i = tid; i < FP; i += NW * 64) wtab[i] = i < F ? ae_freq_weight(expfac, i) : 0.f;
+#endif
+    }
+
     const int ngroups = B * gpw;
     const int KQ = (K + 3) / 4;
     float reg = 0.f;
-    float* const wtab = lds + 2 * CL::FWD_TOTAL;
-    for (int i = tid; i < FP; i += NW * 64) wtab[i] = i < F ? expf(expfac * (float)i) : 0.f;
     unsigned toF[4], toK[4];
 #pragma unroll
     for (int r = 0; r < 4; ++r) { toF[r] = ST_MUL24(4 * g + r, F); toK[r] = ST_MUL24(4 * g + r, KP); }
@@ -711,7 +775,7 @@
 
 constexpr int AE_BWD_SCR = (32 + 16 + 16) * SP + 2 * 4 * 320;
 constexpr int ae_bwd_lds_floats(int nw) { return (CL::BWD_TOTAL + nw * AE_BWD_SCR) > nw * CL::FWD_TOTAL ? (CL::BWD_TOTAL + nw * AE_BWD_SCR) : nw * CL::FWD_TOTAL; }
-template <int NW, bool INNER = false, int BF = 0, int VAR = 1, bool SAVED = false, bool KG = false>
+template <int NW, bool INNER = false, int BF = 0, int VAR = 1, bool SAVED = false, bool KG = false, bool IMG = false>
 __global__ void __launch_bounds__(NW * 64, 1)
 ae_bwd_kernel(const float* __restrict__ mag, const float* __restrict__ phs, const float* __restrict__ knobs,
               const float* __restrict__ ae_m, const float* __restrict__ ae_p, const AEOffsets go, const int PG,
@@ -722,9 +786,11 @@
               const int to_lo, const int to_hi,
               const int nslab, const size_t slab,
               const float* __restrict__ sv = nullptr,
-              float* __restrict__ kg = nullptr)
+              float* __restrict__ kg = nullptr,
+              const float* __restrict__ img = nullptr)
 {
     static_assert(!SAVED || (!INNER && BF == 0), "the kept-activation backward exists for the fused fp32 geometries");
+    static_assert(!IMG || SAVED, "ready-made images: the kept-activation backward only");
     extern __shared__ __attribute__((aligned(16))) float lds[];
     const int ae = blockIdx.y;
     const int tid = threadIdx.x, lane = tid & 63, wave = tid >> 6;
@@ -735,6 +801,17 @@
     float* Ts = Ys + 16 * SP;
     float* XH = Ts + 16 * SP;
     float* XD = XH + 4 * 320;
+    if constexpr (IMG && !(ST_AE_ABLATE & 128)) {
+        const int FPi = KP / 2;
+        const float* const dg = img + 2 * CL::FWD_TOTAL + FPi + ae * AE_IMG_DG;
+        constexpr int N4 = AE_IMG_DG / 4, U = (N4 + NW * 64 - 1) / (NW * 64);
+        f32x4 v[U];
+#pragma unroll
+        for (int u = 0; u < U; ++u) { const int e = tid + u * NW * 64; v[u] = reinterpret_cast<const f32x4*>(dg)[e < N4 ? e : 0]; }
+        for (int i = tid; i < FPi / 4; i += NW * 64) reinterpret_cast<f32x4*>(lds)[i] = reinterpret_cast<const f32x4*>(img + 2 * CL::FWD_TOTAL)[i];
+#pragma unroll
+        for (int u = 0; u < U; ++u) { const int e = tid + u * NW * 64; if (e < N4) reinterpret_cast<f32x4*>(lds + CL::G0)[e] = v[u]; }
+    } else
     ae_load_lds<NW * 64, BF>(lw, ae ? ae_p : ae_m, go, INNER ? 16 : T, INNER ? 16 : OT, K, tid, INNER ? 1 : 0, INNER ? 8 : NL, true);
     __syncthreads();
 
@@ -908,7 +985,9 @@
         float dxA[4], mtA[4];
         if constexpr (!INNER) {
             ST_FENCE();
-            const float wf = fv ? expf(expfac * (float)f) : 0.f;
+            float wf;
+            if constexpr (IMG && !(ST_AE_ABLATE & 128)) wf = fv ? lds[f] : 0.f;
+            else wf = fv ? ae_freq_weight(expfac, f) : 0.f;
 #pragma unroll
             for (int r = 0; r < 4; ++r) {
                 const int to = 4 * g + r;
@@ -1057,6 +1136,17 @@
             }
         }
     }
+#if ST_AE_ABLATE & 256
+    {
+#define ST_KT(x, A, Bq) { _Pragma("unroll") for (int a_ = 0; a_ < A; ++a_) _Pragma("unroll") for (int b_ = 0; b_ < Bq; ++b_) _Pragma("unroll") for (int r_ = 0; r_ < 4; ++r_) asm volatile("" :: "v"(x[a_][b_][r_])); }
+#define ST_KB(x, A) { _Pragma("unroll") for (int a_ = 0; a_ < A; ++a_) asm volatile("" :: "v"(x[a_])); }
+        ST_KT(rW1, 4, 2) ST_KT(rW2, 2, 4) ST_KT(rW3, 1, 2) ST_KT(rW4, 1, 1) ST_KT(rW5, 1, 2) ST_KT(rW6, 1, 1) ST_KT(rW7, 2, 1) ST_KT(rW8, 4, 2) ST_KT(rW9, 1, 4)
+        ST_KB(rb1, 4) ST_KB(rb2, 2) ST_KB(rb3, 1) ST_KB(rb4, 1) ST_KB(rb5, 1) ST_KB(rb6, 1) ST_KB(rb7, 2) ST_KB(rb8, 4) ST_KB(rb9, 1)
+#undef ST_KT
+#undef ST_KB
+        return;
+    }
+#endif
     __syncthreads();
     static_assert(NW == 4, "the store pass sums exactly four per-wave images");
     float* dwl = lds + wave * CL::FWD_TOTAL;
diff --git a/signaltrain_amd/csrc/st_api.hip b/signaltrain_amd/csrc/st_api.hip
--- a/signaltrain_amd/csrc/st_api.hip
+++ b/signaltrain_amd/csrc/st_api.hip
@@ -187,7 +187,7 @@
     {7000, 2, &g_xt, 0, nullptr},
     {8000, 2, &g_ae_split, 0, nullptr}, {8002, 1, &g_ae_split, -1, nullptr},
     {8100, 2, &g_ae32, 0, nullptr},
-    {8200, 2, &g_ae_save, 0, nullptr},
+    {8200, 3, &g_ae_save, 0, nullptr},
     {8300, 2, &g_dp_inline, 0, nullptr},
     {9000, 2, &g_frs_nt, 0, nullptr},
     {9100, 1, &g_pl_shape, 0, nullptr}, {9103, 1, &g_pl_shape, 3, nullptr},
@@ -356,6 +356,15 @@
 static int ae_parts_max(const st_dims* d) { return ae_split_grid(d) > ae_bwd_grid(d) ? ae_split_grid(d) : ae_bwd_grid(d); }
 static bool ae_use_saved(const st_dims* d) { return g_ae_save && !ae_is_wide(d) && ae_ht(d->prec) == 0 && !ae_use_split(d); }
 static float* ae_sv_ptr(const st_dims* d, const Layout& L, float* aews) { return aews + 2 * ae_h4_floats(d) + (size_t)ae_parts_max(d) * 2 * L.PG; }
+static int ae_img_level(const st_dims* d)
+{
+    if (g_ae_save == 2 || ae_is_wide(d) || ae_ht(d->prec) != 0 || ae_use_split(d)) return 0;
+    const int FP = st_kp_of(d->F) / 2;
+    const size_t room = 2 * ae_h4_floats(d);
+    if (FP > sta::CL::FWD_TOTAL || room < (size_t)sta::ae_img_fwd_floats(FP)) return 0;
+    return room >= (size_t)sta::ae_img_floats(FP) ? 2 : 1;
+}
+static float* ae_img_ptr(float* aews) { return aews; }
 static const char* ae_kg_why(const st_dims* d)
 {
     if (ae_is_wide(d)) return nullptr;
@@ -423,7 +432,7 @@
 
 static int ae_fwd_impl(const st_dims* d, const float* mag, const float* phs, const float* knobs,
                        const float* ae_m, const float* ae_p, float* mag_hat, float* phs_hat, float* AA,
-                       float* reg_partial, float* ws, void* stream, unsigned short* AA16 = nullptr, bool wide_in_done = false, float* sv = nullptr);
+                       float* reg_partial, float* ws, void* stream, unsigned short* AA16 = nullptr, bool wide_in_done = false, float* sv = nullptr, const float* img = nullptr);
 extern "C" int st_ae_fwd(const st_dims* d, const float* mag, const float* phs, const float* knobs,
                          const float* ae_m, const float* ae_p, float* mag_hat, float* phs_hat, float* AA,
                          float* reg_partial, float* ws, void* stream)
@@ -432,7 +441,7 @@
 }
 static int ae_fwd_impl(const st_dims* d, const float* mag, const float* phs, const float* knobs,
                        const float* ae_m, const float* ae_p, float* mag_hat, float* phs_hat, float* AA,
-                       float* reg_partial, float* ws, void* stream, unsigned short* AA16, bool wide_in_done, float* sv)
+                       float* reg_partial, float* ws, void* stream, unsigned short* AA16, bool wide_in_done, float* sv, const float* img)
 {
     Layout L; ST_TRY(make_layout(d, &L));
     const int aa_ht = AA16 ? gemm_ht(d->prec) : 0;
@@ -451,7 +460,7 @@
 #define ST_AE_FWD_LAUNCH(HT_) do { ST_DYN_LDS((sta::ae_fwd_kernel<AE_FWD_NW, HT_>)); \
         hipLaunchKernelGGL((sta::ae_fwd_kernel<AE_FWD_NW, HT_>), dim3(ae_fwd_grid(d)), dim3(AE_FWD_NW * 64), lds, st_stream(stream), \
                            mag, phs, knobs, ae_m, ae_p, L.go, mag_hat, phs_hat, AA, reg_partial, \
-                           d->B, d->T, d->OT, d->F, d->K, L.KP, expfac, ws, AA16, aa_ht); } while (0)
+                           d->B, d->T, d->OT, d->F, d->K, L.KP, expfac, ws, AA16, aa_ht, (float*)nullptr, HT_ == 0 ? img : nullptr); } while (0)
     const bool use32 = g_ae32 && ae_ht(d->prec) != 0 && L.KP / 2 <= 17 * 32 && AE_FWD_NW == 8;
 #define ST_AE_FWD32_LAUNCH(HT_) do { ST_DYN_LDS((sta::ae_fwd32_kernel<AE_FWD_NW, HT_>)); \
         hipLaunchKernelGGL((sta::ae_fwd32_kernel<AE_FWD_NW, HT_>), dim3(ae_fwd_grid(d)), dim3(AE_FWD_NW * 64), (size_t)sta::ae32_lds_floats(L.KP / 2) * sizeof(float), st_stream(stream), \
@@ -465,13 +474,13 @@
             ST_REQ(mag_hat, "st_ae_fwd: internal: kept activations on a code-only pass");
 #define ST_AE_FWD_SV(NW_) do { ST_DYN_LDS((sta::ae_fwd_kernel<NW_, 0, true>)); \
             hipLaunchKernelGGL((sta::ae_fwd_kernel<NW_, 0, true>), dim3(ae_fwd_grid(d)), dim3(NW_ * 64), lds, st_stream(stream), \
-                               mag, phs, knobs, ae_m, ae_p, L.go, mag_hat, phs_hat, AA, reg_partial, d->B, d->T, d->OT, d->F, d->K, L.KP, expfac, ws, AA16, aa_ht, sv); } while (0)
+                               mag, phs, knobs, ae_m, ae_p, L.go, mag_hat, phs_hat, AA, reg_partial, d->B, d->T, d->OT, d->F, d->K, L.KP, expfac, ws, AA16, aa_ht, sv, img); } while (0)
             if (ae_fwd_nw(d) == 11) ST_AE_FWD_SV(11); else ST_AE_FWD_SV(AE_FWD_NW);
 #undef ST_AE_FWD_SV
         } else if (ae_fwd_nw(d) == 11) {
             ST_DYN_LDS((sta::ae_fwd_kernel<11, 0>));
             hipLaunchKernelGGL((sta::ae_fwd_kernel<11, 0>), dim3(ae_fwd_grid(d)), dim3(11 * 64), lds, st_stream(stream),
-                               mag, phs, knobs, ae_m, ae_p, L.go, mag_hat, phs_hat, AA, reg_partial, d->B, d->T, d->OT, d->F, d->K, L.KP, expfac, ws, AA16, aa_ht);
+                               mag, phs, knobs, ae_m, ae_p, L.go, mag_hat, phs_hat, AA, reg_partial, d->B, d->T, d->OT, d->F, d->K, L.KP, expfac, ws, AA16, aa_ht, (float*)nullptr, img);
         } else ST_AE_FWD_LAUNCH(0);
     }
 #undef ST_AE_FWD_LAUNCH
@@ -857,7 +866,7 @@
                        const float* dAA, const float* g_mag_hat, float reg_coef, float* dmag, float* dphs, float* ws,
                        float* g_m, float* g_p, bool have_fwd, void* stream, bool* defer_reduce = nullptr,
                        const PolarSink* sink = nullptr, const stw::SynReduce* syn = nullptr, float* norm_e = nullptr, int* n_norm_e = nullptr,
-                       float* kg = nullptr)
+                       float* kg = nullptr, bool have_img = false)
 {
     Layout L; ST_TRY(make_layout(d, &L));
     ST_REQ(mag && phs && (knobs || d->K == 0) && ae_m && ae_p && mag_hat && phs_hat && dAA && dmag && dphs && ws && g_m && g_p, "st_ae_bwd: null pointer");
@@ -912,11 +921,13 @@
     const int var = g_mag_hat ? 1 : (d->T - d->OT == 16 ? 2 : 0);
     if (have_fwd && ae_use_saved(d)) {
         const float* sv = ae_sv_ptr(d, L, ws);
-#define ST_AE_BWD_SV_K(VAR_, KG_) do { ST_DYN_LDS((sta::ae_bwd_kernel<AE_BWD_NW, false, 0, VAR_, true, KG_>)); \
-        hipLaunchKernelGGL((sta::ae_bwd_kernel<AE_BWD_NW, false, 0, VAR_, true, KG_>), dim3(grid, 2), dim3(AE_BWD_NW * 64), lds, st_stream(stream), \
+        const float* img = (have_img && ae_img_level(d) == 2) ? ae_img_ptr(ws) : nullptr;
+#define ST_AE_BWD_SV_K(VAR_, KG_, IMG_) do { ST_DYN_LDS((sta::ae_bwd_kernel<AE_BWD_NW, false, 0, VAR_, true, KG_, IMG_>)); \
+        hipLaunchKernelGGL((sta::ae_bwd_kernel<AE_BWD_NW, false, 0, VAR_, true, KG_, IMG_>), dim3(grid, 2), dim3(AE_BWD_NW * 64), lds, st_stream(stream), \
                        mag, phs, knobs, ae_m, ae_p, L.go, L.PG, mag_hat, phs_hat, dAA, g_mag_hat, reg_coef, expfac, \
-                       dmag, dphs, parts, d->B, d->T, d->OT, d->F, d->K, L.KP, live.t_lo, live.t_lo + live.Tv - 1, st_synth_slabs(d), (size_t)d->B * d->OT * L.KP, sv, kg); } while (0)
-#define ST_AE_BWD_SV(VAR_) do { if (kg) ST_AE_BWD_SV_K(VAR_, true); else ST_AE_BWD_SV_K(VAR_, false); } while (0)
+                       dmag, dphs, parts, d->B, d->T, d->OT, d->F, d->K, L.KP, live.t_lo, live.t_lo + live.Tv - 1, st_synth_slabs(d), (size_t)d->B * d->OT * L.KP, sv, kg, img); } while (0)
+#define ST_AE_BWD_SV(VAR_) do { if (img) { if (kg) ST_AE_BWD_SV_K(VAR_, true, true); else ST_AE_BWD_SV_K(VAR_, false, true); } \
+                                else { if (kg) ST_AE_BWD_SV_K(VAR_, true, false); else ST_AE_BWD_SV_K(VAR_, false, false); } } while (0)
         if (var == 1) ST_AE_BWD_SV(1); else if (var == 2) ST_AE_BWD_SV(2); else ST_AE_BWD_SV(0);
 #undef ST_AE_BWD_SV
 #undef ST_AE_BWD_SV_K
@@ -1324,7 +1335,13 @@
             a.wd.n_vpad = (int)(((size_t)d->B * d->T * (FP - d->F) + 255) / 256); if (a.wd.n_vpad < 1) a.wd.n_vpad = 1;
             a.wd.n_kn = (int)(((size_t)d->K * d->B * (FP / 4) + 255) / 256);
         }
-        hipLaunchKernelGGL(stm::prep_kernel, dim3(a.n_pad + a.n_fold + n_dead + a.wd.n_vpad + a.wd.n_kn + a.wd.n_pj + a.n_w16), dim3(256), 0, st_stream(stream), a);
+        a.ai = sta::AEImgJob{}; a.ai.n_blk = 0;
+        if (ae_img_level(d)) {
+            a.ai.ae[0] = ae_m; a.ai.ae[1] = ae_p; a.ai.img = ae_img_ptr(w.aews); a.ai.go = L.go;
+            a.ai.T = d->T; a.ai.OT = d->OT; a.ai.K = d->K; a.ai.F = d->F; a.ai.FP = L.KP / 2; a.ai.expfac = (float)(7.0 / d->F);
+            a.ai.n = ae_img_level(d) == 2 ? sta::ae_img_floats(L.KP / 2) : sta::ae_img_fwd_floats(L.KP / 2); a.ai.n_blk = (a.ai.n + 255) / 256;
+        }
+        hipLaunchKernelGGL(stm::prep_kernel, dim3(a.n_pad + a.n_fold + n_dead + a.wd.n_vpad + a.wd.n_kn + a.wd.n_pj + a.ai.n_blk + a.n_w16), dim3(256), 0, st_stream(stream), a);
         ST_LAUNCHED("prep");
     }
     const bool planes = use_planes(d) && !w.g16;
@@ -1339,7 +1356,8 @@
     float* sv = nullptr;
     if (save && ae_use_saved(d)) { Layout Ls; ST_TRY(make_layout(d, &Ls)); sv = ae_sv_ptr(d, Ls, w.aews); }
     ST_TRY(ae_fwd_impl(d, w.mag, w.phs, knobs, ae_m, ae_p, w.mag_hat, w.phs_hat, w.AA, w.reg_p,
-                       (ae_is_wide(d) || (save && ae_use_split(d))) ? w.aews : nullptr, stream, w.g16 ? w.AA16 : nullptr, wide_direct, sv));
+                       (ae_is_wide(d) || (save && ae_use_split(d))) ? w.aews : nullptr, stream, w.g16 ? w.AA16 : nullptr, wide_direct, sv,
+                       ae_img_level(d) ? ae_img_ptr(w.aews) : nullptr));
     if (w.g16) ST_TRY(synthesis_frames16(d, w, stream)); else
     if (planes) ST_TRY(synthesis_frames_planes(d, w, stream)); else
     ST_TRY(synthesis_frames_impl(d, w.AA, w.Sfold, w.SfoldT, w.frs, stream));
@@ -1384,7 +1402,7 @@
     }
     ST_TRY(ae_bwd_impl(d, w.mag, w.phs, knobs, ae_m, ae_p, w.mag_hat, w.phs_hat, w.dAA, g_mag_hat, reg_coef, w.dmag, w.dphs,
                        w.aews, grads + L.offs[4], grads + L.offs[22], true, stream, &deferred, &sink, syn.wg ? &syn : nullptr,
-                       (d->clip_all && ae_is_wide(d)) ? w.norm_e : nullptr, &w.n_norm_e, kg));
+                       (d->clip_all && ae_is_wide(d)) ? w.norm_e : nullptr, &w.n_norm_e, kg, true));
     if (!deferred) return ST_OK;
     stm::PostAeArgs a;
     a.ws = w.aews + 2 * ae_h4_floats(d); a.nparts = ae_use_split(d) ? ae_split_grid(d) : ae_bwd_grid(d); a.PG = L.PG; a.g_m = grads + L.offs[4]; a.g_p = grads + L.offs[22];
@@ -2143,7 +2161,9 @@
         ST_PREP3((sta::ae_fwd_kernel<AE_FWD_NW, 0>), (sta::ae_fwd_kernel<AE_FWD_NW, 1>), (sta::ae_fwd_kernel<AE_FWD_NW, 2>));
         if (ht == 1) ST_DYN_LDS((sta::ae_fwd32_kernel<AE_FWD_NW, 1>)); else if (ht == 2) ST_DYN_LDS((sta::ae_fwd32_kernel<AE_FWD_NW, 2>));
         if (ht == 0) { ST_DYN_LDS((sta::ae_fwd_kernel<11, 0>)); ST_DYN_LDS((sta::ae_fwd_kernel<11, 0, true>)); ST_DYN_LDS((sta::ae_fwd_kernel<AE_FWD_NW, 0, true>));
-                       ST_DYN_LDS((sta::ae_bwd_kernel<AE_BWD_NW, false, 0, 0, true>)); ST_DYN_LDS((sta::ae_bwd_kernel<AE_BWD_NW, false, 0, 1, true>)); ST_DYN_LDS((sta::ae_bwd_kernel<AE_BWD_NW, false, 0, 2, true>)); }
+                       ST_DYN_LDS((sta::ae_bwd_kernel<AE_BWD_NW, false, 0, 0, true>)); ST_DYN_LDS((sta::ae_bwd_kernel<AE_BWD_NW, false, 0, 1, true>)); ST_DYN_LDS((sta::ae_bwd_kernel<AE_BWD_NW, false, 0, 2, true>));
+                       ST_DYN_LDS((sta::ae_bwd_kernel<AE_BWD_NW, false, 0, 0, true, false, true>)); ST_DYN_LDS((sta::ae_bwd_kernel<AE_BWD_NW, false, 0, 1, true, false, true>));
+                       ST_DYN_LDS((sta::ae_bwd_kernel<AE_BWD_NW, false, 0, 2, true, false, true>)); }
         ST_PREP3((sta::ae_bwd_part_kernel<AE_SPLIT_NW, 1, 0, false>), (sta::ae_bwd_part_kernel<AE_SPLIT_NW, 1, 1, false>), (sta::ae_bwd_part_kernel<AE_SPLIT_NW, 1, 2, false>));
         ST_PREP3((sta::ae_bwd_part_kernel<AE_SPLIT_NW, 2, 0, false>), (sta::ae_bwd_part_kernel<AE_SPLIT_NW, 2, 1, false>), (sta::ae_bwd_part_kernel<AE_SPLIT_NW, 2, 2, false>));
         if (d->T - d->OT == 16) ST_PREP3((sta::ae_bwd_kernel<AE_BWD_NW, false, 0, 2>), (sta::ae_bwd_kernel<AE_BWD_NW, false, 1, 2>), (sta::ae_bwd_kernel<AE_BWD_NW, false, 2, 2>));
diff --git a/signaltrain_amd/csrc/st_misc.h b/signaltrain_amd/csrc/st_misc.h
--- a/signaltrain_amd/csrc/st_misc.h
+++ b/signaltrain_amd/csrc/st_misc.h
@@ -1,5 +1,6 @@
 #pragma once
 #include "st_common.h"
+#include "st_ae.h"
 
 namespace stm {
 
@@ -248,6 +249,7 @@
     float *re, *im, *mag, *phs; int T, t_lo, Tv;
     int ht; unsigned short *xp16, *Sfold16, *SfoldT16, *W16; const float* Wr; const float* Wi; int n_w16, n_dead;
     PrepWide wd;
+    sta::AEImgJob ai;
 };
 __device__ __forceinline__ void fold_tile(const float* __restrict__ Sr, const float* __restrict__ Si, float* __restrict__ Sfold,
                                           float* __restrict__ SfoldT, const int N, const int F, const int KP, const int tile,
@@ -323,8 +325,10 @@
     }
     else if (blk < a.n_pad + a.n_fold + a.n_dead + a.wd.n_vpad + a.wd.n_kn + a.wd.n_pj)
         pad_rows4_block(a.wd.pj, blk - a.n_pad - a.n_fold - a.n_dead - a.wd.n_vpad - a.wd.n_kn);
+    else if (blk < a.n_pad + a.n_fold + a.n_dead + a.wd.n_vpad + a.wd.n_kn + a.wd.n_pj + a.ai.n_blk)
+        sta::ae_img_build(a.ai, (blk - a.n_pad - a.n_fold - a.n_dead - a.wd.n_vpad - a.wd.n_kn - a.wd.n_pj) * 256 + (int)threadIdx.x);
     else {
-        const size_t i4 = (size_t)(blk - a.n_pad - a.n_fold - a.n_dead - a.wd.n_vpad - a.wd.n_kn - a.wd.n_pj) * 256 + threadIdx.x, n4 = a.N / 4;
+        const size_t i4 = (size_t)(blk - a.n_pad - a.n_fold - a.n_dead - a.wd.n_vpad - a.wd.n_kn - a.wd.n_pj - a.ai.n_blk) * 256 + threadIdx.x, n4 = a.N / 4;
         if (i4 < (size_t)2 * a.F * n4) {
             const int jrow = (int)(i4 / n4), c = (int)(i4 - (size_t)jrow * n4);
             const float4 v = reinterpret_cast<const float4*>(((jrow & 1) ? a.Wi : a.Wr) + (size_t)(jrow >> 1) * a.N)[c];
```

Result: faster. 11.06 million frames/s, median of 6 (+1.3%).
